# halajun/VDO_SLAM

Measured on NVIDIA H100. Metric: LM iterations/sec (batch factor-graph solve), higher is better.
Workload: dtype f64

## Files before the change

### vdo_slam_b200/csrc/ba_bodies.cuh

```cuda
#pragma once
#include "ba_math.cuh"
#include "ba_types.h"

namespace vdo {

VDO_HD double body_lin_tracklet(const BaDev& d, int t, bool write) {
  const int kb = d.tk_begin[t], ke = d.tk_begin[t + 1];
  double chi = 0.0, carry_d = 0.0, carry_b[3] = {0, 0, 0};
  double p[3] = {d.pt[3 * kb], d.pt[3 * kb + 1], d.pt[3 * kb + 2]};
  for (int k = kb; k < ke; ++k) {
    double dsum = carry_d, b[3] = {carry_b[0], carry_b[1], carry_b[2]};
    carry_d = 0; carry_b[0] = carry_b[1] = carry_b[2] = 0;
    const int eb = d.lm_obs_begin[k], ee = d.lm_obs_begin[k + 1];
    for (int e = eb; e < ee; ++e) {
      Iso T; iso_load(d.se3 + 12 * (size_t)d.lm_cam[e], T);
      double Zc[3]; iso_inv_apply(T, p, Zc);
      const double* z = d.lm_z + 3 * (size_t)e;
      double err[3] = {Zc[0] - z[0], Zc[1] - z[1], Zc[2] - z[2]};
      const int cls = d.lm_cls[e];
      const double w = d.obs_cls_w[cls];
      double rho, hw; huber(w * (err[0] * err[0] + err[1] * err[1] + err[2] * err[2]), d.obs_cls_d[cls], rho, hw);
      chi += rho;
      if (write) {
        const double om = w * hw;
// ... 133 lines not shown
    } else {
      d.tk_gamma[k] = 0.0;
    }
    d.pt_g[k] = 1.0 / (sk + tk - dk);
    t_next = tk;
  }
}

VDO_HD void body_vertex_transform(const BaDev& d, int c, const double* __restrict__ v, double* __restrict__ vw) {
  const double* T = d.se3 + 12 * (size_t)c;
  double al[3], be[3], tb[3];
  rot_apply(T, v + 6 * (size_t)c, al);
  rot_apply(T, v + 6 * (size_t)c + 3, be);
  cross3(T + 9, be, tb);
  double* o = vw + 6 * (size_t)c;
  o[0] = -al[0] - 2 * tb[0]; o[1] = -al[1] - 2 * tb[1]; o[2] = -al[2] - 2 * tb[2];
  o[3] = be[0]; o[4] = be[1]; o[5] = be[2];
  if (d.vh) {
    double* oh = d.vh + 6 * (size_t)c;
    oh[0] = al[0] + tb[0]; oh[1] = al[1] + tb[1]; oh[2] = al[2] + tb[2]; oh[3] = be[0]; oh[4] = be[1]; oh[5] = be[2];
  }
}

VDO_HD void body_schur_tracklet(const BaDev& d, int t, int mode, const double* __restrict__ v, double* __restrict__ out) {
  const int kb = d.tk_begin[t], ke = d.tk_begin[t + 1];
  double carry_u[3] = {0, 0, 0};
  double y_prev[3] = {0, 0, 0}, f_prev = 0.0, Rprev[9] = {1, 0, 0, 0, 1, 0, 0, 0, 1};
  double p[3] = {d.pt[3 * kb], d.pt[3 * kb + 1], d.pt[3 * kb + 2]};
  for (int k = kb; k < ke; ++k) {
    double u[3] = {carry_u[0], carry_u[1], carry_u[2]};
    carry_u[0] = carry_u[1] = carry_u[2] = 0;
    const int h = d.tk_h[k];
    double Rh[9] = {1, 0, 0, 0, 1, 0, 0, 0, 1};
    double pn[3] = {0, 0, 0};
    if (mode != 0) {
      const int eb = d.lm_obs_begin[k], ee = d.lm_obs_begin[k + 1];
      for (int e = eb; e < ee; ++e) {
        const double* w = d.vw + 6 * (size_t)d.lm_cam[e];
        double pxb[3]; cross3(p, w + 3, pxb);
        const double om = d.lm_omega[e];
        u[0] += om * (w[0] + 2 * pxb[0]); u[1] += om * (w[1] + 2 * pxb[1]); u[2] += om * (w[2] + 2 * pxb[2]);
      }
    }
    if (h >= 0) {
      Iso H; iso_load(d.se3 + 12 * (size_t)h, H);
#pragma unroll
      for (int i = 0; i < 9; ++i) Rh[i] = H.R[i];
      pn[0] = d.pt[3 * (k + 1)]; pn[1] = d.pt[3 * (k + 1) + 1]; pn[2] = d.pt[3 * (k + 1) + 2];
      if (mode != 0) {
        double q[3]; iso_inv_apply(H, pn, q);
        double a[3]; ter_Jh_mul(q, v + 6 * (size_t)h, a);
        const double om = d.tk_omega[k];
        u[0] += om * a[0]; u[1] += om * a[1]; u[2] += om * a[2];
        double Ra[3]; rot_apply(H.R, a, Ra);
        carry_u[0] = -om * Ra[0]; carry_u[1] = -om * Ra[1]; carry_u[2] = -om * Ra[2];
      }
    }
    double y[3];
    if (mode == 0) { y[0] = d.bl[3 * k]; y[1] = d.bl[3 * k + 1]; y[2] = d.bl[3 * k + 2]; }
    else if (mode == 1) { y[0] = u[0]; y[1] = u[1]; y[2] = u[2]; }
    else { y[0] = d.bl[3 * k] - u[0]; y[1] = d.bl[3 * k + 1] - u[1]; y[2] = d.bl[3 * k + 2] - u[2]; }
    if (k > kb) {
      double Ry[3]; rot_apply(Rprev, y_prev, Ry);
      y[0] += f_prev * Ry[0]; y[1] += f_prev * Ry[1]; y[2] += f_prev * Ry[2];
    }
    if (ke - kb == 1) {
      const double is = 1.0 / d.pt_s[k];
      out[3 * k] = y[0] * is; out[3 * k + 1] = y[1] * is; out[3 * k + 2] = y[2] * is;
      return;
    }
    out[3 * k] = y[0]; out[3 * k + 1] = y[1]; out[3 * k + 2] = y[2];
    y_prev[0] = y[0]; y_prev[1] = y[1]; y_prev[2] = y[2];
    f_prev = d.tk_omega[k] / d.pt_s[k];
#pragma unroll
    for (int i = 0; i < 9; ++i) Rprev[i] = Rh[i];
    if (h >= 0) { p[0] = pn[0]; p[1] = pn[1]; p[2] = pn[2]; }
    else if (k + 1 < ke) { p[0] = d.pt[3 * (k + 1)]; p[1] = d.pt[3 * (k + 1) + 1]; p[2] = d.pt[3 * (k + 1) + 2]; }
  }
  double zn[3] = {0, 0, 0};
  for (int k = ke - 1; k >= kb; --k) {
    double y[3] = {out[3 * k], out[3 * k + 1], out[3 * k + 2]};
    if (k < ke - 1) {
      const int h = d.tk_h[k];
      if (h >= 0) {
        const double* R = d.se3 + 12 * (size_t)h;
        double Rt[3]; rot_t_apply(R, zn, Rt);
        const double om = d.tk_omega[k];
        y[0] += om * Rt[0]; y[1] += om * Rt[1]; y[2] += om * Rt[2];
      }
    }
    const double is = 1.0 / d.pt_s[k];
    zn[0] = y[0] * is; zn[1] = y[1] * is; zn[2] = y[2] * is;
    out[3 * k] = zn[0]; out[3 * k + 1] = zn[1]; out[3 * k + 2] = zn[2];
  }
}

VDO_HD void body_lin_vertex_obs(const BaDev& d, const Iso& T, int e, double* A21, double* g6) {
  const double* p = d.pt + 3 * (size_t)d.vm_pt[e];
  double Zc[3]; iso_inv_apply(T, p, Zc);
  const double* z = d.vm_z + 3 * (size_t)e;
  double err[3] = {Zc[0] - z[0], Zc[1] - z[1], Zc[2] - z[2]};
  const int cls = d.vm_cls[e];
  const double w = d.obs_cls_w[cls];
  double rho, hw; huber(w * (err[0] * err[0] + err[1] * err[1] + err[2] * err[2]), d.obs_cls_d[cls], rho, hw);
  const double om = w * hw;
  d.vm_omega[e] = om;
  obs_accumulate_pose(Zc, err, om, A21, g6);
}
VDO_HD void body_schur_vertex_obs(const BaDev& d, const Iso& T, int e, double* acc6) {
  const int k = d.vm_pt[e];
  const double* p = d.pt + 3 * (size_t)k;
  double Zc[3]; iso_inv_apply(T, p, Zc);
  double a[3]; rot_t_apply(T.R, d.zl + 3 * (size_t)k, a);
  double o[6]; obs_JcT_mul(Zc, a, o);
  const double om = d.vm_omega[e];
#pragma unroll
  for (int i = 0; i < 6; ++i) acc6[i] += om * o[i];
}
VDO_HD void body_lin_vertex_ter(const BaDev& d, const Iso& H, int e, double* A21, double* g6) {
  const int k = d.hm_p1[e];
  const double* p1 = d.pt + 3 * (size_t)k;
  double q[3]; iso_inv_apply(H, p1 + 3, q);
  double err[3] = {p1[0] - q[0], p1[1] - q[1], p1[2] - q[2]};
  const int cls = d.hm_cls[e];
  const double w = d.ter_cls_w[cls];
  double rho, hw; huber(w * (err[0] * err[0] + err[1] * err[1] + err[2] * err[2]), d.ter_cls_d[cls], rho, hw);
  const double om = w * hw;
  d.hm_omega[e] = om;
  ter_accumulate_pose(q, err, om, A21, g6);
}
VDO_HD void body_schur_vertex_ter(const BaDev& d, const Iso& H, int e, double* acc6) {
  const int k = d.hm_p1[e];
  double q[3]; iso_inv_apply(H, d.pt + 3 * (size_t)(k + 1), q);
  double Rz[3]; rot_t_apply(H.R, d.zl + 3 * (size_t)(k + 1), Rz);
  const double* z1 = d.zl + 3 * (size_t)k;
  double a[3] = {z1[0] - Rz[0], z1[1] - Rz[1], z1[2] - Rz[2]};
  double o[6]; ter_JhT_mul(q, a, o);
  const double om = d.hm_omega[e];
#pragma unroll
  for (int i = 0; i < 6; ++i) acc6[i] += om * o[i];
}

VDO_HD bool body_se3_edge(const BaDev& d, int e, bool jac, double& chi, double* Hi, double* Hj, double* Hoff, double* gi, double* gj) {
  const int i = d.se_i[e], j = d.se_j[e];
  Iso Z, Xi; iso_load(d.se_Z + 12 * (size_t)e, Z); iso_load(d.se3 + 12 * (size_t)i, Xi);
  double err[6], Ji[36], Jj[36];
  double w = d.se_w[e];
  if (j < 0) {
    edge_prior_eval(Z, Xi, err, Ji, jac);
    double e2 = 0; for (int k = 0; k < 6; ++k) e2 += err[k] * err[k];
    chi = w * e2;
  } else {
    Iso Xj; iso_load(d.se3 + 12 * (size_t)j, Xj);
    edge_se3_eval(Z, Xi, Xj, err, Ji, Jj, jac);
    double e2 = 0; for (int k = 0; k < 6; ++k) e2 += err[k] * err[k];
    double rho, hw; huber(w * e2, d.se_delta[e], rho, hw);
    chi = rho; w *= hw;
  }
  if (!jac) return j >= 0;
  for (int r = 0; r < 6; ++r) {
    double g = 0;
    for (int k = 0; k < 6; ++k) g += Ji[6 * k + r] * err[k];
    gi[r] = -w * g;
    for (int c = 0; c < 6; ++c) {
      double s = 0;
      for (int k = 0; k < 6; ++k) s += Ji[6 * k + r] * Ji[6 * k + c];
      Hi[6 * r + c] = w * s;
    }
  }
  if (j >= 0) {
    for (int r = 0; r < 6; ++r) {
      double g = 0;
      for (int k = 0; k < 6; ++k) g += Jj[6 * k + r] * err[k];
      gj[r] = -w * g;
      for (int c = 0; c < 6; ++c) {
        double s = 0, o = 0;
        for (int k = 0; k < 6; ++k) { s += Jj[6 * k + r] * Jj[6 * k + c]; o += Ji[6 * k + r] * Jj[6 * k + c]; }
        Hj[6 * r + c] = w * s;
        Hoff[6 * r + c] = w * o;
      }
    }
  }
  return j >= 0;
}

VDO_HD void body_hpp_mul(const BaDev& d, int v, double lambda, const double* __restrict__ x, double* __restrict__ out) {
  const double* H = d.Hpp + 36 * (size_t)v;
  const double* xv = x + 6 * (size_t)v;
  double o[6];
#pragma unroll
  for (int r = 0; r < 6; ++r) {
    double s = lambda * xv[r];
#pragma unroll
    for (int c = 0; c < 6; ++c) s += H[6 * r + c] * xv[c];
    o[r] = s;
  }
  for (int n = d.nbr_begin[v]; n < d.nbr_begin[v + 1]; ++n) {
    const double* B = d.se_Hoff + 36 * (size_t)d.nbr_edge[n];
    const double* xo = x + 6 * (size_t)d.nbr_other[n];
    if (d.nbr_tr[n]) {
#pragma unroll
      for (int r = 0; r < 6; ++r)
#pragma unroll
        for (int c = 0; c < 6; ++c) o[r] += B[6 * c + r] * xo[c];
    } else {
#pragma unroll
      for (int r = 0; r < 6; ++r)
#pragma unroll
        for (int c = 0; c < 6; ++c) o[r] += B[6 * r + c] * xo[c];
    }
  }
#pragma unroll
  for (int r = 0; r < 6; ++r) out[6 * (size_t)v + r] = d.own ? o[r] : 0.0;
  body_vertex_transform(d, v, x, d.vw);
}

VDO_HD void body_precond_vertex_obs(const BaDev& d, const Iso& T, int e, double* A21) {
  const int k = d.vm_pt[e];
  double Zc[3]; iso_inv_apply(T, d.pt + 3 * (size_t)k, Zc);
  const double om = d.vm_omega[e];
  const double zero[3] = {0, 0, 0};
  double g[6] = {0, 0, 0, 0, 0, 0};
  obs_accumulate_pose(Zc, zero, om * om * d.pt_g[k], A21, g);
}
VDO_HD void body_precond_vertex_ter(const BaDev& d, const Iso& H, int e, double* A21) {
  const int k = d.hm_p1[e];
  double q[3]; iso_inv_apply(H, d.pt + 3 * (size_t)(k + 1), q);
  const double om = d.hm_omega[e];
  const double zero[3] = {0, 0, 0};
  double g[6] = {0, 0, 0, 0, 0, 0};
  ter_accumulate_pose(q, zero, om * om * d.tk_gamma[k], A21, g);
}
VDO_HD void mat6_mul(const double* A, const double* B, double* C) {
  for (int r = 0; r < 6; ++r) for (int c = 0; c < 6; ++c) { double s = 0; for (int k = 0; k < 6; ++k) s += A[6 * r + k] * B[6 * k + c]; C[6 * r + c] = s; }
}
VDO_HD void mat6_mul_nt(const double* A, const double* B, double* C) {
  for (int r = 0; r < 6; ++r) for (int c = 0; c < 6; ++c) { double s = 0; for (int k = 0; k < 6; ++k) s += A[6 * r + k] * B[6 * c + k]; C[6 * r + c] = s; }
}
VDO_HD void mat6_mul_tn(const double* A, const double* B, double* C) {
  for (int r = 0; r < 6; ++r) for (int c = 0; c < 6; ++c) { double s = 0; for (int k = 0; k < 6; ++k) s += A[6 * k + r] * B[6 * k + c]; C[6 * r + c] = s; }
}
VDO_HD void body_pcr_setup(const BaDev& d, int v, double* D, double* L) {
  const double* S = d.Minv + 36 * (size_t)v;
  for (int i = 0; i < 36; ++i) D[36 * (size_t)v + i] = S[i];
  const int e = d.pcr_edge[v];
  double* Lv = L + 36 * (size_t)v;
  if (e < 0) { for (int i = 0; i < 36; ++i) Lv[i] = 0; return; }
  const double* B = d.se_Hoff + 36 * (size_t)e;
  if (d.pcr_tr[v]) { for (int r = 0; r < 6; ++r) for (int c = 0; c < 6; ++c) Lv[6 * r + c] = B[6 * c + r]; }
  else { for (int i = 0; i < 36; ++i) Lv[i] = B[i]; }
}
VDO_HD void body_pcr_invert(const BaDev& d, int v, const double* D, double* Dinv, double lambda, int* bad) {
  double M[36];
  for (int i = 0; i < 36; ++i) M[i] = D[36 * (size_t)v + i];
  if (!spd6_inverse(M)) {
    for (int i = 0; i < 36; ++i) M[i] = 0;
    for (int i = 0; i < 6; ++i) M[7 * i] = 1.0 / (fabs(D[36 * (size_t)v + 7 * i]) + lambda);
    *bad = 1;
  }
  for (int i = 0; i < 36; ++i) Dinv[36 * (size_t)v + i] = M[i];
}
VDO_HD void body_pcr_AG(int v, int r, int c, int pb, int pe, int s, const double* L, const double* Dinv, double* A, double* G) {
  double a = 0.0, g = 0.0;
  if (v - s >= pb) {
    const double* Lv = L + 36 * (size_t)v + 6 * r; const double* Di = Dinv + 36 * (size_t)(v - s) + c;
    a = -(Lv[0] * Di[0] + Lv[1] * Di[6] + Lv[2] * Di[12] + Lv[3] * Di[18] + Lv[4] * Di[24] + Lv[5] * Di[30]);
  }
  if (v + s < pe) {
    const double* Lp = L + 36 * (size_t)(v + s) + r; const double* Di = Dinv + 36 * (size_t)(v + s) + c;
    g = -(Lp[0] * Di[0] + Lp[6] * Di[6] + Lp[12] * Di[12] + Lp[18] * Di[18] + Lp[24] * Di[24] + Lp[30] * Di[30]);
  }
  A[36 * (size_t)v + 6 * r + c] = a; G[36 * (size_t)v + 6 * r + c] = g;
}
VDO_HD void body_pcr_DL(int v, int r, int c, int pb, int pe, int s, const double* D, const double* L, const double* A, const double* G,
                        double* Dn, double* Ln) {
  double dd = D[36 * (size_t)v + 6 * r + c], ll = 0.0;
  if (v - s >= pb) {
    const double* a = A + 36 * (size_t)v + 6 * r; const double* Lv = L + 36 * (size_t)v + 6 * c;
    dd += a[0] * Lv[0] + a[1] * Lv[1] + a[2] * Lv[2] + a[3] * Lv[3] + a[4] * Lv[4] + a[5] * Lv[5];
    if (v - 2 * s >= pb) {
      const double* Lm = L + 36 * (size_t)(v - s) + c;
      ll = a[0] * Lm[0] + a[1] * Lm[6] + a[2] * Lm[12] + a[3] * Lm[18] + a[4] * Lm[24] + a[5] * Lm[30];
    }
  }
  if (v + s < pe) {
    const double* g = G + 36 * (size_t)v + 6 * r; const double* Lp = L + 36 * (size_t)(v + s) + c;
    dd += g[0] * Lp[0] + g[1] * Lp[6] + g[2] * Lp[12] + g[3] * Lp[18] + g[4] * Lp[24] + g[5] * Lp[30];
  }
  Dn[36 * (size_t)v + 6 * r + c] = dd; Ln[36 * (size_t)v + 6 * r + c] = ll;
}
VDO_HD void body_pcr_apply(int v, int pb, int pe, int s, const double* A, const double* G, const double* b, double* bn) {
  double o[6];
  for (int i = 0; i < 6; ++i) o[i] = b[6 * (size_t)v + i];
  if (v - s >= pb) {
    const double* a = A + 36 * (size_t)v; const double* x = b + 6 * (size_t)(v - s);
    for (int r = 0; r < 6; ++r) { double t = 0; for (int c = 0; c < 6; ++c) t += a[6 * r + c] * x[c]; o[r] += t; }
  }
  if (v + s < pe) {
    const double* g = G + 36 * (size_t)v; const double* x = b + 6 * (size_t)(v + s);
    for (int r = 0; r < 6; ++r) { double t = 0; for (int c = 0; c < 6; ++c) t += g[6 * r + c] * x[c]; o[r] += t; }
  }
  for (int i = 0; i < 6; ++i) bn[6 * (size_t)v + i] = o[i];
}
VDO_HD double pcr_apply_row(int v, int row, int pb, int pe, int s, const double* A, const double* G, const double* b) {
  double o = b[6 * (size_t)v + row];
  if (v - s >= pb) {
    const double* a = A + 36 * (size_t)v + 6 * row; const double* x = b + 6 * (size_t)(v - s);
    o += a[0] * x[0] + a[1] * x[1] + a[2] * x[2] + a[3] * x[3] + a[4] * x[4] + a[5] * x[5];
  }
  if (v + s < pe) {
    const double* g = G + 36 * (size_t)v + 6 * row; const double* x = b + 6 * (size_t)(v + s);
    o += g[0] * x[0] + g[1] * x[1] + g[2] * x[2] + g[3] * x[3] + g[4] * x[4] + g[5] * x[5];
  }
  return o;
}
VDO_HD int pcr_num_levels(int m) { int l = 0; while ((1 << l) < m) ++l; return l; }
VDO_HD void mul6(const double* M, const double* x, double* o) {
#pragma unroll
  for (int r = 0; r < 6; ++r) {
    double s = 0;
#pragma unroll
    for (int c = 0; c < 6; ++c) s += M[6 * r + c] * x[c];
    o[r] = s;
  }
}

VDO_HD double body_update_se3(const BaDev& d, int v, double lambda, bool reortho) {
  Iso T; iso_load(d.se3 + 12 * (size_t)v, T);
  const double* x = d.xp + 6 * (size_t)v;
  const double* b = d.bp + 6 * (size_t)v;
  iso_oplus(T, x);
  if (reortho) rot_reorthogonalize(T.R);
  iso_store(d.se3 + 12 * (size_t)v, T);
  double s = 0;
#pragma unroll
  for (int i = 0; i < 6; ++i) s += x[i] * (lambda * x[i] + b[i]);
  return d.own ? s : 0.0;
}
VDO_HD double body_update_pt(const BaDev& d, int k, double lambda) {
  double s = 0;
#pragma unroll
  for (int i = 0; i < 3; ++i) {
    const double x = d.xl[3 * (size_t)k + i];
    d.pt[3 * (size_t)k + i] += x;
    s += x * (lambda * x + d.bl[3 * (size_t)k + i]);
  }
  return s;
}

}
```

### vdo_slam_b200/csrc/ba_driver.cpp

```cpp
#include "ba_driver.h"

#include <algorithm>
#include <cfloat>
#include <cmath>
#include <cstdio>
#include <cstdlib>
#include <cstring>
#include <map>
#include <numeric>
#include <chrono>
#include <condition_variable>
#include <functional>
#include <mutex>
#include <thread>
#include <unistd.h>

namespace vdo {

namespace {
int host_threads() {
  const char* e = std::getenv("VDO_HOST_THREADS");
  const int v = e ? std::atoi(e) : (int)std::min(32u, std::max(1u, std::thread::hardware_concurrency()));
  return std::max(1, std::min(v, 64));
}
class HostPool {
 public:
  ~HostPool() {
    { std::lock_guard<std::mutex> lk(m_); stop_ = true; ++gen_; }
    cv_work_.notify_all();
    for (auto& t : th_) t.join();
  }
  void run(int nthreads, const std::function<void(int, int)>& fn) {
    if (nthreads <= 1 || inside_) { for (int t = 0; t < nthreads; ++t) fn(t, nthreads); return; }
    std::lock_guard<std::mutex> section(run_);
    {
      std::lock_guard<std::mutex> lk(m_);
      if (pid_ != getpid()) {
        new std::vector<std::thread>(std::move(th_));
        th_.clear(); pid_ = getpid();
      }
      while ((int)th_.size() < nthreads - 1) { const int id = (int)th_.size() + 1; th_.emplace_back([this, id] { worker(id); }); }
      fn_ = &fn; n_ = nthreads; pending_ = nthreads - 1; ++gen_;
    }
    cv_work_.notify_all();
    inside_ = true; fn(0, nthreads); inside_ = false;
    std::unique_lock<std::mutex> lk(m_);
    cv_done_.wait(lk, [this] { return pending_ == 0; });
    fn_ = nullptr;
  }
 private:
  void worker(int id) {
    inside_ = true;
    unsigned long seen = 0;
    for (;;) {
      const std::function<void(int, int)>* fn = nullptr; int n = 0;
      {
        std::unique_lock<std::mutex> lk(m_);
        cv_work_.wait(lk, [&] { return gen_ != seen; });
        seen = gen_;
        if (stop_) return;
        if (id < n_) { fn = fn_; n = n_; }
      }
      if (!fn) continue;
      (*fn)(id, n);
      std::lock_guard<std::mutex> lk(m_);
      if (--pending_ == 0) cv_done_.notify_one();
    }
  }
  std::vector<std::thread> th_;
  std::mutex m_, run_;
  std::condition_variable cv_work_, cv_done_;
  const std::function<void(int, int)>* fn_ = nullptr;
  int n_ = 0, pending_ = 0;
  unsigned long gen_ = 0;
  bool stop_ = false;
  pid_t pid_ = getpid();
  static thread_local bool inside_;
};
thread_local bool HostPool::inside_ = false;
HostPool& host_pool() { static HostPool* p = new HostPool; return *p; }
template <typename F> void parallel_for(int nthreads, F fn) {
  if (nthreads <= 1) { fn(0, 1); return; }
  const std::function<void(int, int)> f = fn;
  host_pool().run(nthreads, f);
}
struct Phase {
  BaBackend* be; float* acc; bool on;
  Phase(BaBackend* b, float* a, bool o) : be(b), acc(a), on(o) { if (on) be->timer_start(3); }
  ~Phase() { if (on) *acc += be->timer_stop_ms(3); }
};
}

void BaGraph::copy_bytes(void* dst, const void* src, size_t bytes) {
  if (bytes < ((size_t)4 << 20)) { std::memcpy(dst, src, bytes); return; }
  parallel_for(std::min(host_threads(), 16), [&](int t, int n) {
    const size_t a = (bytes * t / n) & ~(size_t)63, b = t + 1 == n ? bytes : ((bytes * (t + 1) / n) & ~(size_t)63);
    std::memcpy((char*)dst + a, (const char*)src + a, b - a);
  });
}
void BaGraph::fill_bytes(void* dst, int byte, size_t bytes) {
  if (bytes < ((size_t)8 << 20)) { std::memset(dst, byte, bytes); return; }
  parallel_for(std::min(host_threads(), 8), [&](int t, int n) {
    const size_t a = (bytes * t / n) & ~(size_t)63, b = t + 1 == n ? bytes : ((bytes * (t + 1) / n) & ~(size_t)63);
    std::memset((char*)dst + a, byte, b - a);
  });
}

BaGraph::~BaGraph() {
  if (finalized_) be_->release(d_);
  drop_stage();
  for (void* p : owned_) be_->free_(p);
}

int BaGraph::set_vertices(int n_se3, const double* se3, int n_pt, const double* pt) {
  if (finalized_) return fail(VDO_ERR_STATE, "set_vertices after finalize");
  if (n_se3 < 0 || n_pt < 0 || (n_se3 && !se3) || (n_pt && !pt)) return fail(VDO_ERR_ARG, "set_vertices: bad arguments");
  n_se3_ = n_se3; n_pt_ = n_pt;
  h_se3_ = HostBuf<double>(); h_pt_ = HostBuf<double>();
  append(h_se3_, se3, 12 * (size_t)n_se3);
  append(h_pt_, pt, 3 * (size_t)n_pt);
  return VDO_OK;
}
int BaGraph::add_prior(int n, const int* v, const double* Z, const double* w) {
  if (finalized_) return fail(VDO_ERR_STATE, "add after finalize");
  for (int i = 0; i < n; ++i) if (v[i] < 0 || v[i] >= n_se3_) return fail(VDO_ERR_ARG, "prior edge: vertex out of range");
  pr_v_.insert(pr_v_.end(), v, v + n); pr_Z_.insert(pr_Z_.end(), Z, Z + 12 * (size_t)n); pr_w_.insert(pr_w_.end(), w, w + n);
  return VDO_OK;
}
int BaGraph::add_se3(int n, const int* ij, const double* Z, const double* w, const double* delta) {
  if (finalized_) return fail(VDO_ERR_STATE, "add after finalize");
  for (int i = 0; i < 2 * n; ++i) if (ij[i] < 0 || ij[i] >= n_se3_) return fail(VDO_ERR_ARG, "se3 edge: vertex out of range");
  for (int i = 0; i < n; ++i) if (ij[2 * i] == ij[2 * i + 1]) return fail(VDO_ERR_ARG, "se3 edge: self loop");
  se_ij_.insert(se_ij_.end(), ij, ij + 2 * (size_t)n); se_Z_.insert(se_Z_.end(), Z, Z + 12 * (size_t)n);
  se_w_.insert(se_w_.end(), w, w + n); se_d_.insert(se_d_.end(), delta, delta + n);
  return VDO_OK;
}
int BaGraph::add_obs(int n, const int* cp, const double* z, const double* w, const double* delta) {
  if (finalized_) return fail(VDO_ERR_STATE, "add after finalize");
  for (int i = 0; i < n; ++i)
    if (cp[2 * i] < 0 || cp[2 * i] >= n_se3_ || cp[2 * i + 1] < 0 || cp[2 * i + 1] >= n_pt_) return fail(VDO_ERR_ARG, "pointxyz edge: vertex out of range");
  append(ob_cp_, cp, 2 * (size_t)n); append(ob_z_, z, 3 * (size_t)n);
  append(ob_w_, w, (size_t)n); append(ob_d_, delta, (size_t)n);
  return VDO_OK;
}
int BaGraph::add_ter(int n, const int* pph, const double* w, const double* delta) {
  if (finalized_) return fail(VDO_ERR_STATE, "add after finalize");
  for (int i = 0; i < n; ++i)
    if (pph[3 * i] < 0 || pph[3 * i] >= n_pt_ || pph[3 * i + 1] < 0 || pph[3 * i + 1] >= n_pt_ || pph[3 * i + 2] < 0 || pph[3 * i + 2] >= n_se3_)
      return fail(VDO_ERR_ARG, "landmark-motion edge: vertex out of range");
  append(te_pph_, pph, 3 * (size_t)n); append(te_w_, w, (size_t)n); append(te_d_, delta, (size_t)n);
  return VDO_OK;
}

namespace {
std::pair<int, int> thread_range(int n, int t, int nt) { return {(int)((int64_t)n * t / nt), (int)((int64_t)n * (t + 1) / nt)}; }
struct Switches { bool chunked, dense, band; };
Switches read_switches() {
  auto is = [](const char* name, const char* v) { const char* e = std::getenv(name); return e && std::string(e) == v; };
  return Switches{is("VDO_BA_LAYOUT", "chunked"), !is("VDO_BA_DENSE", "0"), !is("VDO_BA_BAND", "0")}; }
struct ClassTable {
  std::map<std::pair<double, double>, int> ids;
  std::vector<double> w, d;
  int get(double ww, double dd) {
    auto key = std::make_pair(ww, dd > 0 ? dd : 0.0);
    auto it = ids.find(key);
    if (it != ids.end()) return it->second;
    int id = (int)w.size();
    ids[key] = id; w.push_back(ww); d.push_back(key.second);
    return id;
  }
};
template <typename V, typename F> void vertex_major(int C, int n, V vertex_of, F put, std::vector<Chunk>& chunks) {
  std::vector<int> begin(C + 1, 0);
  for (int i = 0; i < n; ++i) if (vertex_of(i) >= 0) begin[vertex_of(i) + 1]++;
  for (int v = 0; v < C; ++v) begin[v + 1] += begin[v];
  std::vector<int> fill(begin.begin(), begin.end() - 1);
  for (int i = 0; i < n; ++i) if (vertex_of(i) >= 0) put(i, fill[vertex_of(i)]++);
  for (int v = 0; v < C; ++v)
    for (int b = begin[v]; b < begin[v + 1]; b += VDO_CHUNK) chunks.push_back(Chunk{v, b, std::min(b + VDO_CHUNK, begin[v + 1]), 0});
}
void counting_sort(std::vector<int>& ids, const HostBuf<int>& key_of_id, int nkeys, int NT) {
  const int n = (int)ids.size();
  if (n == 0) return;
  const int W = (n < 65536 || (size_t)nkeys * NT > 4 * (size_t)n) ? 1 : NT;
  std::vector<int> keys(n), out(n), hist((size_t)W * nkeys, 0);
  parallel_for(W, [&](int t, int w) {
    const auto [a, b] = thread_range(n, t, w);
    int* h = &hist[(size_t)t * nkeys];
    for (int i = a; i < b; ++i) { const int k = key_of_id[ids[i]]; keys[i] = k; h[k]++; }
  });
  { int run = 0; for (int k = 0; k < nkeys; ++k) for (int t = 0; t < W; ++t) { int& h = hist[(size_t)t * nkeys + k]; const int c = h; h = run; run += c; } }
  parallel_for(W, [&](int t, int w) {
    const auto [a, b] = thread_range(n, t, w);
    int* h = &hist[(size_t)t * nkeys];
    for (int i = a; i < b; ++i) out[h[keys[i]]++] = ids[i];
  });
  ids.swap(out);
}
std::vector<int> se3_path_order(int C, const std::vector<int>& se_ij, std::vector<int>& new_of_old) {
  const int Es = (int)se_ij.size() / 2;
  std::vector<int> path_begin, deg(C, 0), nb0(C, -1), nb1(C, -1), comp(C);
  std::iota(comp.begin(), comp.end(), 0);
  auto find = [&](int x) { while (comp[x] != x) { comp[x] = comp[comp[x]]; x = comp[x]; } return x; };
  std::vector<char> bad_comp(C, 0);
  for (int e = 0; e < Es; ++e) {
    int a = se_ij[2 * e], b = se_ij[2 * e + 1];
    int ra = find(a), rb = find(b);
    if (ra == rb) bad_comp[ra] = 1;
    else { comp[ra] = rb; if (bad_comp[ra]) bad_comp[rb] = 1; }
    if (deg[a] == 0) nb0[a] = b; else if (deg[a] == 1) nb1[a] = b;
    if (deg[b] == 0) nb0[b] = a; else if (deg[b] == 1) nb1[b] = a;
    deg[a]++; deg[b]++;
  }
  for (int v = 0; v < C; ++v) if (deg[v] > 2) bad_comp[find(v)] = 1;
  new_of_old.assign(C, -1);
  int cnt = 0;
  for (int v = 0; v < C; ++v) {
    if (new_of_old[v] != -1) continue;
    const bool is_path = !bad_comp[find(v)];
    if (!is_path || deg[v] == 0) { path_begin.push_back(cnt); new_of_old[v] = cnt++; continue; }
    if (deg[v] == 2) continue;
    path_begin.push_back(cnt);
    int prev = -1, cur = v;
    while (cur != -1) {
      new_of_old[cur] = cnt++;
      int nx = (nb0[cur] != prev) ? nb0[cur] : nb1[cur];
      if (deg[cur] == 1 && prev != -1) nx = -1;
      prev = cur; cur = nx;
    }
  }
  for (int v = 0; v < C; ++v) if (new_of_old[v] == -1) { path_begin.push_back(cnt); new_of_old[v] = cnt++; }
  path_begin.push_back(cnt);
  return path_begin;
}
bool pack_tiles(const std::vector<int>& tk_begin, int Tstat, const HostBuf<int>& lm_begin, const HostBuf<int>& lm_cam, int C, int NT,
                std::vector<Tile>& tiles, int& n_stat) {
  const int T = (int)tk_begin.size() - 1, nseg_st = std::max(1, std::min(48, Tstat / 8192)), nseg_ch = std::max(1, std::min(16, (T - Tstat) / 2048));
  struct SegOut { std::vector<Tile> tiles; int bad = 0; };
  std::vector<SegOut> segs((size_t)nseg_st + nseg_ch);
  auto pack = [&](int t_lo, int t_hi, SegOut& out) {
    if (t_lo >= t_hi) return;
    Tile cur{0, 0, 0, 0, 0, 0, 0, 0, 0, 0, 0, 0, 0, 0, 0, 0};
    std::vector<int> cam_tile(C, -1), fresh;
    int tile_serial = 0, ncam_cur = 0;
    auto close = [&](int t) {
      if (cur.t1 > cur.t0) out.tiles.push_back(cur);
      cur.t0 = cur.t1 = t; cur.k0 = cur.k1 = tk_begin[t]; cur.e0 = cur.e1 = lm_begin[tk_begin[t]];
      ++tile_serial; ncam_cur = 0;
    };
    close(t_lo);
    for (int t = t_lo; t < t_hi; ++t) {
      const int nl = tk_begin[t + 1] - tk_begin[t], ea = lm_begin[tk_begin[t]], eb = lm_begin[tk_begin[t + 1]], ne = eb - ea;
      if (nl > VDO_TILE_L || ne > VDO_TILE_E) { out.bad = 1; return; }
      auto count_fresh = [&]() { fresh.clear(); for (int e = ea; e < eb; ++e) if (cam_tile[lm_cam[e]] != tile_serial) { cam_tile[lm_cam[e]] = tile_serial; fresh.push_back(lm_cam[e]); } };
      count_fresh();
      if ((cur.k1 - cur.k0) + nl > VDO_TILE_L || (cur.e1 - cur.e0) + ne > VDO_TILE_E || ncam_cur + (int)fresh.size() > 255) { close(t); count_fresh(); }
      if ((int)fresh.size() > 255) { out.bad = 1; return; }
      ncam_cur += (int)fresh.size();
      cur.t1 = t + 1; cur.k1 = tk_begin[t + 1]; cur.e1 = eb;
    }
    if (cur.t1 > cur.t0) out.tiles.push_back(cur);
  };
  const int nseg = nseg_st + nseg_ch;
  parallel_for(std::min(NT, nseg), [&](int w, int n) {
    for (int sg = w; sg < nseg; sg += n) {
      const bool st = sg < nseg_st;
      const auto [a, b] = st ? thread_range(Tstat, sg, nseg_st) : thread_range(T - Tstat, sg - nseg_st, nseg_ch);
      pack(st ? a : Tstat + a, st ? b : Tstat + b, segs[sg]);
    }
  });
  for (int sg = 0; sg < nseg; ++sg) {
    if (segs[sg].bad) { tiles.clear(); return false; }
    if (sg == nseg_st) n_stat = (int)tiles.size();
    tiles.insert(tiles.end(), segs[sg].tiles.begin(), segs[sg].tiles.end());
  }
  return true;
}
struct TileRuns {
  std::vector<Seg> os, ts, os2, ts2; std::vector<int> verts;
  void append(const TileRuns& w, Tile* t, int n) {
    auto cat = [&](auto& dst, const auto& src, int Tile::*lo, int Tile::*hi) {
      const int base = (int)dst.size();
      for (int i = 0; i < n; ++i) { t[i].*lo += base; if (hi) t[i].*hi += base; }
      dst.insert(dst.end(), src.begin(), src.end());
    };
    cat(os, w.os, &Tile::os0, &Tile::os1); cat(ts, w.ts, &Tile::ts0, &Tile::ts1);
    cat(os2, w.os2, &Tile::qo0, &Tile::qo1); cat(ts2, w.ts2, &Tile::qt0, &Tile::qt1);
    cat(verts, w.verts, &Tile::vs0, nullptr);
  }
};
void cut_runs(const std::vector<int>& keys, const HostBuf<uint16_t>& perm, int base, int n, int cap, std::vector<Seg>& out) {
  for (int a = 0; a < n;) {
    const int v = keys[perm[base + a]];
    int b = a;
    while (b < n && b - a < cap && keys[perm[base + b]] == v) ++b;
    out.push_back(Seg{v, base + a, b - a, 0});
    a = b;
  }
}
}
struct BaGraph::Tracklets { std::vector<int> begin; HostBuf<int> old_of_new; int Tstat = 0, T = 0, P = 0; std::vector<int64_t> bucket; HostBuf<int> eidx, n_obs; };
struct BaGraph::EdgeClasses { ClassTable table; HostBuf<uint8_t> of_edge; };
struct BaGraph::LmStream { HostBuf<int> begin, cam; HostBuf<double> z; HostBuf<uint8_t> cls; int E = 0; };
struct BaGraph::Ternary { HostBuf<int> h; HostBuf<uint8_t> cls; ClassTable table; int E = 0; };
struct BaGraph::TileLayout { bool tiled = false; std::vector<Tile> tiles; int n_stat = 0; TileRuns runs;
                             HostBuf<uint16_t> ob_perm, tr_perm; HostBuf<uint8_t> lm_lml, lm_cslot, tk_hslot; HostBuf<uint32_t> ob_ps; };
struct BaGraph::Chunked { std::vector<int> vm_pt; std::vector<double> vm_z; std::vector<uint8_t> vm_cls; std::vector<Chunk> obs_chunks;
                          std::vector<int> hm_p1; std::vector<uint8_t> hm_cls; std::vector<Chunk> ter_chunks; };
struct BaGraph::Se3Edges { std::vector<int> i, j; std::vector<double> Z, w, d; std::vector<int> nbr_begin, nbr_edge, nbr_other;
                           std::vector<uint8_t> nbr_tr; std::vector<int> path_of, pcr_edge; std::vector<uint8_t> pcr_tr; int pcr_levels = 0; };
struct BaGraph::Solvers { bool dense = false; int band_W = 0, band_v0 = 0, band_n = 0; };
int BaGraph::order_tracklets(int NT, const Lap& lap, Tracklets& tk) {
  const int C = n_se3_, P = n_pt_, Eo = (int)ob_w_.size(), Et = (int)te_w_.size(), rank = be_->rank, world = be_->world;
  HostBuf<int> next = stage_fill<int>(P, 0xFF), prev = stage_fill<int>(P, 0xFF), ter_of = stage_fill<int>(P, 0xFF);
  for (int e = 0; e < Et; ++e) {
    int p1 = te_pph_[3 * e], p2 = te_pph_[3 * e + 1];
    if (p1 == p2 || next[p1] != -1 || prev[p2] != -1)
      return fail(VDO_ERR_UNSUPPORTED, "landmark-motion edges must form simple chains (one predecessor / successor per landmark)");
    next[p1] = p2; prev[p2] = p1; ter_of[p1] = e;
  }
  lap("  chain links");
  new_of_old_.assign(P, -1);
  tk.old_of_new = stage<int>(P);
  const int NB = NT, P0 = std::max(P, 1);
  auto bucket_of = [NB, P0](int p) { return (int)((int64_t)p * NB / P0); };
  std::vector<int64_t> tb((size_t)NT * NB + 1, 0);
  parallel_for(NT, [&](int t, int n) {
    const auto [a, b] = thread_range(Eo, t, n);
    int64_t* c = &tb[(size_t)t * NB];
    for (int e = a; e < b; ++e) c[bucket_of(ob_cp_[2 * e + 1])]++;
  });
  std::vector<int64_t> off((size_t)NB * NT + 1, 0);
  { int64_t run = 0; for (int b = 0; b < NB; ++b) for (int t = 0; t < NT; ++t) { off[(size_t)b * NT + t] = run; run += tb[(size_t)t * NB + b]; } off[(size_t)NB * NT] = run; }
  tk.eidx = stage<int>(Eo);
  parallel_for(NT, [&](int t, int n) {
    const auto [a, b] = thread_range(Eo, t, n);
    std::vector<int64_t> cur(NB);
    for (int k = 0; k < NB; ++k) cur[k] = off[(size_t)k * NT + t];
    for (int e = a; e < b; ++e) tk.eidx[cur[bucket_of(ob_cp_[2 * e + 1])]++] = e;
  });
  for (int b = 0; b <= NB; ++b) tk.bucket.push_back(off[(size_t)b * NT]);
  HostBuf<int> first_cam = stage<int>(P); tk.n_obs = stage_fill<int>(P, 0);
  parallel_for(NB, [&](int b, int) {
    const int lo = (int)(((int64_t)b * P + NB - 1) / NB), hi = (int)(((int64_t)(b + 1) * P + NB - 1) / NB);
    for (int p = lo; p < hi && p < P; ++p) first_cam[p] = C;
    for (int64_t q = tk.bucket[b]; q < tk.bucket[b + 1]; ++q) {
      const int e = tk.eidx[q], p = ob_cp_[2 * e + 1], c = new_se3_of_old_[ob_cp_[2 * e]];
      if (c < first_cam[p]) first_cam[p] = c;
      tk.n_obs[p]++;
    }
  });
  lap("  first_cam scan");
  std::vector<int> stat_ids, chain_heads;
  {
    std::vector<size_t> ns(NT + 1, 0), nc(NT + 1, 0);
    parallel_for(NT, [&](int t, int n) {
      const auto [a, b] = thread_range(P, t, n);
      size_t s0 = 0, c0 = 0;
      for (int p = a; p < b; ++p) if (prev[p] == -1) { if (next[p] == -1) ++s0; else ++c0; }
      ns[t + 1] = s0; nc[t + 1] = c0;
    });
    for (int t = 0; t < NT; ++t) { ns[t + 1] += ns[t]; nc[t + 1] += nc[t]; }
    stat_ids.resize(ns[NT]); chain_heads.resize(nc[NT]);
    parallel_for(NT, [&](int t, int n) {
      const auto [a, b] = thread_range(P, t, n);
      size_t s0 = ns[t], c0 = nc[t];
      for (int p = a; p < b; ++p) if (prev[p] == -1) { if (next[p] == -1) stat_ids[s0++] = p; else chain_heads[c0++] = p; }
    });
  }
  lap("  collect heads");
  {
    int mx = 0;
    for (int p : stat_ids) mx = std::max(mx, tk.n_obs[p]);
    HostBuf<int> neg = stage<int>(P);
    parallel_for(NT, [&](int t, int n) {
      const auto [a, b] = thread_range((int)stat_ids.size(), t, n);
      for (int i = a; i < b; ++i) neg[stat_ids[i]] = mx - tk.n_obs[stat_ids[i]];
    });
    counting_sort(stat_ids, neg, mx + 1, NT);
  }
  counting_sort(stat_ids, first_cam, C + 1, NT);
  {
    HostBuf<int> first_h = stage_fill<int>(P, 0);
    for (int p : chain_heads) first_h[p] = new_se3_of_old_[te_pph_[3 * ter_of[p] + 2]];
    counting_sort(chain_heads, first_cam, C + 1, NT);
    counting_sort(chain_heads, first_h, C + 1, NT);
  }
  lap("  counting sorts");
  const int n_heads = (int)chain_heads.size();
  std::vector<int> chain_len(n_heads);
  std::vector<int64_t> seen_part(NT, 0);
  parallel_for(NT, [&](int t, int n) {
    const auto [a, b] = thread_range(n_heads, t, n);
    int64_t sum = 0;
    for (int i = a; i < b; ++i) { int len = 0; for (int q = chain_heads[i]; q != -1; q = next[q]) ++len; chain_len[i] = len; sum += len; }
    seen_part[t] = sum;
  });
  int64_t n_seen = (int64_t)stat_ids.size();
  for (int64_t v : seen_part) n_seen += v;
  if (n_seen != P) return fail(VDO_ERR_UNSUPPORTED, "landmark-motion edges contain a cycle");
  std::vector<int> stat_keep, head_keep, head_len;
  if (world == 1) { stat_keep.swap(stat_ids); head_keep.swap(chain_heads); head_len.swap(chain_len); }
  else {
    for (size_t i = rank; i < stat_ids.size(); i += world) stat_keep.push_back(stat_ids[i]);
    for (size_t i = rank; i < chain_heads.size(); i += world) { head_keep.push_back(chain_heads[i]); head_len.push_back(chain_len[i]); }
  }
  const int Tstat = (int)stat_keep.size(), Tch = (int)head_keep.size();
  tk.begin.resize((size_t)Tstat + Tch + 1);
  { int run = Tstat; for (int i = 0; i < Tch; ++i) { tk.begin[Tstat + i] = run; run += head_len[i]; } tk.begin[Tstat + Tch] = run; tk.P = run; }
  parallel_for(NT, [&](int t, int n) {
    const auto [a, b] = thread_range(Tstat, t, n);
    for (int i = a; i < b; ++i) { tk.begin[i] = i; new_of_old_[stat_keep[i]] = i; tk.old_of_new[i] = stat_keep[i]; }
    const auto [c, d2] = thread_range(Tch, t, n);
    for (int i = c; i < d2; ++i) { int k = tk.begin[Tstat + i]; for (int q = head_keep[i]; q != -1; q = next[q]) { new_of_old_[q] = k; tk.old_of_new[k++] = q; } }
  });
  tk.Tstat = Tstat; tk.T = Tstat + Tch;
  return VDO_OK;
}
int BaGraph::edge_classes(const HostBuf<double>& w, const HostBuf<double>& d, int NT, const char* family, EdgeClasses& out) {
  const int n = (int)w.size();
  out.of_edge = stage<uint8_t>(n);
  std::vector<char> uniform(NT, 1);
  if (n > 0) {
    const double w0 = w[0], d0 = d[0];
    parallel_for(NT, [&](int t, int nt) {
      const auto [a, b] = thread_range(n, t, nt);
      char u = 1;
      for (int e = a; e < b; ++e) if (w[e] != w0 || d[e] != d0) { u = 0; break; }
      uniform[t] = u;
    });
  }
  bool all_uniform = n > 0;
  for (char u : uniform) all_uniform = all_uniform && u;
  if (all_uniform) { const int c0 = out.table.get(w[0], d[0]); fill_bytes(out.of_edge.p, c0, (size_t)n); return VDO_OK; }
  double lw = 0, ld = 0; int lc = -1;
  for (int e = 0; e < n; ++e) {
    if (lc < 0 || w[e] != lw || d[e] != ld) {
      lc = out.table.get(w[e], d[e]); lw = w[e]; ld = d[e];
      if (lc > 255) return fail(VDO_ERR_UNSUPPORTED, std::string("more than 256 distinct (information, Huber delta) pairs on ") + family + " edges");
    }
    out.of_edge[e] = (uint8_t)lc;
  }
  return VDO_OK;
}
BaGraph::LmStream BaGraph::landmark_stream(const Tracklets& tk, const HostBuf<uint8_t>& ecls, int NT, const Lap& lap) {
  const int P = tk.P, NB = (int)tk.bucket.size() - 1;
  LmStream lm;
  lm.begin = stage<int>((size_t)P + 1); lm.begin[0] = 0;
  parallel_for(NT, [&](int t, int n) {
    const auto [a, b] = thread_range(P, t, n);
    for (int k = a; k < b; ++k) lm.begin[k + 1] = tk.n_obs[tk.old_of_new[k]];
  });
  lap("  count");
  for (int k = 0; k < P; ++k) lm.begin[k + 1] += lm.begin[k];
  const int Eo = lm.E = lm.begin[P];
  lm.cam = stage<int>(Eo); lm.z = stage<double>(3 * (size_t)Eo); lm.cls = stage<uint8_t>(Eo);
  HostBuf<int> written = tk.n_obs;
  fill_bytes(written.p, 0, sizeof(int) * (size_t)n_pt_);
  lap("  prefix + alloc");
  parallel_for(NB, [&](int b, int) {
    for (int64_t q = tk.bucket[b]; q < tk.bucket[b + 1]; ++q) {
      const int e = tk.eidx[q], p = ob_cp_[2 * e + 1], k = new_of_old_[p];
      if (k < 0) continue;
      const int pos = lm.begin[k] + written[p]++;
      lm.cam[pos] = new_se3_of_old_[ob_cp_[2 * e]];
      lm.z[3 * (size_t)pos] = ob_z_[3 * (size_t)e]; lm.z[3 * (size_t)pos + 1] = ob_z_[3 * (size_t)e + 1]; lm.z[3 * (size_t)pos + 2] = ob_z_[3 * (size_t)e + 2];
      lm.cls[pos] = ecls[e];
    }
  });
  return lm;
}
int BaGraph::ternary_edges(const Tracklets& tk, int NT, Ternary& ter) {
  const int P = tk.P, Et_all = (int)te_w_.size();
  ter.h = stage_fill<int>(P, 0xFF); ter.cls = stage_fill<uint8_t>(P, 0);
  EdgeClasses tc;
  if (int rc = edge_classes(te_w_, te_d_, NT, "landmark-motion", tc)) return rc;
  ter.table = std::move(tc.table);
  parallel_for(NT, [&](int t, int n) {
    const auto [a, b] = thread_range(Et_all, t, n);
    for (int e = a; e < b; ++e)
      if (const int k = new_of_old_[te_pph_[3 * e]]; k >= 0) { ter.h[k] = new_se3_of_old_[te_pph_[3 * e + 2]]; ter.cls[k] = tc.of_edge[e]; }
  });
  ter.E = tk.P - tk.T;
  return VDO_OK;
}
BaGraph::Chunked BaGraph::chunked_streams(const LmStream& lm, const Ternary& ter, int C, int P) {
  Chunked ch;
  ch.vm_pt.resize(lm.E); ch.vm_z.resize(3 * (size_t)lm.E); ch.vm_cls.resize(lm.E);
  int k = 0;
  vertex_major(C, lm.E, [&](int pos) { return lm.cam[pos]; }, [&](int pos, int q) {
    while (lm.begin[k + 1] <= pos) ++k;
    ch.vm_pt[q] = k; ch.vm_cls[q] = lm.cls[pos];
    for (int i = 0; i < 3; ++i) ch.vm_z[3 * (size_t)q + i] = lm.z[3 * (size_t)pos + i];
  }, ch.obs_chunks);
  ch.hm_p1.resize(ter.E); ch.hm_cls.resize(ter.E);
  vertex_major(C, P, [&](int k) { return ter.h[k]; }, [&](int k, int q) { ch.hm_p1[q] = k; ch.hm_cls[q] = ter.cls[k]; }, ch.ter_chunks);
  return ch;
}
int BaGraph::tile_runs(const LmStream& lm, const Ternary& ter, int P, int NT, TileLayout& tl) {
  const int Eo = lm.E;
  tl.ob_perm = stage<uint16_t>(Eo); tl.tr_perm = stage_fill<uint16_t>(P, 0); tl.lm_lml = stage<uint8_t>(Eo); tl.ob_ps = stage<uint32_t>(Eo);
  tl.lm_cslot = stage<uint8_t>(Eo); tl.tk_hslot = stage_fill<uint8_t>(P, 0xFF);
  const int ntl = (int)tl.tiles.size();
  const int NW = std::max(1, std::min(NT, ntl / 64 + 1));
  std::vector<TileRuns> w_runs(NW);
  std::vector<char> w_bad(NW, 0);
  parallel_for(NW, [&](int wt, int wn) {
    std::vector<int> keys(std::max(VDO_TILE_E, VDO_TILE_L)), idx(keys.size()), bucket;
    TileRuns& r = w_runs[wt];
    auto sort_and_cut = [&](int n, int base, HostBuf<uint16_t>& perm, std::vector<Seg>& segs, std::vector<Seg>& segs2, HostBuf<uint8_t>& slot) {
      if (n == 0) return 0;
      int lo = keys[idx[0]], hi = lo;
      for (int a = 1; a < n; ++a) { lo = std::min(lo, keys[idx[a]]); hi = std::max(hi, keys[idx[a]]); }
      const int range = hi - lo + 1;
      if (range <= 8 * n + 64) {
        bucket.assign(range + 1, 0);
        for (int a = 0; a < n; ++a) bucket[keys[idx[a]] - lo + 1]++;
        for (int a = 0; a < range; ++a) bucket[a + 1] += bucket[a];
        for (int a = 0; a < n; ++a) perm[base + bucket[keys[idx[a]] - lo]++] = (uint16_t)idx[a];
      } else {
        std::stable_sort(idx.begin(), idx.begin() + n, [&](int x, int y) { return keys[x] < keys[y]; });
        for (int a = 0; a < n; ++a) perm[base + a] = (uint16_t)idx[a];
      }
      cut_runs(keys, perm, base, n, VDO_SEG, segs);
      cut_runs(keys, perm, base, n, VDO_SEG2, segs2);
      int nv = 0;
      for (int q = 0; q < n; ++q) {
        const int i = perm[base + q];
        if (q == 0 || keys[i] != keys[perm[base + q - 1]]) { r.verts.push_back(keys[i]); ++nv; }
        slot[base + i] = (uint8_t)(nv - 1);
      }
      return nv;
    };
    const auto [ta, tb] = thread_range(ntl, wt, wn);
    for (int ti = ta; ti < tb; ++ti) {
      Tile& t = tl.tiles[ti];
      for (int k = t.k0; k < t.k1; ++k) for (int e = lm.begin[k]; e < lm.begin[k + 1]; ++e) tl.lm_lml[e] = (uint8_t)(k - t.k0);
      const int ne = t.e1 - t.e0;
      for (int i = 0; i < ne; ++i) { keys[i] = lm.cam[t.e0 + i]; idx[i] = i; }
      t.os0 = (int)r.os.size(); t.qo0 = (int)r.os2.size(); t.vs0 = (int)r.verts.size();
      const int ncam = sort_and_cut(ne, t.e0, tl.ob_perm, r.os, r.os2, tl.lm_cslot);
      t.os1 = (int)r.os.size(); t.qo1 = (int)r.os2.size();
      for (int q = 0; q < ne; ++q) { const int i = tl.ob_perm[t.e0 + q]; tl.ob_ps[t.e0 + q] = (uint32_t)i | ((uint32_t)tl.lm_lml[t.e0 + i] << 16); }
      int nt = 0;
      for (int k = t.k0; k < t.k1; ++k) if (ter.h[k] >= 0) { keys[k - t.k0] = ter.h[k]; idx[nt++] = k - t.k0; }
      t.ts0 = (int)r.ts.size(); t.qt0 = (int)r.ts2.size();
      const int nmot = sort_and_cut(nt, t.k0, tl.tr_perm, r.ts, r.ts2, tl.tk_hslot);
      t.ts1 = (int)r.ts.size(); t.qt1 = (int)r.ts2.size();
      if (ncam > 255 || nmot > 255) w_bad[wt] = 1;
      t.nv = ncam | (nmot << 16);
    }
  });
  for (int wt = 0; wt < NW; ++wt) {
    const auto [ta, tb] = thread_range(ntl, wt, NW);
    tl.runs.append(w_runs[wt], tl.tiles.data() + ta, tb - ta);
    if (w_bad[wt]) return fail(VDO_ERR_UNSUPPORTED, "a tile meets more than 255 motion vertices");
  }
  return VDO_OK;
}
BaGraph::Se3Edges BaGraph::se3_edges(const std::vector<int>& path_begin) const {
  const int C = n_se3_, Ep = (int)pr_w_.size(), Es = (int)se_w_.size(), Ese = Ep + Es;
  auto S3 = [&](int old_id) { return new_se3_of_old_[old_id]; };
  Se3Edges se;
  se.i.resize(Ese); se.j.resize(Ese); se.Z.resize(12 * (size_t)Ese); se.w.resize(Ese); se.d.resize(Ese);
  for (int e = 0; e < Ep; ++e) { se.i[e] = S3(pr_v_[e]); se.j[e] = -1; se.w[e] = pr_w_[e]; se.d[e] = 0; std::memcpy(&se.Z[12 * (size_t)e], &pr_Z_[12 * (size_t)e], 96); }
  for (int e = 0; e < Es; ++e) {
    int q = Ep + e;
    se.i[q] = S3(se_ij_[2 * e]); se.j[q] = S3(se_ij_[2 * e + 1]); se.w[q] = se_w_[e]; se.d[q] = se_d_[e] > 0 ? se_d_[e] : 0;
    std::memcpy(&se.Z[12 * (size_t)q], &se_Z_[12 * (size_t)e], 96);
  }
  se.nbr_begin.assign(C + 1, 0);
  for (int e = Ep; e < Ese; ++e) { se.nbr_begin[se.i[e] + 1]++; se.nbr_begin[se.j[e] + 1]++; }
  for (int v = 0; v < C; ++v) se.nbr_begin[v + 1] += se.nbr_begin[v];
  std::vector<int> nfill(se.nbr_begin.begin(), se.nbr_begin.end() - 1);
  se.nbr_edge.resize(2 * (size_t)Es); se.nbr_other.resize(2 * (size_t)Es); se.nbr_tr.resize(2 * (size_t)Es);
  for (int e = Ep; e < Ese; ++e) {
    int a = nfill[se.i[e]]++; se.nbr_edge[a] = e; se.nbr_other[a] = se.j[e]; se.nbr_tr[a] = 0;
    int b = nfill[se.j[e]]++; se.nbr_edge[b] = e; se.nbr_other[b] = se.i[e]; se.nbr_tr[b] = 1;
  }
  const int n_paths = (int)path_begin.size() - 1;
  se.path_of.resize(C); se.pcr_edge.assign(C, -1); se.pcr_tr.assign(C, 0);
  int max_len = 1;
  for (int pth = 0; pth < n_paths; ++pth) {
    for (int v = path_begin[pth]; v < path_begin[pth + 1]; ++v) se.path_of[v] = pth;
    max_len = std::max(max_len, path_begin[pth + 1] - path_begin[pth]);
  }
  for (int e = Ep; e < Ese; ++e) {
    int a = se.i[e], b = se.j[e];
    if (se.path_of[a] != se.path_of[b]) continue;
    if (b == a + 1) { se.pcr_edge[b] = e; se.pcr_tr[b] = 1; }
    else if (a == b + 1) { se.pcr_edge[a] = e; se.pcr_tr[a] = 0; }
  }
  while ((1 << se.pcr_levels) < max_len) ++se.pcr_levels;
  return se;
}
void BaGraph::states(const Tracklets& tk, int NT, HostBuf<double>& se3, HostBuf<double>& pt) {
  const int C = n_se3_, P = tk.P;
  se3 = stage<double>(12 * (size_t)C);
  for (int o = 0; o < C; ++o) std::memcpy(&se3[12 * (size_t)new_se3_of_old_[o]], &h_se3_[12 * (size_t)o], 96);
  pt = stage<double>(3 * (size_t)P);
  parallel_for(NT, [&](int t, int n) {
    const auto [a, b] = thread_range(P, t, n);
    for (int k = a; k < b; ++k) for (int i = 0; i < 3; ++i) pt[3 * (size_t)k + i] = h_pt_[3 * (size_t)tk.old_of_new[k] + i];
  });
}
BaGraph::Solvers BaGraph::choose_solvers(bool allow_dense, bool allow_band, bool tiled, const Tracklets& tk, const LmStream& lm, int NT) const {
  const int C = n_se3_, Tstat = tk.Tstat, Wmax = be_->band_max_width();
  Solvers s;
  s.dense = allow_dense && tiled && be_->world == 1 && Tstat == tk.T && 6 * C <= be_->dense_capacity();
  if (!tiled || Tstat == 0 || Wmax <= 0) return s;
  std::vector<int> w_W(NT, 0), w_v0(NT, C), w_v1(NT, -1), w_bad(NT, 0);
  parallel_for(NT, [&](int t, int n) {
    const auto [a, b] = thread_range(Tstat, t, n);
    int W = 0, v0 = C, v1 = -1, bad = 0;
    for (int k = a; k < b && !bad; ++k) {
      const int e0 = lm.begin[k], e1 = lm.begin[k + 1];
      if (e1 <= e0) continue;
      for (int e = e0 + 1; e < e1; ++e) if (lm.cam[e] <= lm.cam[e - 1]) { bad = 1; break; }
      W = std::max(W, lm.cam[e1 - 1] - lm.cam[e0] + 1); v0 = std::min(v0, lm.cam[e0]); v1 = std::max(v1, lm.cam[e1 - 1]);
    }
    w_W[t] = W; w_v0[t] = v0; w_v1[t] = v1; w_bad[t] = bad;
  });
  int W = 0, v0 = C, v1 = -1, bad = 0;
  for (int t = 0; t < NT; ++t) { W = std::max(W, w_W[t]); v0 = std::min(v0, w_v0[t]); v1 = std::max(v1, w_v1[t]); bad |= w_bad[t]; }
  if (allow_band && !bad && v1 >= v0 && W <= Wmax && (size_t)(v1 - v0 + 1) * W * 80 <= ((size_t)512 << 20)) {
    s.band_W = W; s.band_v0 = v0; s.band_n = v1 - v0 + 1;
  }
  return s;
}
void BaGraph::upload_layout(const std::vector<int>& path_begin, const Tracklets& tk, const LmStream& lm, const EdgeClasses& oc, const Ternary& ter,
                            const TileLayout& tl, const Chunked& ch, const Se3Edges& se, const HostBuf<double>& se3, const HostBuf<double>& pt,
                            const Solvers& sv) {
  const int C = n_se3_, P = tk.P, Eo = lm.E, Ese = (int)se.i.size(), n_paths = (int)path_begin.size() - 1, rank = be_->rank, world = be_->world;
  BaDev& d = d_;
  d.C = C; d.P = P; d.T = tk.T; d.Tstat = tk.Tstat; d.own = (rank == 0) ? 1 : 0;
  P_all_ = n_pt_; d.Eobs = Eo; d.Eter = ter.E; d.Ese = Ese;
  d.n_obs_chunks = (int)ch.obs_chunks.size(); d.n_ter_chunks = (int)ch.ter_chunks.size(); d.n_nbr = (int)se.nbr_edge.size();
  d.se3 = upload(se3); d.pt = upload(pt);
  d.se3_init = dalloc<double>(12 * (size_t)C); d.pt_init = dalloc<double>(3 * (size_t)P);
  be_->d2d(d.se3_init, d.se3, 96 * (size_t)C); be_->d2d(d.pt_init, d.pt, 24 * (size_t)P);
  d.se3_bk = dalloc<double>(12 * (size_t)C); d.pt_bk = dalloc<double>(3 * (size_t)P);
  d.tk_begin = upload(tk.begin);
  d.lm_obs_begin = upload(lm.begin); d.lm_cam = upload(lm.cam); d.lm_z = upload(lm.z); d.lm_cls = upload(lm.cls); d.lm_omega = dalloc<double>(Eo);
  d.tk_h = upload(ter.h); d.tk_cls = upload(ter.cls); d.tk_omega = dalloc<double>(P);
  d.tiled = tl.tiled ? 1 : 0;
  if (!tl.tiled) {
    d.vm_pt = upload(ch.vm_pt); d.vm_z = upload(ch.vm_z); d.vm_cls = upload(ch.vm_cls); d.vm_omega = dalloc<double>(Eo); d.obs_chunks = upload(ch.obs_chunks);
    d.hm_p1 = upload(ch.hm_p1); d.hm_cls = upload(ch.hm_cls); d.hm_omega = dalloc<double>(ter.E); d.ter_chunks = upload(ch.ter_chunks);
  } else {
    const std::vector<Tile>& tiles = tl.tiles;
    d.n_tiles = (int)tiles.size(); d.n_tiles_stat = tl.n_stat; d.n_osegs = (int)tl.runs.os.size(); d.n_tsegs = (int)tl.runs.ts.size();
    d.capE_st = d.capE_ch = 16; d.capV_st = d.capV_ch = d.capH_ch = 1;
    for (int ti = 0; ti < d.n_tiles; ++ti) {
      const bool st = ti < tl.n_stat;
      int& cap = st ? d.capE_st : d.capE_ch;
      cap = std::max(cap, (tiles[ti].e1 - tiles[ti].e0 + 15) & ~15);
      int& cv = st ? d.capV_st : d.capV_ch;
      cv = std::max(cv, tiles[ti].nv & 0xFFFF);
      if (!st) d.capH_ch = std::max(d.capH_ch, tiles[ti].nv >> 16);
    }
    d.tiles = upload(tiles); d.osegs = upload(tl.runs.os); d.tsegs = upload(tl.runs.ts); d.osegs2 = upload(tl.runs.os2); d.tsegs2 = upload(tl.runs.ts2);
    d.ob_perm = upload(tl.ob_perm); d.tr_perm = upload(tl.tr_perm); d.lm_lml = upload(tl.lm_lml); d.ob_ps = upload(tl.ob_ps);
    d.tile_verts = upload(tl.runs.verts); d.lm_cslot = upload(tl.lm_cslot); d.tk_hslot = upload(tl.tk_hslot);
    d.pt_Q = dalloc<double>(9 * (size_t)std::max(P - tk.Tstat, 1));
    d.accO = dalloc<double>(16 * (size_t)C); d.accT = dalloc<double>(16 * (size_t)C); d.acc6 = dalloc<double>(12 * (size_t)C);
    d.vh = dalloc<double>(6 * (size_t)C);
  }
  d.se_i = upload(se.i); d.se_j = upload(se.j); d.se_Z = upload(se.Z); d.se_w = upload(se.w); d.se_delta = upload(se.d); d.se_Hoff = dalloc<double>(36 * (size_t)Ese);
  d.nbr_begin = upload(se.nbr_begin); d.nbr_edge = upload(se.nbr_edge); d.nbr_other = upload(se.nbr_other); d.nbr_tr = upload(se.nbr_tr);
  d.Hpp = dalloc<double>(42 * (size_t)C); d.bp = d.Hpp + 36 * (size_t)C; d.hll = dalloc<double>(P); d.bl = dalloc<double>(3 * (size_t)P);
  d.pt_s = dalloc<double>(P); d.Minv = dalloc<double>(36 * (size_t)C);
  d.pt_g = dalloc<double>(P); d.tk_gamma = dalloc<double>(P);
  d.n_paths = n_paths; d.pcr_levels = se.pcr_levels;
  d.path_begin = upload(path_begin); d.path_of = upload(se.path_of); d.pcr_edge = upload(se.pcr_edge); d.pcr_tr = upload(se.pcr_tr);
  d.pcr_D = dalloc<double>(72 * (size_t)C); d.pcr_L = dalloc<double>(72 * (size_t)C); d.pcr_Dinv = dalloc<double>(36 * (size_t)C);
  d.pcr_A = dalloc<double>(36 * (size_t)C * std::max(se.pcr_levels, 1)); d.pcr_G = dalloc<double>(36 * (size_t)C * std::max(se.pcr_levels, 1));
  d.pcr_b = dalloc<double>(12 * (size_t)C);
  d.xp = dalloc<double>(6 * (size_t)C); d.r = dalloc<double>(6 * (size_t)C); d.z = dalloc<double>(6 * (size_t)C);
  d.p = dalloc<double>(6 * (size_t)C); d.Ap = dalloc<double>(6 * (size_t)C); d.rhs = dalloc<double>(6 * (size_t)C);
  d.p2 = dalloc<double>(6 * (size_t)C); d.ticket = dalloc<unsigned int>(4);
  if (sv.dense) d.Sdense = dalloc<double>((size_t)36 * C * C + 6 * (size_t)C + 8);
  if (sv.band_W) {
    d.band_W = sv.band_W; d.band_v0 = sv.band_v0; d.band_n = sv.band_n;
    d.band = dalloc<double>((size_t)d.band_n * d.band_W * 10);
  }
  d.zl = tl.tiled ? nullptr : dalloc<double>(3 * (size_t)P); d.xl = dalloc<double>(3 * (size_t)P); d.vw = dalloc<double>(6 * (size_t)C);
  auto upload256 = [&](std::vector<double> v) { v.resize(256, 0.0); return upload(v); };
  d.obs_cls_w = upload256(oc.table.w); d.obs_cls_d = upload256(oc.table.d); d.ter_cls_w = upload256(ter.table.w); d.ter_cls_d = upload256(ter.table.d);
  d.scal = dalloc<double>(SC_N);
  d.n_part_pap = tl.tiled ? std::max(1, (C + 127) / 128) : 148;
  d.n_part_rz = std::max(1, n_paths) * 8;
  d.part_pap = dalloc<double>(d.n_part_pap); d.part_rz = dalloc<double>(d.n_part_rz);
  const bool sharded = be_->shard_paths(d);
  std::vector<int> own, shorts;
  for (int pth = 0; pth < n_paths; ++pth) {
    if (sharded && pth % world != rank) continue;
    if (path_begin[pth + 1] - path_begin[pth] > VDO_PCR_SHORT) own.push_back(pth); else shorts.push_back(pth);
  }
  d.n_own_long = (int)own.size();
  own.insert(own.end(), shorts.begin(), shorts.end());
  d.n_own_paths = (int)own.size();
  d.own_paths = upload(own);
  be_->sync();
}
int BaGraph::finalize() {
  if (finalized_) return fail(VDO_ERR_STATE, "finalize called twice");
  const Switches sw = read_switches();
  const bool prof = std::getenv("VDO_PROFILE") != nullptr;
  auto tp0 = std::chrono::steady_clock::now();
  const Lap lap = [&](const char* what) {
    if (!prof) return;
    auto t = std::chrono::steady_clock::now();
    std::fprintf(stderr, "[vdo_b200] finalize: %-28s %.1f ms\n", what, std::chrono::duration<double, std::milli>(t - tp0).count());
    tp0 = t;
  };
  const int C = n_se3_, NT = host_threads();
  int rc;
  const std::vector<int> path_begin = se3_path_order(C, se_ij_, new_se3_of_old_);
  lap("se3 paths");
  Tracklets tk; if ((rc = order_tracklets(NT, lap, tk))) return rc;
  lap("tracklet order");
  EdgeClasses oc; if ((rc = edge_classes(ob_w_, ob_d_, NT, "pointxyz", oc))) return rc;
  lap("  edge classes");
  const LmStream lm = landmark_stream(tk, oc.of_edge, NT, lap);
  lap("landmark-major stream");
  TileLayout tl;
  tl.tiled = !sw.chunked && pack_tiles(tk.begin, tk.Tstat, lm.begin, lm.cam, C, NT, tl.tiles, tl.n_stat);
  Ternary ter; if ((rc = ternary_edges(tk, NT, ter))) return rc;
  const Chunked ch = tl.tiled ? Chunked() : chunked_streams(lm, ter, C, tk.P);
  lap("ternary / chunked streams");
  if (tl.tiled && (rc = tile_runs(lm, ter, tk.P, NT, tl))) return rc;
  lap("tile segments");
  const Se3Edges se = se3_edges(path_begin);
  HostBuf<double> se3, pt; states(tk, NT, se3, pt);
  lap("se3 edges, states");
  upload_layout(path_begin, tk, lm, oc, ter, tl, ch, se, se3, pt, choose_solvers(sw.dense, sw.band, tl.tiled, tk, lm, NT));
  lap("alloc + upload");
  ob_z_ = HostBuf<double>(); ob_w_ = HostBuf<double>(); ob_d_ = HostBuf<double>(); ob_cp_ = HostBuf<int>();
  te_pph_ = HostBuf<int>(); te_w_ = HostBuf<double>(); te_d_ = HostBuf<double>();
  std::vector<double>().swap(se_Z_); std::vector<double>().swap(pr_Z_);
  h_se3_ = HostBuf<double>(); h_pt_ = HostBuf<double>();
  n_prior_ = (int)pr_w_.size();
  drop_stage();
  finalized_ = true;
  return VDO_OK;
}

int BaGraph::get_vertices(double* se3, double* pt) {
  if (!finalized_) return fail(VDO_ERR_STATE, "get_vertices before finalize");
  if (se3) {
    std::vector<double> tmp(12 * (size_t)d_.C);
    be_->d2h(tmp.data(), d_.se3, 96 * (size_t)d_.C);
    for (int o = 0; o < d_.C; ++o) std::memcpy(se3 + 12 * (size_t)o, &tmp[12 * (size_t)new_se3_of_old_[o]], 96);
  }
  if (pt) {
    HostBuf<double> tmp = stage<double>(3 * (size_t)d_.P);
    be_->d2h(tmp.data(), d_.pt, 24 * (size_t)d_.P);
    const int Pa = P_all_;
    parallel_for(std::min(host_threads(), 8), [&](int t, int n) {
      const auto [a, b] = thread_range(Pa, t, n);
      for (int o = a; o < b; ++o) {
        const int k = new_of_old_[o];
        if (k < 0) continue;
        pt[3 * (size_t)o] = tmp[3 * (size_t)k]; pt[3 * (size_t)o + 1] = tmp[3 * (size_t)k + 1]; pt[3 * (size_t)o + 2] = tmp[3 * (size_t)k + 2];
      }
    });
    drop_stage();
  }
  return VDO_OK;
}
int BaGraph::reset_vertices() {
  if (!finalized_) return fail(VDO_ERR_STATE, "reset_vertices before finalize");
  be_->d2d(d_.se3, d_.se3_init, 96 * (size_t)d_.C);
  be_->d2d(d_.pt, d_.pt_init, 24 * (size_t)d_.P);
  oplus_calls_ = 0;
  return VDO_OK;
}
int BaGraph::info(int64_t out[8]) const {
  out[0] = d_.C; out[1] = d_.P; out[2] = d_.Eobs; out[3] = d_.Eter; out[4] = d_.Ese; out[5] = n_prior_; out[6] = d_.T; out[7] = (int64_t)bytes_;
  return VDO_OK;
}

int BaGraph::solver_info(int64_t out[8]) const {
  out[0] = d_.tiled; out[1] = d_.n_tiles; out[2] = d_.n_tiles_stat; out[3] = d_.band ? d_.band_W : 0; out[4] = d_.band ? d_.band_n : 0;
  out[5] = d_.Sdense ? 1 : 0; out[6] = d_.xg_paths; out[7] = d_.n_paths;
  return VDO_OK;
}

void BaGraph::zero_system() {
  be_->zero(d_.Hpp, 336 * (size_t)d_.C);
  be_->zero(d_.scal, sizeof(double) * SC_LAMBDA);
}

struct BaGraph::Round {
  std::vector<int> flag, rt;
  std::vector<double> lam, tol2;
  explicit Round(int n) : flag(n, 0), rt(n, 0), lam(n, 0.0), tol2(n, 0.0) {}
  void set(BaBackend* be) const { be->batch_set(flag.data(), lam.data(), rt.data(), tol2.data()); }
};

void BaGraph::lin_round(BaGraph* const* gs, int n, Round& r) {
  BaBackend* be = gs[0]->be_;
  for (int k = 0; k < n; ++k) if (r.flag[k] & BaBackend::BATCH_LIN) gs[k]->zero_system();
  r.set(be);
  be->lin_tracklets_batch(BaBackend::BATCH_LIN, true);
  be->lin_vertex_batch(BaBackend::BATCH_LIN);
  be->lin_se3_edges_batch(BaBackend::BATCH_LIN, true);
  for (int k = 0; k < n; ++k) {
    if (!(r.flag[k] & BaBackend::BATCH_LIN)) continue;
    be->allreduce_sum(gs[k]->d_.Hpp, 42 * (size_t)gs[k]->d_.C);
    be->allreduce_sum(gs[k]->d_.scal + SC_CHI2, 1);
  }
  be->max_diagonal_batch(BaBackend::BATCH_MAXDIAG);
  for (int k = 0; k < n; ++k) if (r.flag[k] & BaBackend::BATCH_MAXDIAG) be->allreduce_max(gs[k]->d_.scal + SC_MAXDIAG, 1);
}

void BaGraph::chi2_step(BaGraph* const* gs, int n, const Round& r, int len) {
  BaBackend* be = gs[0]->be_;
  for (int k = 0; k < n; ++k) if (r.flag[k] & BaBackend::BATCH_TRIAL) be->zero(gs[k]->d_.scal + SC_CHI2, sizeof(double));
  be->lin_tracklets_batch(BaBackend::BATCH_TRIAL, false);
  be->lin_se3_edges_batch(BaBackend::BATCH_TRIAL, false);
  for (int k = 0; k < n; ++k) if (r.flag[k] & BaBackend::BATCH_TRIAL) be->allreduce_sum(gs[k]->d_.scal + SC_CHI2, len);
}

void BaGraph::trial_round(BaGraph* const* gs, int n, Round& r, int pcg_max_iterations, Stage last, float* prof_ms, int* pcg_iters, int* ok) {
  using B = BaBackend;
  BaBackend* be = gs[0]->be_;
  const bool prof = prof_ms != nullptr;
  float unused[5];
  float* ms = prof ? prof_ms : unused;
  for (int k = 0; k < n; ++k) if (r.flag[k] & B::BATCH_TRIAL) { gs[k]->push(); pcg_iters[k] = 0; ok[k] = 1; }
  r.set(be);
  {
    Phase ph(be, &ms[0], prof);
    be->factor_landmarks_batch(B::BATCH_TRIAL);
    be->dense_solve_batch(B::BATCH_DENSE);
    be->precondition_batch(B::BATCH_PCG);
  }
  {
    Phase ph(be, &ms[1], prof);
    be->schur_rhs_batch(B::BATCH_PCG);
    for (int k = 0; k < n; ++k) if (r.flag[k] & B::BATCH_PCG) be->allreduce_sum(gs[k]->d_.rhs, 6 * (size_t)gs[k]->d_.C);
    be->pcg_init_batch(B::BATCH_PCG);
  }
  if (last == SETUP) return;
  {
    Phase ph(be, &ms[2], prof);
    const int chunk = 8;
    std::vector<int> run;
    for (int k = 0; k < n; ++k) if (r.flag[k] & B::BATCH_PCG) run.push_back(k);
    std::vector<const double*> src;
    std::vector<double> sc;
    for (int it = 0; !run.empty() && it < pcg_max_iterations; it += chunk) {
      be->pcg_iterate_batch(B::BATCH_PCG, chunk);
      src.clear();
      for (int k : run) src.push_back(gs[k]->d_.scal);
      sc.resize(run.size() * SC_N);
      be->read_scalars(src.data(), (int)run.size(), SC_N, sc.data());
      size_t m = 0;
      for (size_t j = 0; j < run.size(); ++j) {
        const int k = run[j];
        const double* c = &sc[j * SC_N];
        if (c[SC_DONE] == 0.0 && it + chunk < pcg_max_iterations) { run[m++] = k; continue; }
        BaDev& d = gs[k]->d_;
        pcg_iters[k] = (int)c[SC_ITERS];
        if (c[SC_DONE] >= 2.0 || !std::isfinite(c[SC_RZ])) ok[k] = 0;
        if (d.xg_paths) be->allreduce_sum(d.xp, 6 * (size_t)d.C);
        r.flag[k] &= ~B::BATCH_PCG;
      }
      const bool changed = m < run.size();
      run.resize(m);
      if (changed && !run.empty()) r.set(be);
    }
  }
  {
    Phase ph(be, &ms[3], prof);
    be->back_substitute_batch(B::BATCH_TRIAL);
  }
  if (last == BACKSUB) return;
  Phase ph(be, &ms[4], prof);
  for (int k = 0; k < n; ++k) if (r.flag[k] & B::BATCH_TRIAL) be->zero(gs[k]->d_.scal + SC_SCALE, sizeof(double));
  be->apply_update_batch(B::BATCH_TRIAL);
  chi2_step(gs, n, r, 2);
}

bool BaGraph::lone(Stage last, double lambda, int solver, double tol2, int pcg_max_iterations, int* pcg_iters) {
  BaGraph* self = this;
  BaDev* d = &d_;
  Round r(1);
  int it = 0, ok = 1;
  be_->batch_begin(&d, 1);
  r.flag[0] = BaBackend::BATCH_LIN;
  lin_round(&self, 1, r);
  if (last != LINEARIZE) {
    r.flag[0] = BaBackend::BATCH_TRIAL | solver; r.lam[0] = lambda; r.tol2[0] = tol2;
    trial_round(&self, 1, r, pcg_max_iterations, last, nullptr, &it, &ok);
  }
  be_->batch_end();
  if (pcg_iters) *pcg_iters = it;
  return ok != 0;
}

struct BaGraph::LmState {
  BaGraph* g = nullptr; double* hist = nullptr;
  double lambda = -1, ni = 2; int nbad = 0, trials = 0, pcg_total = 0, iters_done = 0, it = 0;
  bool stop_flag = false, ok = true, done = false;
  double chi2_check = 0, last_chi_action = 0, chi_cur = 0, chi_init = 0, gain_prev = 1.0;
  bool in_iter = false, trial_ok = true;
  double ini = 0, current = 0; int qmax = 0; double rho = 0;
};

int BaGraph::optimize(const vdo_lm_options& o_in, vdo_lm_stats* stats, double* hist) {
  BaGraph* self = this;
  return optimize_batch(&self, 1, o_in, stats, &hist);
}

void BaGraph::push() {
  be_->d2d(d_.se3_bk, d_.se3, 96 * (size_t)d_.C);
  be_->d2d(d_.pt_bk, d_.pt, 24 * (size_t)d_.P);
}
void BaGraph::pop() {
  be_->d2d(d_.se3, d_.se3_bk, 96 * (size_t)d_.C);
  be_->d2d(d_.pt, d_.pt_bk, 24 * (size_t)d_.P);
}
bool BaGraph::next_oplus_reorthogonalizes() {
  ++oplus_calls_;
  if (oplus_calls_ <= 1000) return false;
  oplus_calls_ = 0;
  return true;
}

int BaGraph::optimize_batch(BaGraph* const* gs, int n, const vdo_lm_options& o_in, vdo_lm_stats* stats, double* const* hists) {
  for (int k = 0; k < n; ++k) if (!gs[k]->finalized_) return gs[k]->fail(VDO_ERR_STATE, "optimize before finalize");
  vdo_lm_options opt = o_in;
  if (opt.max_trials <= 0) opt.max_trials = 10;
  if (opt.pcg_rel_tol <= 0) opt.pcg_rel_tol = 1e-6;
  if (opt.pcg_max_iterations <= 0) opt.pcg_max_iterations = 2000;
  BaBackend* be = gs[0]->be_;
  const int launches0 = be->launches();
  const bool prof = std::getenv("VDO_PROFILE") != nullptr;
  float prof_ms[5] = {0, 0, 0, 0, 0};
  std::vector<LmState> S(n);
  std::vector<const double*> src(n);
  std::vector<double> sc((size_t)n * SC_N);
  std::vector<int> act, pcg_iters(n, 0), trial_ok(n, 1);
  act.reserve(n);
  std::vector<BaDev*> ds(n);
  Round r(n);
  be->timer_start(0);
  for (int k = 0; k < n; ++k) {
    S[k].g = gs[k]; S[k].hist = hists ? hists[k] : nullptr;
    ds[k] = &gs[k]->d_;
    r.flag[k] = BaBackend::BATCH_TRIAL;
    src[k] = gs[k]->d_.scal + SC_CHI2;
  }
  be->batch_begin(ds.data(), n);
  r.set(be);
  chi2_step(gs, n, r, 1);
  float ms_lin = 0, ms_solve = 0;
  be->read_scalars(src.data(), n, 1, sc.data());
  for (int k = 0; k < n; ++k) {
    S[k].chi_cur = S[k].chi_init = sc[k];
    if (S[k].hist) S[k].hist[0] = sc[k];
  }
  const double loose_tol = opt.pcg_loose_tol, switch_gain = opt.pcg_switch_gain;
  bool solve_timer = false;
  for (;;) {
    act.clear();
    for (int k = 0; k < n; ++k) {
      LmState& s = S[k];
      if (s.done || s.in_iter) continue;
      if (s.it < opt.max_iterations && ((!s.stop_flag && s.ok) || opt.force_all_iterations)) act.push_back(k); else s.done = true;
    }
    if (!act.empty()) {
      be->timer_start(1);
      int n0 = 0;
      std::fill(r.flag.begin(), r.flag.end(), 0);
      for (int k : act) {
        LmState& s = S[k]; BaGraph* g = s.g;
        g->cur_pcg_tol_ = (loose_tol > opt.pcg_rel_tol && switch_gain > 0 && s.gain_prev > switch_gain) ? loose_tol : opt.pcg_rel_tol;
// ... 285 lines not shown
```

### vdo_slam_b200/csrc/ba_kernels.cu

```cuda
#include <cuda_runtime.h>
#include <cooperative_groups.h>

#include <cstdio>
#include <cstring>

#include <dlfcn.h>
#include <nccl.h>

#include <map>
#include <set>
#include <type_traits>
#include <utility>

#include "ba_bodies.cuh"

namespace cg = cooperative_groups;

namespace vdo {

constexpr int PCR_CL = 8;

#define CK(x)                                                                                       \
  do {                                                                                              \
    cudaError_t e_ = (x);                                                                           \
// ... 29 lines not shown
       BT_DINIT, BT_DSE3, BT_FROM_BAND, BT_SCHUR2, BT_FIN_SCHUR2, BT_DSCHUR, BT_CHOL,
       BT_PRE_BEGIN, BT_PRE_ST, BT_PRE_CH, BT_PRE_FIN, BT_PCR_L, BT_PCR_S, BT_RHS_ST, BT_RHS_CH, BT_VERT, BT_PCG_L, BT_PCG_S, BT_PCG_FIN, BT_BAND_MUL,
       BT_S2_ST, BT_S2_CH, BT_PHPP, BT_FIN_DOT, BT_N };
struct BatchDev { const BaDev* ds; const int* first; const int* band_per; int* flags; double* lambda; int* reortho; double* tol2; int n; };
struct One {
  BaDev d; double lam; int rt, par, band_per;
  __device__ __forceinline__ const BaDev* pick(int& blk, int& g) const { blk = blockIdx.x; g = 0; return &d; }
  __device__ __forceinline__ double lambda(int) const { return lam; }
  __device__ __forceinline__ int reortho(int) const { return rt; }
  __device__ __forceinline__ int parity() const { return par; }
  __device__ __forceinline__ int tiles_per_cta(int) const { return band_per; }
  __device__ __forceinline__ int ctas(int) const { return (int)gridDim.x; }
};
struct Many {
  BatchDev B; const int* f; int bit, par;
  __device__ __forceinline__ const BaDev* pick(int& blk, int& g) const {
    const int b = blockIdx.x;
    int lo = 0, hi = B.n;
    while (hi - lo > 1) { const int mid = (lo + hi) >> 1; if (f[mid] <= b) lo = mid; else hi = mid; }
    blk = b - f[lo]; g = lo;
    return (B.flags[lo] & bit) ? B.ds + lo : nullptr;
  }
  __device__ __forceinline__ double lambda(int g) const { return B.lambda[g]; }
  __device__ __forceinline__ int reortho(int g) const { return B.reortho[g]; }
  __device__ __forceinline__ int parity() const { return par; }
  __device__ __forceinline__ int tiles_per_cta(int g) const { return B.band_per[g]; }
  __device__ __forceinline__ int ctas(int g) const { return f[g + 1] - f[g]; }
};
#define VDO_PICK                                   \
  int blk_, g_;                                    \
  const BaDev* const dp_ = s.pick(blk_, g_);       \
  if (!dp_) return;                                \
  const BaDev& d = *dp_;
__host__ __device__ __forceinline__ unsigned int pcg_total_ctas(const BaDev& d) { return (unsigned int)(d.n_own_long * PCR_CL + (d.n_own_paths - d.n_own_long)); }

template <bool WRITE>
__global__ void __launch_bounds__(128) k_lin_tracklets(BaDev d) {
  __shared__ double red[32];
  const int t = d.Tstat + blockIdx.x * blockDim.x + threadIdx.x;
  double chi = 0.0;
  if (t < d.T) chi = body_lin_tracklet(d, t, WRITE);
  chi = block_sum(chi, red);
  if (threadIdx.x == 0 && chi != 0.0) atomicAdd(d.scal + SC_CHI2, chi);
}
template <bool WRITE>
__global__ void __launch_bounds__(256) k_lin_static(BaDev d) {
  __shared__ double red[32];
  const int k = blockIdx.x * blockDim.x + threadIdx.x;
  double chi = 0.0;
  if (k < d.Tstat) chi = body_lin_static(d, k, WRITE);
  chi = block_sum(chi, red);
  if (threadIdx.x == 0 && chi != 0.0) atomicAdd(d.scal + SC_CHI2, chi);
}

template <int NV>
__device__ __forceinline__ void block_reduce_vec(double* acc, double* smem ) {
  const int lane = threadIdx.x & 31, w = threadIdx.x >> 5, nw = blockDim.x >> 5;
#pragma unroll
  for (int i = 0; i < NV; ++i) {
    double v = warp_sum(acc[i]);
    if (lane == 0) smem[w * NV + i] = v;
  }
  __syncthreads();
  if (threadIdx.x < NV) {
    double s = 0;
    for (int k = 0; k < nw; ++k) s += smem[k * NV + threadIdx.x];
    smem[threadIdx.x] = s;
  }
  __syncthreads();
}

template <int MODE, bool OBS>
__global__ void __launch_bounds__(128) k_vertex_sym(BaDev d) {
  __shared__ double sm[4 * 27];
  const Chunk ch = OBS ? d.obs_chunks[blockIdx.x] : d.ter_chunks[blockIdx.x];
  Iso T; iso_load(d.se3 + 12 * (size_t)ch.v, T);
  double acc[27];
#pragma unroll
  for (int i = 0; i < 27; ++i) acc[i] = 0.0;
  for (int e = ch.begin + threadIdx.x; e < ch.end; e += blockDim.x) {
    if (MODE == 0) { if (OBS) body_lin_vertex_obs(d, T, e, acc, acc + 21); else body_lin_vertex_ter(d, T, e, acc, acc + 21); }
    else { if (OBS) body_precond_vertex_obs(d, T, e, acc); else body_precond_vertex_ter(d, T, e, acc); }
  }
  block_reduce_vec<27>(acc, sm);
  if (threadIdx.x < 36) {
    const int r = threadIdx.x / 6, c = threadIdx.x % 6;
    const double v = sm[r <= c ? sym6_idx(r, c) : sym6_idx(c, r)];
    if (MODE == 0) atomicAdd(d.Hpp + 36 * (size_t)ch.v + threadIdx.x, v);
    else atomicAdd(d.Minv + 36 * (size_t)ch.v + threadIdx.x, -v);
  } else if (MODE == 0 && threadIdx.x < 42) {
    atomicAdd(d.bp + 6 * (size_t)ch.v + (threadIdx.x - 36), sm[21 + threadIdx.x - 36]);
  }
}

template <bool OBS>
__global__ void __launch_bounds__(128) k_schur_vertex(BaDev d, double sign, double* __restrict__ out, int check_done) {
  __shared__ double sm[4 * 6];
  if (check_done && d.scal[SC_DONE] != 0.0) return;
  const Chunk ch = OBS ? d.obs_chunks[blockIdx.x] : d.ter_chunks[blockIdx.x];
  Iso T; iso_load(d.se3 + 12 * (size_t)ch.v, T);
  double acc[6] = {0, 0, 0, 0, 0, 0};
  for (int e = ch.begin + threadIdx.x; e < ch.end; e += blockDim.x) {
    if (OBS) body_schur_vertex_obs(d, T, e, acc); else body_schur_vertex_ter(d, T, e, acc);
  }
  block_reduce_vec<6>(acc, sm);
  if (threadIdx.x < 6) atomicAdd(out + 6 * (size_t)ch.v + threadIdx.x, sign * sm[threadIdx.x]);
}

template <bool WRITE>
__device__ __forceinline__ void k_lin_se3_edges_body(const BaDev& d, int bx) {
  __shared__ double red[32];
  const int e = bx * blockDim.x + threadIdx.x;
  double chi = 0.0;
  if (e < d.Ese) {
    double Hi[36], Hj[36], Ho[36], gi[6], gj[6];
    const bool binary = body_se3_edge(d, e, WRITE, chi, Hi, Hj, Ho, gi, gj);
    if (!d.own) chi = 0.0;
    if (WRITE) {
      const int i = d.se_i[e];
      if (d.own) {
        for (int k = 0; k < 36; ++k) atomicAdd(d.Hpp + 36 * (size_t)i + k, Hi[k]);
        for (int k = 0; k < 6; ++k) atomicAdd(d.bp + 6 * (size_t)i + k, gi[k]);
      }
      if (binary) {
        const int j = d.se_j[e];
        for (int k = 0; k < 36; ++k) { if (d.own) atomicAdd(d.Hpp + 36 * (size_t)j + k, Hj[k]); d.se_Hoff[36 * (size_t)e + k] = Ho[k]; }
        if (d.own) for (int k = 0; k < 6; ++k) atomicAdd(d.bp + 6 * (size_t)j + k, gj[k]);
      }
    }
  }
  chi = block_sum(chi, red);
  if (threadIdx.x == 0 && chi != 0.0) atomicAdd(d.scal + SC_CHI2, chi);
}
template <class S, bool WRITE>
__global__ void __launch_bounds__(64) k_lin_se3_edges(S s) { VDO_PICK k_lin_se3_edges_body<WRITE>(d, blk_); }

__device__ __forceinline__ void k_max_diagonal_body(const BaDev& d, int bx, int gx) {
  __shared__ double red[32];
  const int n1 = d.C * 6, n = n1 + d.P;
  double m = 0.0;
  for (int i = bx * blockDim.x + threadIdx.x; i < n; i += gx * blockDim.x)
    m = fmax(m, i < n1 ? fabs(d.Hpp[36 * (size_t)(i / 6) + 7 * (i % 6)]) : fabs(d.hll[i - n1]));
#pragma unroll
  for (int o = 16; o > 0; o >>= 1) m = fmax(m, __shfl_down_sync(0xffffffffu, m, o));
  const int lane = threadIdx.x & 31, w = threadIdx.x >> 5;
  if (lane == 0) red[w] = m;
  __syncthreads();
  if (threadIdx.x == 0) {
    for (int k = 1; k < (int)(blockDim.x >> 5); ++k) m = fmax(m, red[k]);
    atomicMax(reinterpret_cast<unsigned long long*>(d.scal + SC_MAXDIAG), (unsigned long long)__double_as_longlong(m));
  }
}
template <class S>
__global__ void __launch_bounds__(256) k_max_diagonal(S s) { VDO_PICK k_max_diagonal_body(d, blk_, s.ctas(g_)); }

__device__ __forceinline__ void k_factor_landmarks_body(const BaDev& d, double lambda, int bx) {
  const int t = bx * blockDim.x + threadIdx.x;
  if (t < d.Tstat) body_factor_static(d, t, lambda);
  else if (t < d.T) body_factor_tracklet(d, t, lambda);
}
template <class S>
__global__ void __launch_bounds__(128) k_factor_landmarks(S s) { VDO_PICK k_factor_landmarks_body(d, s.lambda(g_), blk_); }

template <int MODE>
__global__ void __launch_bounds__(128) k_schur_chains8(BaDev d, const double* __restrict__ v, double* __restrict__ out) {
  if (MODE == 1 && d.scal[SC_DONE] != 0.0) return;
  const int lane8 = threadIdx.x & 7;
  const int t = d.Tstat + ((blockIdx.x * blockDim.x + threadIdx.x) >> 3);
  const bool live = t < d.T;
  const int kb = live ? d.tk_begin[t] : 0, ke = live ? d.tk_begin[t + 1] : 0;
  const unsigned FULL = 0xffffffffu;
  double seg_w[3] = {0, 0, 0};
  double seg_c[3] = {0, 0, 0};
  for (int base = kb; __any_sync(FULL, base < ke); base += 8) {
    const int k = base + lane8;
    const bool valid = k < ke;
    double u[3] = {0, 0, 0}, cn[3] = {0, 0, 0}, R[9] = {1, 0, 0, 0, 1, 0, 0, 0, 1};
    double f = 0.0;
    if (valid) {
      const int h = d.tk_h[k];
      const double om = d.tk_omega[k];
      f = om / d.pt_s[k];
      if (MODE != 0) {
        const double p[3] = {d.pt[3 * (size_t)k], d.pt[3 * (size_t)k + 1], d.pt[3 * (size_t)k + 2]};
        for (int e = d.lm_obs_begin[k]; e < d.lm_obs_begin[k + 1]; ++e) {
          const double* w = d.vw + 6 * (size_t)d.lm_cam[e];
          double pxb[3]; cross3(p, w + 3, pxb);
          const double oe = d.lm_omega[e];
          u[0] += oe * (w[0] + 2 * pxb[0]); u[1] += oe * (w[1] + 2 * pxb[1]); u[2] += oe * (w[2] + 2 * pxb[2]);
        }
      }
      if (h >= 0) {
        Iso H; iso_load(d.se3 + 12 * (size_t)h, H);
#pragma unroll
        for (int i = 0; i < 9; ++i) R[i] = H.R[i];
        if (MODE != 0) {
          const double pn[3] = {d.pt[3 * (size_t)(k + 1)], d.pt[3 * (size_t)(k + 1) + 1], d.pt[3 * (size_t)(k + 1) + 2]};
          double q[3]; iso_inv_apply(H, pn, q);
          double a[3]; ter_Jh_mul(q, v + 6 * (size_t)h, a);
          u[0] += om * a[0]; u[1] += om * a[1]; u[2] += om * a[2];
          double Ra[3]; rot_apply(H.R, a, Ra);
          cn[0] = -om * Ra[0]; cn[1] = -om * Ra[1]; cn[2] = -om * Ra[2];
        }
      }
    }
    double cp[3];
#pragma unroll
    for (int i = 0; i < 3; ++i) { cp[i] = __shfl_up_sync(FULL, cn[i], 1, 8); if (lane8 == 0) cp[i] = seg_c[i]; }
#pragma unroll
    for (int i = 0; i < 3; ++i) { u[i] += cp[i]; seg_c[i] = __shfl_sync(FULL, cn[i], 7, 8); }
    double y[3];
    if (valid) {
      if (MODE == 0) { y[0] = d.bl[3 * (size_t)k]; y[1] = d.bl[3 * (size_t)k + 1]; y[2] = d.bl[3 * (size_t)k + 2]; }
      else if (MODE == 1) { y[0] = u[0]; y[1] = u[1]; y[2] = u[2]; }
      else { y[0] = d.bl[3 * (size_t)k] - u[0]; y[1] = d.bl[3 * (size_t)k + 1] - u[1]; y[2] = d.bl[3 * (size_t)k + 2] - u[2]; }
    } else { y[0] = y[1] = y[2] = 0; }
    double wout[3] = {0, 0, 0};
#pragma unroll
    for (int j = 0; j < 8; ++j) {
      double win[3];
#pragma unroll
      for (int i = 0; i < 3; ++i) win[i] = __shfl_up_sync(FULL, wout[i], 1, 8);
      if (lane8 == j) {
        if (j == 0) { win[0] = seg_w[0]; win[1] = seg_w[1]; win[2] = seg_w[2]; }
        y[0] += win[0]; y[1] += win[1]; y[2] += win[2];
        double Ry[3]; rot_apply(R, y, Ry);
        wout[0] = f * Ry[0]; wout[1] = f * Ry[1]; wout[2] = f * Ry[2];
      }
    }
#pragma unroll
    for (int i = 0; i < 3; ++i) seg_w[i] = __shfl_sync(FULL, wout[i], 7, 8);
    if (valid) { out[3 * (size_t)k] = y[0]; out[3 * (size_t)k + 1] = y[1]; out[3 * (size_t)k + 2] = y[2]; }
  }
  double seg_z[3] = {0, 0, 0};
  const int nseg = (ke - kb + 7) >> 3;
  int max_seg = nseg;
  { const int a = __shfl_xor_sync(FULL, max_seg, 8); if (a > max_seg) max_seg = a; }
  { const int a = __shfl_xor_sync(FULL, max_seg, 16); if (a > max_seg) max_seg = a; }
  for (int sgi = max_seg - 1; sgi >= 0; --sgi) {
    const int k = kb + 8 * sgi + lane8;
    const bool valid = sgi < nseg && k < ke;
    double y[3] = {0, 0, 0}, Rt[9] = {1, 0, 0, 0, 1, 0, 0, 0, 1}, om = 0.0, is = 0.0;
    bool last = true;
    if (valid) {
      y[0] = out[3 * (size_t)k]; y[1] = out[3 * (size_t)k + 1]; y[2] = out[3 * (size_t)k + 2];
      is = 1.0 / d.pt_s[k];
      const int h = d.tk_h[k];
      if (h >= 0 && k + 1 < ke) {
        last = false; om = d.tk_omega[k];
        const double* Rp = d.se3 + 12 * (size_t)h;
#pragma unroll
        for (int i = 0; i < 9; ++i) Rt[i] = Rp[i];
      }
    }
    double z[3] = {0, 0, 0};
#pragma unroll
    for (int j = 7; j >= 0; --j) {
      double zn[3];
#pragma unroll
      for (int i = 0; i < 3; ++i) zn[i] = __shfl_down_sync(FULL, z[i], 1, 8);
      if (lane8 == j && valid) {
        if (j == 7) { zn[0] = seg_z[0]; zn[1] = seg_z[1]; zn[2] = seg_z[2]; }
        if (!last) {
          double t3[3]; rot_t_apply(Rt, zn, t3);
          y[0] += om * t3[0]; y[1] += om * t3[1]; y[2] += om * t3[2];
        }
        z[0] = y[0] * is; z[1] = y[1] * is; z[2] = y[2] * is;
      }
    }
#pragma unroll
    for (int i = 0; i < 3; ++i) seg_z[i] = __shfl_sync(FULL, z[i], 0, 8);
    if (valid) { out[3 * (size_t)k] = z[0]; out[3 * (size_t)k + 1] = z[1]; out[3 * (size_t)k + 2] = z[2]; }
  }
}

template <int MODE>
__global__ void __launch_bounds__(256) k_schur_static(BaDev d, double* __restrict__ out) {
  if (MODE == 1 && d.scal[SC_DONE] != 0.0) return;
  const int k = blockIdx.x * blockDim.x + threadIdx.x;
  if (k < d.Tstat) body_schur_static(d, k, MODE, out);
}

__device__ __forceinline__ void k_precond_begin_body(const BaDev& d, double lambda, int bx) {
  const int i = bx * blockDim.x + threadIdx.x;
  if (i < d.C * 36) { const int k = i % 36; d.Minv[i] = d.own ? d.Hpp[i] + ((k % 7) == 0 ? lambda : 0.0) : 0.0; }
}
template <class S>
__global__ void __launch_bounds__(128) k_precond_begin(S s) { VDO_PICK k_precond_begin_body(d, s.lambda(g_), blk_); }

__global__ void k_set_scalars(BaDev d, double lambda, double tol2) { d.scal[SC_LAMBDA] = lambda; d.scal[SC_TOL2] = tol2; }
__device__ __forceinline__ void k_vertex_transform_body(const BaDev& d, const double* __restrict__ x, int bx) {
  const int v = bx * blockDim.x + threadIdx.x;
  if (v < d.C) body_vertex_transform(d, v, x, d.vw);
}
template <class S>
__global__ void __launch_bounds__(128) k_vertex_transform(S s, const double* __restrict__ x) { VDO_PICK k_vertex_transform_body(d, x ? x : d.xp, blk_); }
__global__ void __launch_bounds__(128) k_hpp_mul(BaDev d, const double* __restrict__ x, double* __restrict__ out) {
  if (d.scal[SC_DONE] != 0.0) return;
  const double lambda = d.scal[SC_LAMBDA];
  const int v = blockIdx.x * blockDim.x + threadIdx.x;
  if (v < d.C) body_hpp_mul(d, v, lambda, x, out);
}


__device__ __forceinline__ bool gj6_rows(double (&a)[6], int i) {
  bool ok = true;
#pragma unroll
  for (int k = 0; k < 6; ++k) {
    double rk[6];
#pragma unroll
    for (int c = 0; c < 6; ++c) rk[c] = __shfl_sync(0xffffffffu, a[c], k, 8);
    const double piv = rk[k];
    if (!(piv > 0.0) || !(piv < 1e300)) ok = false;
    const double pinv = 1.0 / piv;
    if (i == k) {
#pragma unroll
      for (int c = 0; c < 6; ++c) a[c] = (c == k) ? pinv : rk[c] * pinv;
    } else {
      const double f = a[k] * pinv;
#pragma unroll
      for (int c = 0; c < 6; ++c) a[c] = (c == k) ? -f : a[c] - f * rk[c];
    }
  }
  return ok;
}
template <int CL>
__device__ __forceinline__ void k_pcr_factor_body(const BaDev& d, double lambda, int path0, int bx) {
  cg::cluster_group cl = cg::this_cluster();
  const int path = d.own_paths[path0 + bx / CL];
  const int pb = d.path_begin[path], pe = d.path_begin[path + 1];
  const int nl = pcr_num_levels(pe - pb);
  const int tid = cl.block_rank() * blockDim.x + threadIdx.x, nth = CL * blockDim.x;
  const int grp = tid >> 3, i = tid & 7, ngrp = nth >> 3;
  const size_t N36 = 36 * (size_t)d.C;
  __shared__ double sblk[32 * 180];
  double* const Dm = d.pcr_D;
  double* const DI[2] = {d.pcr_Dinv, d.pcr_D + N36};
  int bad = 0;
  const int n_round = (pe - pb + ngrp - 1) / ngrp;
  auto idle_row = [&](double (&a)[6]) {
#pragma unroll
    for (int c = 0; c < 6; ++c) a[c] = (c == (i % 6)) ? 1.0 : 0.0;
  };
  auto finish = [&](double (&a)[6], bool act, int v, double* out) {
    double dii = 1.0;
#pragma unroll
    for (int c = 0; c < 6; ++c) if (act && c == i) dii = a[c];
    const bool ok = gj6_rows(a, i);
    if (!act) return;
    if (!ok) {
#pragma unroll
      for (int c = 0; c < 6; ++c) a[c] = (c == i) ? 1.0 / (fabs(dii) + lambda) : 0.0;
      if (i == 0) bad = 1;
    }
    double* o = out + 36 * (size_t)v + 6 * i;
#pragma unroll
    for (int c = 0; c < 6; ++c) o[c] = a[c];
  };
  for (int r = 0; r < n_round; ++r) {
    const int v = pb + r * ngrp + grp;
    const bool act = v < pe && i < 6;
    double a[6];
    idle_row(a);
    if (act) {
      const double* S = d.Minv + 36 * (size_t)v + 6 * i;
      double* Dv = Dm + 36 * (size_t)v + 6 * i;
#pragma unroll
      for (int c = 0; c < 6; ++c) { a[c] = S[c]; Dv[c] = a[c]; }
      const int e = d.pcr_edge[v];
      double* Lv = d.pcr_L + 36 * (size_t)v + 6 * i;
      if (e < 0) {
#pragma unroll
        for (int c = 0; c < 6; ++c) Lv[c] = 0.0;
      } else {
        const double* B = d.se_Hoff + 36 * (size_t)e;
        const bool tr = d.pcr_tr[v] != 0;
#pragma unroll
        for (int c = 0; c < 6; ++c) Lv[c] = tr ? B[6 * c + i] : B[6 * i + c];
      }
    }
    finish(a, act, v, nl > 0 ? DI[0] : d.Minv);
  }
  if (nl > 0) cl.sync();
  int cur = 0;
  for (int l = 0; l < nl; ++l) {
    const double* L = d.pcr_L + cur * N36; double* Ln = d.pcr_L + (1 - cur) * N36;
    const double* Di = DI[cur]; double* Dout = (l + 1 < nl) ? DI[1 - cur] : d.Minv;
    double *A = d.pcr_A + l * N36, *G = d.pcr_G + l * N36;
    const int s = 1 << l;
    for (int r = 0; r < n_round; ++r) {
      const int v = pb + r * ngrp + grp;
      const bool has_v = v < pe, act = has_v && i < 6;
      double* blk = sblk + 180 * (threadIdx.x >> 3);
      __syncwarp();
      if (has_v) {
        const bool hm = v - s >= pb, hp = v + s < pe, hmm = v - 2 * s >= pb;
        const double *s0 = L + 36 * (size_t)v, *s1 = Di + 36 * (size_t)(hm ? v - s : v), *s2 = L + 36 * (size_t)(hm ? v - s : v), *s3 = L + 36 * (size_t)(hp ? v + s : v),
                     *s4 = Di + 36 * (size_t)(hp ? v + s : v);
        double tmp[23];
#pragma unroll
        for (int u = 0; u < 23; ++u) {
          const int e = (threadIdx.x & 7) + 8 * u, bq = e / 36, o = e - 36 * bq;
          const double* sp = bq == 0 ? s0 : bq == 1 ? s1 : bq == 2 ? s2 : bq == 3 ? s3 : s4;
          const bool on = bq == 0 ? true : bq == 1 ? hm : bq == 2 ? hmm : hp;
          tmp[u] = (e < 180 && on) ? sp[o] : 0.0;
        }
#pragma unroll
        for (int u = 0; u < 23; ++u) { const int e = (threadIdx.x & 7) + 8 * u; if (e < 180) blk[e] = tmp[u]; }
      }
      __syncwarp();
      double dn[6];
      idle_row(dn);
      if (act) {
        const double *Lv = blk, *Dim = blk + 36, *Lm = blk + 72, *Lp = blk + 108, *Dip = blk + 144;
        double av[6] = {0, 0, 0, 0, 0, 0}, gv[6] = {0, 0, 0, 0, 0, 0}, ln[6] = {0, 0, 0, 0, 0, 0};
        double* Dv = Dm + 36 * (size_t)v + 6 * i;
#pragma unroll
        for (int c = 0; c < 6; ++c) dn[c] = Dv[c];
#pragma unroll
        for (int k = 0; k < 6; ++k) {
          const double lk = Lv[6 * i + k], lp = Lp[6 * k + i];
#pragma unroll
          for (int c = 0; c < 6; ++c) { av[c] -= lk * Dim[6 * k + c]; gv[c] -= lp * Dip[6 * k + c]; }
        }
#pragma unroll
        for (int k = 0; k < 6; ++k) {
#pragma unroll
          for (int c = 0; c < 6; ++c) { dn[c] += av[k] * Lv[6 * c + k] + gv[k] * Lp[6 * k + c]; ln[c] += av[k] * Lm[6 * k + c]; }
        }
        double* Ao = A + 36 * (size_t)v + 6 * i; double* Go = G + 36 * (size_t)v + 6 * i; double* Lo = Ln + 36 * (size_t)v + 6 * i;
#pragma unroll
        for (int c = 0; c < 6; ++c) { Ao[c] = av[c]; Go[c] = gv[c]; Lo[c] = ln[c]; Dv[c] = dn[c]; }
      }
      finish(dn, act, v, Dout);
    }
    if (l + 1 < nl) cl.sync();
    cur = 1 - cur;
  }
  if (bad) atomicAdd(d.scal + SC_BAD, 1.0);
}
template <class S, int CL>
__global__ void __cluster_dims__(CL, 1, 1) __launch_bounds__(256, 2) k_pcr_factor(S s) { VDO_PICK k_pcr_factor_body<CL>(d, s.lambda(g_), CL > 1 ? 0 : d.n_own_long, blk_); }

template <int CL>
__device__ __forceinline__ double pcr_solve_path(const BaDev& d, cg::cluster_group& cl, int pb, int pe, const double* __restrict__ r, double* __restrict__ z) {
  const int nl = pcr_num_levels(pe - pb);
  const int tid = cl.block_rank() * blockDim.x + threadIdx.x, nth = CL * blockDim.x;
  const int n_items = 6 * (pe - pb);
  const size_t N6 = 6 * (size_t)d.C, N36 = 36 * (size_t)d.C;
  const double* src = r;
  int cur = 0;
  constexpr int KP = 3;
  double pa[KP][6], pg[KP][6];
  auto fetch = [&](int l) {
    const int s = 1 << l;
    const double* A = d.pcr_A + l * N36; const double* G = d.pcr_G + l * N36;
#pragma unroll
    for (int k = 0; k < KP; ++k) {
      const int w = tid + k * nth;
      const int v = pb + w / 6, row = w % 6;
      const bool ia = w < n_items && v - s >= pb, ig = w < n_items && v + s < pe;
      const double* a = A + 36 * (size_t)v + 6 * row; const double* g = G + 36 * (size_t)v + 6 * row;
#pragma unroll
      for (int i = 0; i < 6; ++i) { pa[k][i] = ia ? a[i] : 0.0; pg[k][i] = ig ? g[i] : 0.0; }
    }
  };
  if (nl > 0) fetch(0);
  for (int l = 0; l < nl; ++l) {
    double* dst = d.pcr_b + cur * N6;
    const int s = 1 << l;
#pragma unroll
    for (int k = 0; k < KP; ++k) {
      const int w = tid + k * nth;
      if (w < n_items) {
        const int v = pb + w / 6, row = w % 6;
        double o = src[6 * (size_t)v + row];
        if (v - s >= pb) { const double* x = src + 6 * (size_t)(v - s); o += pa[k][0] * x[0] + pa[k][1] * x[1] + pa[k][2] * x[2] + pa[k][3] * x[3] + pa[k][4] * x[4] + pa[k][5] * x[5]; }
        if (v + s < pe) { const double* x = src + 6 * (size_t)(v + s); o += pg[k][0] * x[0] + pg[k][1] * x[1] + pg[k][2] * x[2] + pg[k][3] * x[3] + pg[k][4] * x[4] + pg[k][5] * x[5]; }
        dst[6 * (size_t)v + row] = o;
      }
    }
    for (int w = tid + KP * nth; w < n_items; w += nth) {
      const int v = pb + w / 6, row = w % 6;
      dst[6 * (size_t)v + row] = pcr_apply_row(v, row, pb, pe, s, d.pcr_A + l * N36, d.pcr_G + l * N36, src);
    }
    if (l + 1 < nl) fetch(l + 1);
    cl.sync();
    src = dst; cur = 1 - cur;
  }
  double rz = 0.0;
  for (int w = tid; w < n_items; w += nth) {
    const int v = pb + w / 6, row = w % 6;
    const double* m = d.Minv + 36 * (size_t)v + 6 * row; const double* x = src + 6 * (size_t)v;
    const double zz = m[0] * x[0] + m[1] * x[1] + m[2] * x[2] + m[3] * x[3] + m[4] * x[4] + m[5] * x[5];
    z[6 * (size_t)v + row] = zz;
    rz += zz * r[6 * (size_t)v + row];
  }
  return rz;
}

template <int CL>
__device__ __forceinline__ void xchg_publish_z(const BaDev& d, cg::cluster_group& cl, int path, int pb, int pe, double rz_part, int* is_last_sm, unsigned int total_ctas) {
  const int tid = cl.block_rank() * blockDim.x + threadIdx.x, nth = CL * blockDim.x;
  const int pidx = path * PCR_CL + (int)cl.block_rank();
  if (threadIdx.x == 0) d.part_rz[pidx] = rz_part;
  if (!d.xg_paths) return;
  cl.sync();
  for (int r = 0; r < d.xg_world; ++r) {
    if (r == d.xg_rank) continue;
    double* zr = d.xg_slots[r] + d.xg_off_z;
    for (int w = tid; w < 6 * (pe - pb); w += nth) { const size_t q = 6 * (size_t)pb + w; zr[q] = d.z[q]; }
    if (threadIdx.x == 0) (d.xg_slots[r] + d.xg_off_prz)[pidx] = rz_part;
  }
  __syncthreads();
  if (threadIdx.x == 0) {
    __threadfence_system();
    const unsigned int t = atomicAdd(d.ticket + 2, 1u);
    *is_last_sm = (t == total_ctas - 1) ? 1 : 0;
  }
  __syncthreads();
  if (!*is_last_sm || threadIdx.x != 0) return;
  __threadfence_system();
  d.ticket[2] = 0u;
  const unsigned long long epoch = d.xg_epoch[192] + 1ull;
  d.xg_epoch[192] = epoch;
  for (int r = 0; r < d.xg_world; ++r) { volatile unsigned long long* f = d.xg_flags[r] + 320 + d.xg_rank; *f = epoch; }
}
__device__ __forceinline__ bool xchg_wait_z(const BaDev& d) {
  const unsigned long long epoch = d.xg_epoch[192];
  volatile unsigned long long* f = d.xg_flags[d.xg_rank] + 320;
  const long long t0 = clock64();
  for (int r = 0; r < d.xg_world; ++r)
    while (f[r] < epoch) if (clock64() - t0 > 4000000000ll) return false;
  __threadfence_system();
  return true;
}

template <int CL>
__device__ __forceinline__ void k_pcg_init_body(const BaDev& d, int path0, unsigned int total_ctas, int bx) {
  __shared__ double red[32];
  __shared__ int is_last;
  cg::cluster_group cl = cg::this_cluster();
  const int path = d.own_paths[path0 + bx / CL];
  const int pb = d.path_begin[path], pe = d.path_begin[path + 1];
  const int tid = cl.block_rank() * blockDim.x + threadIdx.x, nth = CL * blockDim.x;
  for (int w = tid; w < 6 * (pe - pb); w += nth) { const size_t q = 6 * (size_t)pb + w; d.r[q] = d.rhs[q]; d.xp[q] = 0.0; }
  if (pe - pb > 1) cl.sync();
  double rz = pcr_solve_path<CL>(d, cl, pb, pe, d.r, d.z);
  for (int w = tid; w < 6 * (pe - pb); w += nth) { const size_t q = 6 * (size_t)pb + w; d.p[q] = d.z[q]; }
  rz = block_sum(rz, red);
  if (threadIdx.x == 0) red[0] = rz;
  __syncthreads();
  xchg_publish_z<CL>(d, cl, path, pb, pe, red[0], &is_last, total_ctas);
}
template <class S, int CL>
__global__ void __cluster_dims__(CL, 1, 1) __launch_bounds__(256) k_pcg_init(S s) { VDO_PICK k_pcg_init_body<CL>(d, CL > 1 ? 0 : d.n_own_long, pcg_total_ctas(d), blk_); }
__device__ __forceinline__ void k_pcg_init_fin_body(const BaDev& d) {
  __shared__ double red[33];
  __shared__ int okw;
  if (d.xg_paths) {
    if (threadIdx.x == 0) okw = xchg_wait_z(d) ? 1 : 0;
    __syncthreads();
    if (!okw) { if (threadIdx.x == 0) d.scal[SC_DONE] = 3.0; return; }
  }
  const double rz = det_sum(d.part_rz, d.n_paths * PCR_CL, red);
  if (threadIdx.x != 0) return;
  d.scal[SC_RZ] = rz; d.scal[SC_RZ0] = rz; d.scal[SC_RZ_NEW] = 0.0; d.scal[SC_PAP] = 0.0; d.scal[SC_ITERS] = 0.0; d.scal[SC_BETA] = 0.0;
  d.scal[SC_DONE] = (rz > 0.0) ? 0.0 : 1.0;
}
template <class S>
__global__ void __launch_bounds__(256) k_pcg_init_fin(S s) { VDO_PICK (void)blk_; k_pcg_init_fin_body(d); }
__global__ void __launch_bounds__(256) k_pcg_dot(BaDev d) {
  __shared__ double red[32];
  if (d.scal[SC_DONE] != 0.0) return;
  const int n = d.C * 6;
  double s = 0.0;
  for (int i = blockIdx.x * blockDim.x + threadIdx.x; i < n; i += gridDim.x * blockDim.x) s += d.p[i] * d.Ap[i];
  s = block_sum(s, red);
  if (threadIdx.x == 0) d.part_pap[blockIdx.x] = s;
}
template <bool FUSED, int CL>
__device__ __forceinline__ void k_pcg_step_a_body(const BaDev& d, const double* __restrict__ p, int path0, unsigned int total_ctas, int bx) {
  __shared__ double red[33];
  __shared__ int is_last;
  if (d.scal[SC_DONE] != 0.0) return;
  cg::cluster_group cl = cg::this_cluster();
  const double pap = det_sum(d.part_pap, d.n_part_pap, red), rz = d.scal[SC_RZ];
  const double alpha = (pap > 0.0) ? rz / pap : 0.0;
  const int path = d.own_paths[path0 + bx / CL];
  const int pb = d.path_begin[path], pe = d.path_begin[path + 1];
  const int tid = cl.block_rank() * blockDim.x + threadIdx.x, nth = CL * blockDim.x;
  for (int w = tid; w < 6 * (pe - pb); w += nth) { const size_t q = 6 * (size_t)pb + w; d.xp[q] += alpha * p[q]; d.r[q] -= alpha * d.Ap[q]; }
  if (pe - pb > 1) cl.sync();
  double rzn = pcr_solve_path<CL>(d, cl, pb, pe, d.r, d.z);
  rzn = block_sum(rzn, red);
  if (threadIdx.x == 0) red[0] = rzn;
  __syncthreads();
  xchg_publish_z<CL>(d, cl, path, pb, pe, red[0], &is_last, total_ctas);
  if (!FUSED || d.xg_paths) return;
  if (threadIdx.x == 0) {
    __threadfence();
    const unsigned int t = atomicAdd(d.ticket, 1u);
    is_last = (t == total_ctas - 1) ? 1 : 0;
  }
  __syncthreads();
  if (!is_last) return;
  __threadfence();
  const double rz_new = det_sum(d.part_rz, d.n_paths * PCR_CL, red);
  if (threadIdx.x != 0) return;
  *d.ticket = 0u;
  if (!(pap > 0.0) || !isfinite(pap) || !isfinite(rz_new)) { d.scal[SC_DONE] = 2.0; return; }
  d.scal[SC_BETA] = rz_new / rz; d.scal[SC_RZ] = rz_new; d.scal[SC_ITERS] += 1.0;
  if (rz_new <= d.scal[SC_TOL2] * d.scal[SC_RZ0]) d.scal[SC_DONE] = 1.0;
}
template <class S, bool FUSED, int CL>
__global__ void __cluster_dims__(CL, 1, 1) __launch_bounds__(256) k_pcg_step_a(S s) {
  VDO_PICK k_pcg_step_a_body<FUSED, CL>(d, s.parity() ? d.p : d.p2, CL > 1 ? 0 : d.n_own_long, pcg_total_ctas(d), blk_);
}
__device__ __forceinline__ void k_pcg_p_hpp_body(const BaDev& d, const double* __restrict__ p_in, double* __restrict__ p_out, double* __restrict__ out, int bx) {
  if (d.scal[SC_DONE] != 0.0) return;
  const double lambda = d.scal[SC_LAMBDA], beta = d.scal[SC_BETA];
  const int v = bx * (blockDim.x >> 3) + (threadIdx.x >> 3), r = threadIdx.x & 7;
  if (v >= d.C) return;
  double xv[6];
#pragma unroll
  for (int c = 0; c < 6; ++c) xv[c] = d.z[6 * (size_t)v + c] + beta * p_in[6 * (size_t)v + c];
  if (r < 6) {
    const double xr = d.z[6 * (size_t)v + r] + beta * p_in[6 * (size_t)v + r];
    p_out[6 * (size_t)v + r] = xr;
    const double* H = d.Hpp + 36 * (size_t)v + 6 * r;
    double o = lambda * xr;
#pragma unroll
    for (int c = 0; c < 6; ++c) o += H[c] * xv[c];
    for (int n = d.nbr_begin[v]; n < d.nbr_begin[v + 1]; ++n) {
      const double* B = d.se_Hoff + 36 * (size_t)d.nbr_edge[n];
      const size_t u = 6 * (size_t)d.nbr_other[n];
      double xo[6];
#pragma unroll
      for (int c = 0; c < 6; ++c) xo[c] = d.z[u + c] + beta * p_in[u + c];
      if (d.nbr_tr[n]) {
#pragma unroll
        for (int c = 0; c < 6; ++c) o += B[6 * c + r] * xo[c];
      } else {
#pragma unroll
        for (int c = 0; c < 6; ++c) o += B[6 * r + c] * xo[c];
      }
    }
    out[6 * (size_t)v + r] = d.own ? o : 0.0;
  }
  __syncwarp(0xffu << (threadIdx.x & 24));
  if (r == 0) body_vertex_transform(d, v, p_out, d.vw);
}
template <class S>
__global__ void __launch_bounds__(128) k_pcg_p_hpp(S s) { VDO_PICK k_pcg_p_hpp_body(d, s.parity() ? d.p2 : d.p, s.parity() ? d.p : d.p2, d.Ap, blk_); }

__global__ void __launch_bounds__(128) k_xchg_scatter(BaDev d, double sign, const double* __restrict__ own_part) {
  __shared__ int is_last;
  if (d.scal[SC_DONE] != 0.0) return;
  const unsigned long long epoch = *d.xg_epoch + 1ull;
  const size_t n6 = 6 * (size_t)d.C;
  const size_t slot = ((epoch & 1ull) * (size_t)d.xg_world + (size_t)d.xg_rank) * n6;
  const int v = blockIdx.x * blockDim.x + threadIdx.x;
  if (v < d.C) {
    const double* T = d.se3 + 12 * (size_t)v;
    double* a = d.acc6 + 12 * (size_t)v;
    const double F[3] = {a[0] + a[6], a[1] + a[7], a[2] + a[8]};
    const double G[3] = {2 * a[0] + a[6], 2 * a[1] + a[7], 2 * a[2] + a[8]};
    double txg[3]; cross3(T + 9, G, txg);
    const double M[3] = {a[3] + a[9] - txg[0], a[4] + a[10] - txg[1], a[5] + a[11] - txg[2]};
    double o0[3], o1[3];
    rot_t_apply(T, F, o0); rot_t_apply(T, M, o1);
    const double* op = own_part + 6 * (size_t)v;
    const double o[6] = {op[0] + sign * o0[0], op[1] + sign * o0[1], op[2] + sign * o0[2], op[3] + sign * o1[0], op[4] + sign * o1[1], op[5] + sign * o1[2]};
#pragma unroll
    for (int i = 0; i < 12; ++i) a[i] = 0.0;
    for (int r = 0; r < d.xg_world; ++r) {
      double* dst = d.xg_slots[r] + slot + 6 * (size_t)v;
#pragma unroll
      for (int i = 0; i < 6; ++i) dst[i] = o[i];
    }
  }
  __syncthreads();
  if (threadIdx.x == 0) {
    __threadfence_system();
    const unsigned int t = atomicAdd(d.ticket + 1, 1u);
    is_last = (t == gridDim.x - 1) ? 1 : 0;
  }
  __syncthreads();
  if (!is_last || threadIdx.x != 0) return;
  __threadfence_system();
  d.ticket[1] = 0u;
  *d.xg_epoch = epoch;
  for (int r = 0; r < d.xg_world; ++r) {
    volatile unsigned long long* f = d.xg_flags[r] + d.xg_rank;
    *f = epoch;
  }
}
__global__ void __launch_bounds__(128) k_xchg_reduce(BaDev d, double* __restrict__ out, const double* __restrict__ pdot) {
  __shared__ double red[32];
  __shared__ int failed;
  if (d.scal[SC_DONE] != 0.0) return;
  const unsigned long long epoch = *d.xg_epoch;
  if (threadIdx.x == 0) {
    failed = 0;
    volatile unsigned long long* f = d.xg_flags[d.xg_rank];
    const long long t0 = clock64();
    for (int r = 0; r < d.xg_world; ++r)
      while (f[r] < epoch) {
        if (clock64() - t0 > 4000000000ll) { failed = 1; break; }
      }
    __threadfence_system();
  }
  __syncthreads();
  if (failed) { if (threadIdx.x == 0 && blockIdx.x == 0) d.scal[SC_DONE] = 3.0; return; }
  const size_t n6 = 6 * (size_t)d.C;
  const double* base = d.xg_slots[d.xg_rank] + (epoch & 1ull) * (size_t)d.xg_world * n6;
  const int v = blockIdx.x * blockDim.x + threadIdx.x;
  double s = 0.0;
  if (v < d.C) {
    double o[6] = {0, 0, 0, 0, 0, 0};
    for (int r = 0; r < d.xg_world; ++r) {
      const volatile double* src = base + (size_t)r * n6 + 6 * (size_t)v;
#pragma unroll
      for (int i = 0; i < 6; ++i) o[i] += src[i];
    }
    const double* pv = pdot + 6 * (size_t)v;
#pragma unroll
    for (int i = 0; i < 6; ++i) { out[6 * (size_t)v + i] = o[i]; s += pv[i] * o[i]; }
  }
  s = block_sum(s, red);
  if (threadIdx.x == 0) d.part_pap[blockIdx.x] = s;
}

__global__ void __launch_bounds__(256) k_pcg_step_b(BaDev d) {
  __shared__ double red[33];
  if (d.scal[SC_DONE] != 0.0) return;
  const double beta = det_sum(d.part_rz, d.n_paths * PCR_CL, red) / d.scal[SC_RZ];
  const int n = d.C * 6;
  for (int i = blockIdx.x * blockDim.x + threadIdx.x; i < n; i += gridDim.x * blockDim.x) d.p[i] = d.z[i] + beta * d.p[i];
}
__global__ void __launch_bounds__(256) k_pcg_scalars(BaDev d) {
  __shared__ double red[33];
  if (d.scal[SC_DONE] != 0.0) return;
  const double tol2 = d.scal[SC_TOL2];
  const double pap = det_sum(d.part_pap, d.n_part_pap, red);
  const double rzn = det_sum(d.part_rz, d.n_paths * PCR_CL, red);
  if (threadIdx.x != 0) return;
  if (!(pap > 0.0) || !isfinite(pap) || !isfinite(rzn)) { d.scal[SC_DONE] = 2.0; return; }
  d.scal[SC_RZ] = rzn; d.scal[SC_RZ_NEW] = 0.0; d.scal[SC_PAP] = 0.0; d.scal[SC_ITERS] += 1.0;
  if (rzn <= tol2 * d.scal[SC_RZ0]) d.scal[SC_DONE] = 1.0;
}

__global__ void __launch_bounds__(256) k_pcg_scalars_x(BaDev d) {
  __shared__ double red[33];
  __shared__ int okw;
  if (d.scal[SC_DONE] != 0.0) return;
  if (threadIdx.x == 0) okw = xchg_wait_z(d) ? 1 : 0;
  __syncthreads();
  if (!okw) { if (threadIdx.x == 0) d.scal[SC_DONE] = 3.0; return; }
  const double pap = det_sum(d.part_pap, d.n_part_pap, red);
  const double rz_new = det_sum(d.part_rz, d.n_paths * PCR_CL, red);
  if (threadIdx.x != 0) return;
  const double rz = d.scal[SC_RZ];
  if (!(pap > 0.0) || !isfinite(pap) || !isfinite(rz_new)) { d.scal[SC_DONE] = 2.0; return; }
  d.scal[SC_BETA] = rz_new / rz; d.scal[SC_RZ] = rz_new; d.scal[SC_ITERS] += 1.0;
  if (rz_new <= d.scal[SC_TOL2] * d.scal[SC_RZ0]) d.scal[SC_DONE] = 1.0;
}

__device__ __forceinline__ void k_dense_init_body(const BaDev& d, double lambda, int n, int bx) {
  const int i = bx * blockDim.x + threadIdx.x;
  double* S = d.Sdense; double* rhs = S + (size_t)n * n;
  if (i < n * n) {
    const int r = i / n, c = i % n, vr = r / 6, vc = c / 6;
    double v = 0.0;
    if (vr == vc) { v = d.Hpp[36 * (size_t)vr + 6 * (r % 6) + (c % 6)]; if (r == c) v += lambda; }
    S[i] = v;
  }
  if (i < n) rhs[i] = d.bp[i];
  if (i == 0) rhs[n] = 0.0;
}
template <class S>
__global__ void __launch_bounds__(128) k_dense_init(S s) { VDO_PICK k_dense_init_body(d, s.lambda(g_), 6 * d.C, blk_); }
__device__ __forceinline__ void k_dense_se3_edges_body(const BaDev& d, int n, int bx) {
  const int e = bx * blockDim.x + threadIdx.x;
  if (e >= d.Ese || d.se_j[e] < 0) return;
  const int i = d.se_i[e], j = d.se_j[e];
  const double* H = d.se_Hoff + 36 * (size_t)e;
  double* S = d.Sdense;
  for (int r = 0; r < 6; ++r)
    for (int c = 0; c < 6; ++c) {
      if (i > j) atomicAdd(S + (size_t)(6 * i + r) * n + 6 * j + c, H[6 * r + c]);
      else atomicAdd(S + (size_t)(6 * j + c) * n + 6 * i + r, H[6 * r + c]);
    }
}
template <class S>
__global__ void __launch_bounds__(64) k_dense_se3_edges(S s) { VDO_PICK k_dense_se3_edges_body(d, 6 * d.C, blk_); }
__device__ __forceinline__ void k_dense_schur_body(const BaDev& d, int n, int bx) {
  const int k = bx * blockDim.x + threadIdx.x;
  if (k >= d.P) return;
  const int eb = d.lm_obs_begin[k], ee = d.lm_obs_begin[k + 1];
  if (ee <= eb) return;
  const double is = 1.0 / d.pt_s[k];
  const double p[3] = {d.pt[3 * (size_t)k], d.pt[3 * (size_t)k + 1], d.pt[3 * (size_t)k + 2]};
  const double bls[3] = {d.bl[3 * (size_t)k] * is, d.bl[3 * (size_t)k + 1] * is, d.bl[3 * (size_t)k + 2] * is};
  double* S = d.Sdense; double* rhs = S + (size_t)n * n;
  auto make_M = [&](int e, double* M) -> int {
    const int c = d.lm_cam[e];
    const double* T = d.se3 + 12 * (size_t)c;
    const double w[3] = {p[0] - T[9], p[1] - T[10], p[2] - T[11]};
    double Zc[3]; rot_t_apply(T, w, Zc);
    const double om = d.lm_omega[e];
    const double A[9] = {0, 2 * Zc[2], -2 * Zc[1], -2 * Zc[2], 0, 2 * Zc[0], 2 * Zc[1], -2 * Zc[0], 0};
#pragma unroll
    for (int r = 0; r < 3; ++r)
#pragma unroll
      for (int q = 0; q < 3; ++q) {
        M[3 * r + q] = -om * T[3 * q + r];
        M[9 + 3 * r + q] = om * (A[3 * r] * T[3 * q] + A[3 * r + 1] * T[3 * q + 1] + A[3 * r + 2] * T[3 * q + 2]);
      }
    return c;
  };
  for (int e1 = eb; e1 < ee; ++e1) {
    double M1[18]; const int c1 = make_M(e1, M1);
#pragma unroll
    for (int r = 0; r < 6; ++r) atomicAdd(rhs + 6 * c1 + r, -(M1[3 * r] * bls[0] + M1[3 * r + 1] * bls[1] + M1[3 * r + 2] * bls[2]));
    for (int e2 = eb; e2 < ee; ++e2) {
      double M2[18]; const int c2 = make_M(e2, M2);
      if (c2 > c1) continue;
#pragma unroll
      for (int r = 0; r < 6; ++r)
#pragma unroll
        for (int q = 0; q < 6; ++q) {
          atomicAdd(S + (size_t)(6 * c1 + r) * n + 6 * c2 + q, -is * (M1[3 * r] * M2[3 * q] + M1[3 * r + 1] * M2[3 * q + 1] + M1[3 * r + 2] * M2[3 * q + 2]));
        }
    }
  }
}
template <class S>
__global__ void __launch_bounds__(128) k_dense_schur(S s) { VDO_PICK k_dense_schur_body(d, 6 * d.C, blk_); }
__device__ __forceinline__ void k_dense_from_band_body(const BaDev& d, int n, int bx) {
  const int idx = bx * blockDim.x + threadIdx.x;
  const int W = d.band_W;
  if (idx >= d.band_n * W) return;
  const int a = idx / W, k = idx - a * W, b = a + k;
  if (b >= d.band_n) return;
  const double* m = d.band + (size_t)idx * 10;
  if (m[0] == 0.0) return;
  const int va = d.band_v0 + a, vb = d.band_v0 + b;
  const double* Ta = d.se3 + 12 * (size_t)va; const double* Tb = d.se3 + 12 * (size_t)vb;
  auto skew = [](const double* t, double* K) { K[0] = 0; K[1] = -t[2]; K[2] = t[1]; K[3] = t[2]; K[4] = 0; K[5] = -t[0]; K[6] = -t[1]; K[7] = t[0]; K[8] = 0; };
  double X[36], Kc[36], Z[36];
  {
    double tx[9]; skew(Ta + 9, tx);
    for (int r = 0; r < 3; ++r)
      for (int c = 0; c < 3; ++c) {
        const double txr = tx[3 * r] * Ta[c] + tx[3 * r + 1] * Ta[3 + c] + tx[3 * r + 2] * Ta[6 + c];
        X[6 * r + c] = -Ta[3 * r + c]; X[6 * r + 3 + c] = -2.0 * txr;
        X[6 * (r + 3) + c] = 0.0; X[6 * (r + 3) + 3 + c] = Ta[3 * r + c];
      }
  }
  {
    const double m1[3] = {m[1], m[2], m[3]};
    double m1x[9]; skew(m1, m1x);
    const double M2[9] = {m[4], m[5], m[6], m[5], m[7], m[8], m[6], m[8], m[9]};
    const double tr = m[4] + m[7] + m[9];
    for (int r = 0; r < 3; ++r)
      for (int c = 0; c < 3; ++c) {
        Kc[6 * r + c] = (r == c) ? m[0] : 0.0; Kc[6 * r + 3 + c] = 2.0 * m1x[3 * r + c];
        Kc[6 * (r + 3) + c] = 2.0 * m1x[3 * r + c]; Kc[6 * (r + 3) + 3 + c] = 4.0 * (M2[3 * r + c] - (r == c ? tr : 0.0));
      }
  }
  mat6_mul(Kc, X, Z);
  double Y[36];
  {
    double tx[9]; skew(Tb + 9, tx);
    for (int r = 0; r < 3; ++r)
      for (int c = 0; c < 3; ++c) {
        const double rtx = Tb[r] * tx[c] + Tb[3 + r] * tx[3 + c] + Tb[6 + r] * tx[6 + c];
        Y[6 * r + c] = Tb[3 * c + r]; Y[6 * r + 3 + c] = 0.0;
        Y[6 * (r + 3) + c] = -2.0 * rtx; Y[6 * (r + 3) + 3 + c] = Tb[3 * c + r];
      }
  }
  double B[36];
  mat6_mul(Y, Z, B);
  double* S = d.Sdense;
  for (int r = 0; r < 6; ++r)
    for (int c = 0; c < 6; ++c) S[(size_t)(6 * vb + r) * n + 6 * va + c] += B[6 * r + c];
}
template <class S>
__global__ void __launch_bounds__(128) k_dense_from_band(S s) { VDO_PICK k_dense_from_band_body(d, 6 * d.C, blk_); }
constexpr int DENSE_MAX = 168;
__device__ __forceinline__ void dmma_m8n8k4(double& c0, double& c1, double a, double b) {
  asm volatile("mma.sync.aligned.m8n8k4.row.col.f64.f64.f64.f64 {%0, %1}, {%2}, {%3}, {%0, %1};" : "+d"(c0), "+d"(c1) : "d"(a), "d"(b));
}
__device__ __forceinline__ void k_dense_chol_body(const BaDev& d, int n, int bx) {
  extern __shared__ double sA[];
  const int npad = (n + 7) & ~7, ld = npad + 1;
  const int tid = threadIdx.x, lane = tid & 31, warp = tid >> 5, nw = blockDim.x >> 5;
  double* S = d.Sdense; double* rhs = S + (size_t)n * n;
  __shared__ int bad;
  if (tid == 0) bad = 0;
  for (int i = tid; i < npad * npad; i += blockDim.x) {
    const int r = i / npad, c = i % npad;
    double v = 0.0;
    if (r < n && c < n) v = (c <= r) ? S[(size_t)r * n + c] : S[(size_t)c * n + r];
    else if (r == c) v = 1.0;
    sA[r * ld + c] = v;
  }
  __syncthreads();
  const int nb = npad / 8;
  for (int kb = 0; kb < nb; ++kb) {
    const int k0 = 8 * kb;
    if (warp == 0) {
      for (int j = 0; j < 8; ++j) {
        double djj = sA[(k0 + j) * ld + k0 + j];
        if (!(djj > 0.0)) { if (lane == 0) bad = 1; djj = 1.0; }
        const double l = sqrt(djj);
        __syncwarp();
        if (lane == j) sA[(k0 + j) * ld + k0 + j] = l;
// ... 196 lines not shown
    if (flag != 0.0) { xchg_release(); xg.tried = true; std::fprintf(stderr, "[vdo_b200] rank %d: peer-memory exchange unavailable, using NCCL all-reduces per PCG iteration\n", rank); return false; }
    std::vector<double*> hs(world); std::vector<unsigned long long*> hf(world);
    for (int r = 0; r < world; ++r) { hf[r] = (unsigned long long*)xg.peer[r]; hs[r] = (double*)(xg.peer[r] + XG_HDR); }
    CK(cudaMalloc(&xg.d_slots, sizeof(double*) * (size_t)world)); CK(cudaMalloc(&xg.d_flags, sizeof(unsigned long long*) * (size_t)world));
    CK(cudaMemcpyAsync(xg.d_slots, hs.data(), sizeof(double*) * (size_t)world, cudaMemcpyHostToDevice, st));
    CK(cudaMemcpyAsync(xg.d_flags, hf.data(), sizeof(unsigned long long*) * (size_t)world, cudaMemcpyHostToDevice, st));
    xg.d_epoch = (unsigned long long*)(xg.local + 8 * 256);
    CK(cudaStreamSynchronize(st));
    xg.ok = true;
    return true;
  }
  cudaStream_t st = nullptr, st2 = nullptr;
  cudaEvent_t ev_fork = nullptr, ev_join = nullptr;
  int n_launch = 0;
  cudaEvent_t ev0[4], ev1[4];
  ~CudaBackend() override {
    for (int i = 0; i < 4; ++i) { cudaEventDestroy(ev0[i]); cudaEventDestroy(ev1[i]); }
    if (gather_buf) free_(gather_buf);
    for (auto& kv : pool) cudaFree(kv.second);
    arena.destroy();
    xchg_release();
    if (comm) g_nccl.CommDestroy(comm);
    if (ev_fork) cudaEventDestroy(ev_fork);
    if (ev_join) cudaEventDestroy(ev_join);
    if (st2) cudaStreamDestroy(st2);
    if (st) cudaStreamDestroy(st);
  }
  struct PinnedArena : HostArena {
    char* raw_alloc(size_t b) override { void* p = nullptr; if (cudaHostAlloc(&p, b, cudaHostAllocDefault) != cudaSuccess) { cudaGetLastError(); p = std::malloc(b); pageable.insert(p); } return (char*)p; }
    void raw_free(char* p) override { if (pageable.count(p)) { pageable.erase(p); std::free(p); } else cudaFreeHost(p); }
    std::set<void*> pageable;
  } arena;
  HostArena& staging() override { return arena; }
  std::multimap<size_t, void*> pool;
  std::map<void*, size_t> live;
  size_t pool_bytes = 0;
  static constexpr size_t POOL_MAX = (size_t)24 << 30;
  static size_t size_class(size_t b) {
    size_t p2 = 256;
    while (p2 < b) p2 <<= 1;
    if (p2 <= 4096) return p2;
    const size_t step = p2 >> 4;
    return (b + step - 1) / step * step;
  }
  void* alloc(size_t b) override {
    b = b ? b : 8;
    const size_t cls = size_class(b);
    void* p = nullptr;
    auto it = pool.find(cls);
    if (it != pool.end()) { p = it->second; pool_bytes -= cls; pool.erase(it); }
    else CK(cudaMalloc(&p, cls));
    live[p] = cls;
    CK(cudaMemsetAsync(p, 0, b, st));
    return p;
  }
  void free_(void* p) override {
    auto it = live.find(p);
    if (it == live.end()) { cudaFree(p); return; }
    const size_t b = it->second;
    live.erase(it);
    if (pool_bytes + b <= POOL_MAX) { pool.emplace(b, p); pool_bytes += b; }
    else cudaFree(p);
  }
  void h2d_async(void* d, const void* s, size_t b) override { CK(cudaMemcpyAsync(d, s, b, cudaMemcpyHostToDevice, st)); }
  void h2d(void* d, const void* s, size_t b) override { CK(cudaMemcpyAsync(d, s, b, cudaMemcpyHostToDevice, st)); CK(cudaStreamSynchronize(st)); }
  void d2h(void* d, const void* s, size_t b) override { CK(cudaMemcpyAsync(d, s, b, cudaMemcpyDeviceToHost, st)); CK(cudaStreamSynchronize(st)); }
  void d2d(void* d, const void* s, size_t b) override { CK(cudaMemcpyAsync(d, s, b, cudaMemcpyDeviceToDevice, st)); }
  double* gather_buf = nullptr; size_t gather_cap = 0;
  void read_scalars(const double* const* src, int n, int len, double* out) override {
    if (n == 1) { d2h(out, src[0], sizeof(double) * (size_t)len); return; }
    const size_t total = (size_t)n * len;
    if (total > gather_cap) {
      if (gather_buf) free_(gather_buf);
      gather_cap = std::max(total, (size_t)1024);
      gather_buf = (double*)alloc(sizeof(double) * gather_cap);
    }
    for (int k0 = 0; k0 < n; k0 += GATHER_MAX) {
      GatherSrc g;
      g.n = std::min(GATHER_MAX, n - k0); g.len = len;
      for (int k = 0; k < g.n; ++k) g.src[k] = src[k0 + k];
      k_gather_scalars<<<1, 256, 0, st>>>(g, gather_buf + (size_t)k0 * len); ++n_launch;
    }
    d2h(out, gather_buf, sizeof(double) * total);
  }
  void zero(void* d, size_t b) override { CK(cudaMemsetAsync(d, 0, b, st)); }
  void sync() override { CK(cudaStreamSynchronize(st)); }
  int launches() const override { return n_launch; }
  void* stream() const override { return (void*)st; }
  void timer_start(int s) override { CK(cudaEventRecord(ev0[s], st)); }
  float timer_stop_ms(int s) override { float ms = 0; CK(cudaEventRecord(ev1[s], st)); CK(cudaEventSynchronize(ev1[s])); CK(cudaEventElapsedTime(&ms, ev0[s], ev1[s])); return ms; }

  static int nblk(int n, int b) { return n > 0 ? (n + b - 1) / b : 0; }
#define LAUNCH(kern, grid, block, ...)                         \
  do {                                                         \
    if ((grid) > 0) { kern<<<(grid), (block), 0, st>>>(__VA_ARGS__); ++n_launch; } \
  } while (0)

  int band_per(const BaDev& d) const { return max(1, (d.n_tiles_stat + n_sm * 3 - 1) / (n_sm * 3)); }
  int grid(const BaDev& d, int t) const {
    const int ns = d.n_tiles_stat, nc = d.n_tiles - d.n_tiles_stat;
    switch (t) {
      case BT_TILE_LIN: case BT_BACKSUB: case BT_PRE_ST: case BT_RHS_ST: return ns;
      case BT_TILE_LIN_CH: case BT_BACKSUB_CH: case BT_PRE_CH: case BT_RHS_CH: case BT_S2_CH: return nc;
      case BT_FIN_LIN: case BT_VTRANS: case BT_PRE_FIN: case BT_VERT: return nblk(d.C, 128);
      case BT_SE3: case BT_DSE3: return nblk(d.Ese, 64);
      case BT_MAXDIAG: return min(nblk(d.C * 6 + d.P, 256), n_sm * 8);
      case BT_FACTOR: return nblk(d.T, 128);
      case BT_BAND_FORM: return d.band && ns > 0 ? nblk(ns, band_per(d)) : 0;
      case BT_UPDATE: return nblk(d.C + d.P, 128);
      case BT_DINIT: return nblk(36 * d.C * d.C, 128);
      case BT_FROM_BAND: return d.band ? nblk(d.band_n * d.band_W, 128) : 0;
      case BT_SCHUR2: return d.band ? ns : 0;
      case BT_FIN_SCHUR2: return d.band ? nblk(d.C, 128) : 0;
      case BT_DSCHUR: return d.band ? 0 : nblk(d.P, 128);
      case BT_CHOL: case BT_PCG_FIN: return 1;
      case BT_PRE_BEGIN: return nblk(d.C * 36, 128);
      case BT_PCR_L: case BT_PCG_L: return d.n_own_long * PCR_CL;
      case BT_PCR_S: case BT_PCG_S: return d.n_own_paths - d.n_own_long;
      case BT_BAND_MUL: return d.band && ns > 0 ? nblk(d.band_n, 8) : 0;
      case BT_S2_ST: return d.band ? 0 : ns;
      case BT_PHPP: return nblk(d.C, 16);
      case BT_FIN_DOT: return nblk(d.C, 128);
    }
    return 0;
  }
  static int threads(int t) {
    switch (t) {
      case BT_TILE_LIN: case BT_TILE_LIN_CH: case BT_BAND_FORM: case BT_BACKSUB: case BT_BACKSUB_CH: case BT_SCHUR2: case BT_PRE_ST: case BT_PRE_CH:
      case BT_RHS_ST: case BT_RHS_CH: case BT_S2_ST: case BT_S2_CH: return VDO_TILE_L;
      case BT_SE3: case BT_DSE3: return 64;
      case BT_MAXDIAG: case BT_CHOL: case BT_PCR_L: case BT_PCR_S: case BT_PCG_L: case BT_PCG_S: case BT_PCG_FIN: case BT_BAND_MUL: return 256;
      case BT_FIN_DOT: return 1024;
    }
    return 128;
  }
  static size_t smem(const BaDev& d, int t) {
    switch (t) {
      case BT_TILE_LIN: return smem_lin(false, d.capE_st, d.capV_st, 0);
      case BT_TILE_LIN_CH: return smem_lin(true, d.capE_ch, d.capV_ch, d.capH_ch);
      case BT_PRE_ST: return smem_pre(false, d.capE_st);
      case BT_PRE_CH: return smem_pre(true, d.capE_ch);
      case BT_SCHUR2: case BT_RHS_ST: case BT_S2_ST: case BT_BACKSUB: return smem_sch2(false, d.capE_st, d.capV_st, 1);
      case BT_RHS_CH: case BT_S2_CH: case BT_BACKSUB_CH: return smem_sch2(true, d.capE_ch, d.capV_ch, d.capH_ch);
      case BT_BAND_FORM: return smem_band(d.capE_st);
      case BT_CHOL: { const size_t npad = (6 * (size_t)d.C + 7) & ~(size_t)7; return sizeof(double) * npad * (npad + 1); }
    }
    return 0;
  }
  template <class S> static void optin() {
    BaDev m;
    m.capE_st = m.capE_ch = VDO_TILE_E; m.capV_st = m.capV_ch = m.capH_ch = 255; m.C = DENSE_MAX / 6;
    auto set = [&](const void* f, int t) { if (smem(m, t) > 48 * 1024) CK(cudaFuncSetAttribute(f, cudaFuncAttributeMaxDynamicSharedMemorySize, (int)smem(m, t))); };
    set((const void*)k_tile_lin<S, false, true>, BT_TILE_LIN); set((const void*)k_tile_lin<S, false, false>, BT_TILE_LIN);
    set((const void*)k_tile_lin<S, true, true>, BT_TILE_LIN_CH); set((const void*)k_tile_lin<S, true, false>, BT_TILE_LIN_CH);
    set((const void*)k_tile_precond<S, false>, BT_PRE_ST); set((const void*)k_tile_precond<S, true>, BT_PRE_CH);
    set((const void*)k_tile_schur2<S, false, 0>, BT_RHS_ST); set((const void*)k_tile_schur2<S, false, 1>, BT_S2_ST);
    set((const void*)k_tile_schur2<S, true, 0>, BT_RHS_CH); set((const void*)k_tile_schur2<S, true, 1>, BT_S2_CH);
    set((const void*)k_tile_schur2<S, false, 2>, BT_BACKSUB); set((const void*)k_tile_schur2<S, true, 2>, BT_BACKSUB_CH);
    set((const void*)k_band_form<S>, BT_BAND_FORM);
    set((const void*)k_dense_chol<S>, BT_CHOL);
  }

  One one(const BaDev& d, double lambda = 0.0, int reortho = 0, int parity = 0) const { return One{d, lambda, reortho, parity, band_per(d)}; }
  Many many(int bit) const {
    Many s{bdev, nullptr, bit, 0};
    bool live = false;
    for (int f : tflags) live |= (f & (bit == BATCH_PCG ? BATCH_PCG : ~0)) != 0;
    if (!live) s.B.n = 0;
    return s;
  }
  static void set_parity(One& s, int par) { s.par = par; }
  static void set_parity(Many& s, int par) { s.par = par; }
  int ctas(const One& s, int t) const { return grid(s.d, t); }
  int ctas(const Many& s, int t) const { return s.B.n ? bfirst[(size_t)t * (s.B.n + 1) + s.B.n] : 0; }
  size_t smem_of(const One& s, int t) const { return smem(s.d, t); }
  size_t smem_of(const Many&, int t) const { return bsmem[t]; }
  static One with_table(One s, int) { return s; }
  static Many with_table(Many s, int t) { s.f = s.B.first + (size_t)t * (s.B.n + 1); return s; }
  template <class F> void each(const One& s, F f) { f(s.d); }
  template <class F> void each(const Many& s, F f) { for (size_t i = 0; i < tab.size(); ++i) if (tflags[i] & s.bit) f(*bds_[tab[i]]); }
  template <class S, class... P, class... A> void run(void (*k)(S, P...), const S& s, int t, cudaStream_t stream, A... a) {
    const int n = ctas(s, t);
    if (n > 0) { k<<<n, threads(t), smem_of(s, t), stream>>>(with_table(s, t), a...); ++n_launch; }
  }

  template <class S> void lin_tiles(const S& s, bool write, int part) {
    if (part != 1) run(write ? k_tile_lin<S, false, true> : k_tile_lin<S, false, false>, s, BT_TILE_LIN, st);
    if (part != 0) run(write ? k_tile_lin<S, true, true> : k_tile_lin<S, true, false>, s, BT_TILE_LIN_CH, st);
  }
  template <class S> void max_diag(const S& s) {
    each(s, [&](const BaDev& d) { zero(d.scal + SC_MAXDIAG, sizeof(double)); });
    run(k_max_diagonal<S>, s, BT_MAXDIAG, st);
  }
  template <class S> void band_form_(const S& s) {
    each(s, [&](const BaDev& d) { if (d.band && d.n_tiles_stat > 0) zero(d.band, sizeof(double) * 10 * (size_t)d.band_n * d.band_W); });
    run(k_band_form<S>, s, BT_BAND_FORM, st);
  }
  template <class S> void dense_solve_(const S& s) {
    run(k_dense_init<S>, s, BT_DINIT, st);
    run(k_dense_se3_edges<S>, s, BT_DSE3, st);
    band_form_(s);
    run(k_dense_from_band<S>, s, BT_FROM_BAND, st);
    run(k_tile_schur2<S, false, 0>, s, BT_SCHUR2, st);
    run(k_tile_finalize_schur2<S, FIN_DENSE_RHS>, s, BT_FIN_SCHUR2, st);
    run(k_dense_schur<S>, s, BT_DSCHUR, st);
    run(k_dense_chol<S>, s, BT_CHOL, st);
    each(s, [&](const BaDev& d) { d2d(d.scal + SC_DENSE, d.Sdense + 36 * (size_t)d.C * d.C + 6 * (size_t)d.C, sizeof(double)); });
  }
  template <class S> void precond_tiles(const S& s) {
    run(k_tile_precond<S, false>, s, BT_PRE_ST, st);
    run(k_tile_precond<S, true>, s, BT_PRE_CH, st);
    run(k_tile_finalize_precond<S>, s, BT_PRE_FIN, st);
  }
  template <class S> void pcr_factor(const S& s) {
    run(k_pcr_factor<S, PCR_CL>, s, BT_PCR_L, st);
    run(k_pcr_factor<S, 1>, s, BT_PCR_S, st);
  }
  template <class S> void rhs_tiles(const S& s) {
    run(k_tile_schur2<S, false, 0>, s, BT_RHS_ST, st);
    run(k_tile_schur2<S, true, 0>, s, BT_RHS_CH, st);
  }
  template <class S> void schur_product(const S& s, int part, cudaStream_t chain_stream) {
    if (part != 1) { run(k_band_mul<S>, s, BT_BAND_MUL, st); run(k_tile_schur2<S, false, 1>, s, BT_S2_ST, st); }
    if (part != 0) run(k_tile_schur2<S, true, 1>, s, BT_S2_CH, chain_stream);
  }
  template <class S> void backsub_tiles(const S& s) {
    run(k_tile_schur2<S, false, 2>, s, BT_BACKSUB, st);
    run(k_tile_schur2<S, true, 2>, s, BT_BACKSUB_CH, st);
  }
  template <bool FUSED, class S> void step_a(const S& s) {
    bool fork = ctas(s, BT_PCG_L) > 0 && ctas(s, BT_PCG_S) > 0;
    if constexpr (std::is_same<S, One>::value) fork &= !s.d.xg_paths;
    if (fork) { CK(cudaEventRecord(ev_fork, st)); CK(cudaStreamWaitEvent(st2, ev_fork, 0)); }
    run(k_pcg_step_a<S, FUSED, PCR_CL>, s, BT_PCG_L, st);
    run(k_pcg_step_a<S, FUSED, 1>, s, BT_PCG_S, fork ? st2 : st);
    if (fork) { CK(cudaEventRecord(ev_join, st2)); CK(cudaStreamWaitEvent(st, ev_join, 0)); }
  }
  template <class S> void pcg_init_(const S& s) {
    each(s, [&](const BaDev& d) {
      zero(d.scal + SC_PAP, 6 * sizeof(double));
      if (d.xg_paths) zero(d.xp, 48 * (size_t)d.C);
    });
    if constexpr (std::is_same<S, Many>::value) {
      if (s.B.n) { k_batch_scalars<<<nblk(s.B.n, 128), 128, 0, st>>>(s.B, s.bit); ++n_launch; }
      each(s, [&](const BaDev& d) { set_cache.erase(d.scal); });
    }
    run(k_pcg_init<S, PCR_CL>, s, BT_PCG_L, st);
    run(k_pcg_init<S, 1>, s, BT_PCG_S, st);
    run(k_pcg_init_fin<S>, s, BT_PCG_FIN, st);
  }
  template <class S> void pcg_fused(S s, int b, bool peer) {
    set_parity(s, b & 1);
    run(k_pcg_p_hpp<S>, s, BT_PHPP, st);
    CK(cudaEventRecord(ev_fork, st)); CK(cudaStreamWaitEvent(st2, ev_fork, 0));
    schur_product(s, -1, st2);
    CK(cudaEventRecord(ev_join, st2)); CK(cudaStreamWaitEvent(st, ev_join, 0));
    if constexpr (std::is_same<S, One>::value) {
      const BaDev& d = s.d;
      const double* p_out = (b & 1) ? d.p : d.p2;
      if (peer) {
        LAUNCH(k_xchg_scatter, nblk(d.C, 128), 128, d, -1.0, (const double*)d.Ap);
        LAUNCH(k_xchg_reduce, nblk(d.C, 128), 128, d, d.Ap, p_out);
      }
    }
    if (!peer) run(k_tile_finalize_ap_dot<S>, s, BT_FIN_DOT, st);
    step_a<true>(s);
    if constexpr (std::is_same<S, One>::value) { if (s.d.xg_paths) LAUNCH(k_pcg_scalars_x, 1, 256, s.d); }
  }
  template <class F> cudaGraphExec_t capture(F body, int* launches) {
    cudaGraph_t g = nullptr; cudaGraphExec_t ge = nullptr;
    const int before = n_launch;
    CK(cudaStreamBeginCapture(st, cudaStreamCaptureModeThreadLocal));
    body();
    CK(cudaStreamEndCapture(st, &g));
    CK(cudaGraphInstantiate(&ge, g, 0));
    cudaGraphDestroy(g);
    *launches = n_launch - before;
    n_launch = before;
    return ge;
  }

  void lin_tracklets(BaDev& d, bool write) override {
    if (d.tiled) { lin_tiles(one(d), write, -1); return; }
    if (write) { LAUNCH(k_lin_static<true>, nblk(d.Tstat, 256), 256, d); LAUNCH(k_lin_tracklets<true>, nblk(d.T - d.Tstat, 128), 128, d); }
    else { LAUNCH(k_lin_static<false>, nblk(d.Tstat, 256), 256, d); LAUNCH(k_lin_tracklets<false>, nblk(d.T - d.Tstat, 128), 128, d); }
  }
  void lin_vertex_obs(BaDev& d) override {
    if (d.tiled) { run(k_tile_finalize_lin<One>, one(d), BT_FIN_LIN, st); return; }
    auto k = k_vertex_sym<0, true>; LAUNCH(k, d.n_obs_chunks, 128, d);
  }
  void lin_vertex_ter(BaDev& d) override { if (d.tiled) return; auto k = k_vertex_sym<0, false>; LAUNCH(k, d.n_ter_chunks, 128, d); }
  void lin_se3_edges(BaDev& d, bool write) override { run(write ? k_lin_se3_edges<One, true> : k_lin_se3_edges<One, false>, one(d), BT_SE3, st); }
  void max_diagonal(BaDev& d) override { max_diag(one(d)); }
  int band_max_width() const override { return 32; }
  void band_form(BaDev& d) override { band_form_(one(d)); }
  void factor_landmarks(BaDev& d, double lambda) override { run(k_factor_landmarks<One>, one(d, lambda), BT_FACTOR, st); }
  void precond_begin(BaDev& d, double lambda) override { run(k_precond_begin<One>, one(d, lambda), BT_PRE_BEGIN, st); }
  void precond_vertex_obs(BaDev& d) override {
    if (d.tiled) { precond_tiles(one(d)); return; }
    auto k = k_vertex_sym<1, true>; LAUNCH(k, d.n_obs_chunks, 128, d);
  }
  void precond_vertex_ter(BaDev& d) override { if (d.tiled) return; auto k = k_vertex_sym<1, false>; LAUNCH(k, d.n_ter_chunks, 128, d); }
  void precond_factor(BaDev& d, double lambda) override { pcr_factor(one(d, lambda)); }
  void schur_landmarks(BaDev& d, int mode, const double* v) override {
    if (d.tiled) {
      if (mode == 0) rhs_tiles(one(d)); else if (mode == 1) schur_product(one(d), -1, st); else backsub_tiles(one(d));
      return;
    }
    const int g = nblk((d.T - d.Tstat) * 8, 128), gs = nblk(d.Tstat, 256);
    if (mode == 0) { LAUNCH(k_schur_static<0>, gs, 256, d, d.zl); LAUNCH(k_schur_chains8<0>, g, 128, d, v, d.zl); }
    else if (mode == 1) { LAUNCH(k_schur_static<1>, gs, 256, d, d.zl); LAUNCH(k_schur_chains8<1>, g, 128, d, v, d.zl); }
    else { LAUNCH(k_schur_static<2>, gs, 256, d, d.xl); LAUNCH(k_schur_chains8<2>, g, 128, d, v, d.xl); }
  }
  void schur_landmarks_part(BaDev& d, int mode, const double* v, int part) override {
    if (d.tiled) { schur_product(one(d), part, st); return; }
    const int g = nblk((d.T - d.Tstat) * 8, 128), gs = nblk(d.Tstat, 256);
    if (part == 0) LAUNCH(k_schur_static<1>, gs, 256, d, d.zl); else LAUNCH(k_schur_chains8<1>, g, 128, d, v, d.zl);
    (void)mode;
  }
  void lin_tracklets_part(BaDev& d, bool write, int part) override {
    if (d.tiled) { lin_tiles(one(d), true, part); return; }
    (void)write;
    if (part == 0) LAUNCH(k_lin_static<true>, nblk(d.Tstat, 256), 256, d); else LAUNCH(k_lin_tracklets<true>, nblk(d.T - d.Tstat, 128), 128, d);
  }
  void schur_vertex_obs(BaDev& d, double sign, double* out) override {
    if (d.tiled) { run(out == d.Ap ? k_tile_finalize_schur2<One, FIN_AP> : k_tile_finalize_schur2<One, FIN_RHS>, one(d), BT_VERT, st); return; }
    LAUNCH(k_schur_vertex<true>, d.n_obs_chunks, 128, d, sign, out, out == d.Ap ? 1 : 0);
  }
  void schur_vertex_ter(BaDev& d, double sign, double* out) override {
    if (d.tiled) return;
    LAUNCH(k_schur_vertex<false>, d.n_ter_chunks, 128, d, sign, out, out == d.Ap ? 1 : 0);
  }
  std::map<const double*, std::pair<double, double>> set_cache;
  std::pair<double, double>& cached(const BaDev& d) { return set_cache.try_emplace(d.scal, -1.0, -1.0).first->second; }
  void set_scalars(BaDev& d, double lambda, double tol2) {
    std::pair<double, double>& c = cached(d);
    if (lambda != c.first || tol2 != c.second) { LAUNCH(k_set_scalars, 1, 1, d, lambda, tol2); c = {lambda, tol2}; }
  }
  void vertex_transform(BaDev& d, const double* v) override { run(k_vertex_transform<One>, one(d), BT_VTRANS, st, v); }
  void hpp_mul(BaDev& d, double lambda, const double* x, double* out) override { const double t2 = cached(d).second; set_scalars(d, lambda, t2 < 0 ? 0.0 : t2); LAUNCH(k_hpp_mul, nblk(d.C, 128), 128, d, x, out); }
  void pcg_init(BaDev& d) override { pcg_init_(one(d)); }
  void pcg_dot_pAp(BaDev& d) override { LAUNCH(k_pcg_dot, d.n_part_pap, 256, d); }
  void pcg_step(BaDev& d, double tol2) override {
    set_scalars(d, cached(d).first, tol2);
    step_a<false>(one(d, 0.0, 0, 1));
    LAUNCH(k_pcg_step_b, min(nblk(d.C * 6, 256), n_sm), 256, d);
    LAUNCH(k_pcg_scalars, 1, 256, d);
  }
  std::map<std::pair<const void*, int>, cudaGraphExec_t> graphs;
  void pcg_iterate(BaDev& d, double lambda, double tol2, int n) override {
    bool peer = false;
    if (world > 1) {
      peer = d.tiled && d.xg_paths && xg.ok;
      if (!peer) { BaBackend::pcg_iterate(d, lambda, tol2, n); return; }
    }
    set_scalars(d, lambda, tol2);
    auto key = std::make_pair((const void*)d.scal, n);
    auto it = graphs.find(key);
    if (it == graphs.end()) {
      cudaGraphExec_t ge = capture([&] {
        const int gch = nblk((d.T - d.Tstat) * 8, 128), gst = nblk(d.Tstat, 256);
        for (int b = 0; b < n; ++b) {
          if (d.tiled) { pcg_fused(one(d), b, peer); continue; }
          LAUNCH(k_hpp_mul, nblk(d.C, 128), 128, d, (const double*)d.p, d.Ap);
          CK(cudaEventRecord(ev_fork, st)); CK(cudaStreamWaitEvent(st2, ev_fork, 0));
          LAUNCH(k_schur_static<1>, gst, 256, d, d.zl);
          if (gch > 0) { k_schur_chains8<1><<<gch, 128, 0, st2>>>(d, (const double*)d.p, d.zl); ++n_launch; }
          CK(cudaEventRecord(ev_join, st2)); CK(cudaStreamWaitEvent(st, ev_join, 0));
          CK(cudaEventRecord(ev_fork, st)); CK(cudaStreamWaitEvent(st2, ev_fork, 0));
          schur_vertex_obs(d, -1.0, d.Ap);
          if (d.n_ter_chunks > 0) { k_schur_vertex<false><<<d.n_ter_chunks, 128, 0, st2>>>(d, -1.0, d.Ap, 1); ++n_launch; }
          CK(cudaEventRecord(ev_join, st2)); CK(cudaStreamWaitEvent(st, ev_join, 0));
          LAUNCH(k_pcg_dot, d.n_part_pap, 256, d);
          step_a<false>(one(d, 0.0, 0, 1));
          LAUNCH(k_pcg_step_b, min(nblk(d.C * 6, 256), n_sm), 256, d);
          LAUNCH(k_pcg_scalars, 1, 256, d);
        }
      }, &per_batch[key]);
      it = graphs.emplace(key, ge).first;
    }
    CK(cudaGraphLaunch(it->second, st));
    n_launch += per_batch[key];
  }
  std::map<std::pair<const void*, int>, int> per_batch;
  bool shard_paths(BaDev& d) override {
    if (world <= 1 || !d.tiled || d.n_paths < world) return false;
    if (!xchg_setup(d.C, d.n_paths)) return false;
    d.xg_rank = rank; d.xg_world = world; d.xg_slots = xg.d_slots; d.xg_flags = xg.d_flags; d.xg_epoch = xg.d_epoch;
    d.xg_paths = 1; d.xg_off_z = xg.off_z; d.xg_off_prz = xg.off_prz;
    d.z = (double*)(xg.local + XG_HDR) + xg.off_z;
    d.part_rz = (double*)(xg.local + XG_HDR) + xg.off_prz;
    return true;
  }
  void drop_graphs() {
    for (auto& kv : graphs) cudaGraphExecDestroy(kv.second);
    graphs.clear(); per_batch.clear();
  }
  void release(BaDev& d) override {
    for (auto it = graphs.begin(); it != graphs.end();) {
      if (it->first.first == (const void*)d.scal) { cudaGraphExecDestroy(it->second); per_batch.erase(it->first); it = graphs.erase(it); } else ++it;
    }
    set_cache.erase(d.scal);
  }
  int dense_capacity() const override { return DENSE_MAX; }
  void dense_solve(BaDev& d, double lambda) override { dense_solve_(one(d, lambda)); }
  void apply_update(BaDev& d, double lambda, bool reortho) override { run(k_apply_update<One>, one(d, lambda, reortho ? 1 : 0), BT_UPDATE, st); }

  BatchDev bdev{};
  std::vector<int> tab;
  std::vector<int> tflags;
  std::vector<int> wflags, wrt; std::vector<double> wlam, wtol2;
  std::vector<int> bfirst;
  size_t bsmem[BT_N] = {};
  void* bbuf = nullptr;
  static size_t align16(size_t b) { return (b + 15) & ~(size_t)15; }
  cudaGraphExec_t bpcg = nullptr; int bpcg_n = 0, bpcg_launches = 0;
  void batch_begin(BaDev* const* all, int n_all) override {
    BaBackend::batch_begin(all, n_all);
    tab.clear();
    for (int pass = 0; pass < 2; ++pass) {
      std::vector<int> ks;
      for (int k = 0; k < n_all; ++k) {
        const BaDev& d = *all[k];
        if (pass == 0 ? d.Sdense != nullptr : (!d.Sdense && d.tiled && !d.xg_paths && world == 1)) ks.push_back(k);
      }
      if (ks.size() >= 2) tab.insert(tab.end(), ks.begin(), ks.end());
    }
    const int n = (int)tab.size();
    tflags.assign(n, 0); wflags.assign(n, 0); wrt.assign(n, 0); wlam.assign(n, 0.0); wtol2.assign(n, 0.0);
    if (!n) return;
    bfirst.assign((size_t)BT_N * (n + 1), 0);
    std::vector<int> per(n, 1);
    for (int t = 0; t < BT_N; ++t) bsmem[t] = 0;
    for (int k = 0; k < n; ++k) {
      const BaDev& d = *all[tab[k]];
      const bool dn = d.Sdense != nullptr;
      per[k] = band_per(d);
      for (int t = 0; t < BT_N; ++t) {
        const int g = (t >= BT_PRE_BEGIN ? dn : (t >= BT_DINIT && !dn)) ? 0 : grid(d, t);
        bfirst[(size_t)t * (n + 1) + k + 1] = bfirst[(size_t)t * (n + 1) + k] + g;
        if (g > 0) bsmem[t] = std::max(bsmem[t], smem(d, t));
      }
    }
    const size_t o_first = align16(sizeof(BaDev) * (size_t)n), o_per = o_first + align16(sizeof(int) * bfirst.size()), o_flags = o_per + align16(sizeof(int) * n),
                 o_rt = o_flags + align16(sizeof(int) * n), o_lam = o_rt + align16(sizeof(int) * n), o_tol = o_lam + align16(sizeof(double) * (size_t)n),
                 total = o_tol + sizeof(double) * (size_t)n;
    std::vector<char> h(o_flags, 0);
    for (int k = 0; k < n; ++k) std::memcpy(h.data() + sizeof(BaDev) * (size_t)k, all[tab[k]], sizeof(BaDev));
    std::memcpy(h.data() + o_first, bfirst.data(), sizeof(int) * bfirst.size());
    std::memcpy(h.data() + o_per, per.data(), sizeof(int) * n);
    bbuf = alloc(total);
    h2d(bbuf, h.data(), h.size());
    char* b = (char*)bbuf;
    bdev = BatchDev{(const BaDev*)b, (const int*)(b + o_first), (const int*)(b + o_per), (int*)(b + o_flags), (double*)(b + o_lam), (int*)(b + o_rt), (double*)(b + o_tol), n};
  }
  void batch_end() override {
    if (bpcg) { CK(cudaGraphExecDestroy(bpcg)); bpcg = nullptr; }
    if (bbuf) free_(bbuf);
    bbuf = nullptr; bdev = BatchDev{}; tab.clear(); tflags.clear();
    BaBackend::batch_end();
  }
  void batch_set(const int* flags, const double* lambda, const int* reortho, const double* tol2) override {
    BaBackend::batch_set(flags, lambda, reortho, tol2);
    const int n = (int)tab.size();
    bool on = false, pcg = false;
    for (int i = 0; i < n; ++i) { tflags[i] = bflags_[tab[i]]; bflags_[tab[i]] = 0; on |= tflags[i] != 0; pcg |= (tflags[i] & BATCH_PCG) != 0; }
    const int mask = pcg ? ~0 : ~BATCH_PCG;
    bool stale = false;
    for (int i = 0; i < n; ++i) {
      const int k = tab[i];
      stale |= ((tflags[i] ^ wflags[i]) & mask) != 0 || lambda[k] != wlam[i] || reortho[k] != wrt[i] || tol2[k] != wtol2[i];
    }
    if (!on || !stale) return;
    for (int k0 = 0; k0 < n; k0 += BATCH_PARAMS_MAX) {
      BatchParams p;
      p.n0 = k0; p.n = std::min(BATCH_PARAMS_MAX, n - k0);
      for (int i = 0; i < p.n; ++i) {
        const int j = k0 + i, k = tab[j];
        p.flags[i] = wflags[j] = tflags[j]; p.lambda[i] = wlam[j] = lambda[k]; p.reortho[i] = wrt[j] = reortho[k]; p.tol2[i] = wtol2[j] = tol2[k];
      }
      k_batch_params<<<1, BATCH_PARAMS_MAX, 0, st>>>(bdev, p); ++n_launch;
    }
  }
  void lin_tracklets_batch(int bit, bool write) override { lin_tiles(many(bit), write, -1); BaBackend::lin_tracklets_batch(bit, write); }
  void lin_vertex_batch(int bit) override { run(k_tile_finalize_lin<Many>, many(bit), BT_FIN_LIN, st); BaBackend::lin_vertex_batch(bit); }
  void lin_se3_edges_batch(int bit, bool write) override {
    run(write ? k_lin_se3_edges<Many, true> : k_lin_se3_edges<Many, false>, many(bit), BT_SE3, st);
    BaBackend::lin_se3_edges_batch(bit, write);
  }
  void max_diagonal_batch(int bit) override { max_diag(many(bit)); BaBackend::max_diagonal_batch(bit); }
  void factor_landmarks_batch(int bit) override { run(k_factor_landmarks<Many>, many(bit), BT_FACTOR, st); BaBackend::factor_landmarks_batch(bit); }
  void dense_solve_batch(int bit) override { dense_solve_(many(bit)); BaBackend::dense_solve_batch(bit); }
  void back_substitute_batch(int bit) override {
    run(k_vertex_transform<Many>, many(bit), BT_VTRANS, st, (const double*)nullptr);
    backsub_tiles(many(bit));
    BaBackend::back_substitute_batch(bit);
  }
  void apply_update_batch(int bit) override { run(k_apply_update<Many>, many(bit), BT_UPDATE, st); BaBackend::apply_update_batch(bit); }
  void precondition_batch(int bit) override {
    const Many s = many(bit);
    each(s, [&](const BaDev& d) { zero(d.scal + SC_BAD, sizeof(double)); });
    run(k_precond_begin<Many>, s, BT_PRE_BEGIN, st);
    precond_tiles(s);
    pcr_factor(s);
    band_form_(s);
    BaBackend::precondition_batch(bit);
  }
  void schur_rhs_batch(int bit) override {
    const Many s = many(bit);
    rhs_tiles(s);
    each(s, [&](const BaDev& d) { d2d(d.rhs, d.bp, 48 * (size_t)d.C); });
    run(k_tile_finalize_schur2<Many, FIN_RHS>, s, BT_VERT, st);
    BaBackend::schur_rhs_batch(bit);
  }
  void pcg_init_batch(int bit) override { pcg_init_(many(bit)); BaBackend::pcg_init_batch(bit); }
  void pcg_iterate_batch(int bit, int n) override {
    if (many(bit).B.n) {
      if (bpcg && bpcg_n != n) { CK(cudaGraphExecDestroy(bpcg)); bpcg = nullptr; }
      if (!bpcg) {
        bpcg = capture([&] { for (int b = 0; b < n; ++b) pcg_fused(many(bit), b, false); }, &bpcg_launches);
        bpcg_n = n;
      }
      CK(cudaGraphLaunch(bpcg, st));
      n_launch += bpcg_launches;
    }
    BaBackend::pcg_iterate_batch(bit, n);
  }
};

BaBackend* make_backend(int device, char* err, size_t errlen) {
  int n = 0;
  cudaError_t e = cudaGetDeviceCount(&n);
  if (e != cudaSuccess || n <= 0) { std::snprintf(err, errlen, "no CUDA device (%s); libvdo_b200 has no CPU path", cudaGetErrorString(e)); return nullptr; }
  if (device < 0 || device >= n) { std::snprintf(err, errlen, "device %d out of range (%d visible)", device, n); return nullptr; }
  cudaDeviceProp prop;
  if ((e = cudaGetDeviceProperties(&prop, device)) != cudaSuccess) { std::snprintf(err, errlen, "cudaGetDeviceProperties: %s", cudaGetErrorString(e)); return nullptr; }
  if (prop.major != 9 || prop.minor != 0) { std::snprintf(err, errlen, "device %d is sm_%d%d; this build carries sm_90a code only", device, prop.major, prop.minor); return nullptr; }
  if ((e = cudaSetDevice(device)) != cudaSuccess) { std::snprintf(err, errlen, "cudaSetDevice: %s", cudaGetErrorString(e)); return nullptr; }
  CudaBackend::optin<One>();
  CudaBackend::optin<Many>();
  CudaBackend* b = new CudaBackend;
  b->dev = device;
  b->n_sm = prop.multiProcessorCount;
  if ((e = cudaStreamCreateWithFlags(&b->st, cudaStreamNonBlocking)) != cudaSuccess) { std::snprintf(err, errlen, "cudaStreamCreate: %s", cudaGetErrorString(e)); delete b; return nullptr; }
  for (int i = 0; i < 4; ++i) { cudaEventCreate(&b->ev0[i]); cudaEventCreate(&b->ev1[i]); }
  cudaStreamCreateWithFlags(&b->st2, cudaStreamNonBlocking);
  cudaEventCreateWithFlags(&b->ev_fork, cudaEventDisableTiming);
  cudaEventCreateWithFlags(&b->ev_join, cudaEventDisableTiming);
  return b;
}

}

struct vdo_ctx;
namespace vdo {
BaBackend* ctx_backend(vdo_ctx* c);
void ctx_device(vdo_ctx* c, int* dev, int* n_sm) {
  const CudaBackend* be = static_cast<const CudaBackend*>(ctx_backend(c));
  *dev = be->dev; *n_sm = be->n_sm;
}
}
extern "C" int vdo_nccl_unique_id(char* out128) {
  if (!out128) return -2;
  if (!vdo::g_nccl.load()) return -5;
  ncclUniqueId id;
  if (vdo::g_nccl.GetUniqueId(&id) != ncclSuccess) return -5;
  std::memcpy(out128, &id, sizeof id);
  return 0;
}
extern "C" int vdo_ctx_init_comm(vdo_ctx* ctx, int rank, int world, const char* id128) {
  vdo::CudaBackend* be = static_cast<vdo::CudaBackend*>(vdo::ctx_backend(ctx));
  if (!be || !id128 || world < 1 || rank < 0 || rank >= world) return -2;
  if (world == 1) { be->rank = 0; be->world = 1; return 0; }
  if (!vdo::g_nccl.load()) return -5;
  ncclUniqueId id;
  std::memcpy(&id, id128, sizeof id);
  cudaSetDevice(be->dev);
  ncclResult_t r = vdo::g_nccl.CommInitRank(&be->comm, world, id, rank);
  if (r != ncclSuccess) { std::fprintf(stderr, "[vdo_b200] ncclCommInitRank failed: %s\n", vdo::g_nccl.GetErrorString ? vdo::g_nccl.GetErrorString(r) : "?"); return -5; }
  be->rank = rank; be->world = world;
  return 0;
}
```

### vdo_slam_b200/csrc/ba_types.h

```cpp
#pragma once
#include <stdint.h>
#include <stddef.h>
#include <cstdio>
#include <cstdlib>
#include <vector>

#define VDO_CHUNK 512
#define VDO_TILE_L 256
#define VDO_TILE_E 768
#define VDO_PCR_SHORT 32
#define VDO_SEG 64
#define VDO_SEG2 15

namespace vdo {

struct Chunk { int v, begin, end, pad; };
struct Tile { int k0, k1, e0, e1, t0, t1, os0, os1, ts0, ts1, qo0, qo1, qt0, qt1, vs0, nv; };
struct Seg { int v, begin, n, pad; };

struct BaDev {
  int own = 1;
  int Tstat = 0;
  int C = 0, P = 0, T = 0, Eobs = 0, Eter = 0, Ese = 0, n_obs_chunks = 0, n_ter_chunks = 0, n_nbr = 0;
  double *se3 = 0, *pt = 0, *se3_bk = 0, *pt_bk = 0, *se3_init = 0, *pt_init = 0;
  int* tk_begin = 0;
  int* lm_obs_begin = 0; int* lm_cam = 0; double* lm_z = 0; uint8_t* lm_cls = 0; double* lm_omega = 0;
  int* tk_h = 0; uint8_t* tk_cls = 0; double* tk_omega = 0;
  int* vm_pt = 0; double* vm_z = 0; uint8_t* vm_cls = 0; double* vm_omega = 0; Chunk* obs_chunks = 0;
  int* hm_p1 = 0; uint8_t* hm_cls = 0; double* hm_omega = 0; Chunk* ter_chunks = 0;
  int *se_i = 0, *se_j = 0; double *se_Z = 0, *se_w = 0, *se_delta = 0, *se_Hoff = 0;
  int *nbr_begin = 0, *nbr_edge = 0, *nbr_other = 0; uint8_t* nbr_tr = 0;
  double *Hpp = 0, *bp = 0, *hll = 0, *bl = 0, *pt_s = 0, *Minv = 0;
  double *pt_g = 0, *tk_gamma = 0;
  int n_paths = 0, pcr_levels = 0;
  int* path_begin = 0;
  int* path_of = 0;
  int* pcr_edge = 0; uint8_t* pcr_tr = 0;
  double *pcr_D = 0, *pcr_L = 0, *pcr_Dinv = 0;
  double *pcr_A = 0, *pcr_G = 0;
  double *pcr_b = 0;
  double *xp = 0, *r = 0, *z = 0, *p = 0, *Ap = 0, *rhs = 0;
  double* band = 0; int band_W = 0, band_v0 = 0, band_n = 0;
  double* Sdense = 0;
  double* p2 = 0;
  unsigned int* ticket = 0;
  int xg_rank = 0, xg_world = 1;
  double** xg_slots = 0;
  unsigned long long** xg_flags = 0;
  unsigned long long* xg_epoch = 0;
  int xg_paths = 0;
  size_t xg_off_z = 0, xg_off_prz = 0;
  int* own_paths = 0; int n_own_paths = 0;
  int n_own_long = 0;
  double *zl = 0, *xl = 0;
  double *vw = 0;
  double *obs_cls_w = 0, *obs_cls_d = 0, *ter_cls_w = 0, *ter_cls_d = 0;
  int tiled = 0, n_tiles_stat = 0, n_tiles = 0, n_osegs = 0, n_tsegs = 0;
  int capE_st = 16, capE_ch = 16;
  Tile* tiles = 0; Seg* osegs = 0; Seg* tsegs = 0; Seg* osegs2 = 0; Seg* tsegs2 = 0;
  uint32_t* ob_ps = 0;
  int* tile_verts = 0;
  uint8_t* lm_cslot = 0;
  uint8_t* tk_hslot = 0;
  int capV_st = 1, capV_ch = 1, capH_ch = 1;
  uint16_t* ob_perm = 0;
  uint16_t* tr_perm = 0;
  uint8_t* lm_lml = 0;
  double* pt_Q = 0;
  double *accO = 0, *accT = 0;
  double* acc6 = 0;
  double* vh = 0;
  double* scal = 0;
  double *part_pap = 0, *part_rz = 0;
  int n_part_pap = 0, n_part_rz = 0;
};

enum { SC_CHI2 = 0, SC_SCALE = 1, SC_MAXDIAG = 2, SC_PAP = 3, SC_RZ = 4, SC_RZ_NEW = 5, SC_RZ0 = 6, SC_DONE = 7, SC_ITERS = 8, SC_BAD = 9,
       SC_LAMBDA = 10, SC_TOL2 = 11, SC_BETA = 12, SC_DENSE = 13, SC_N = 16 };

struct HostArena {
  struct Block { char* p; size_t cap, used; };
  std::vector<Block> blocks;
  int users = 0;
  virtual ~HostArena() {}
  virtual char* raw_alloc(size_t bytes) = 0;
  virtual void raw_free(char* p) = 0;
  void* take(size_t bytes) {
    bytes = (bytes + 255) & ~(size_t)255;
    for (Block& b : blocks) if (b.cap - b.used >= bytes) { void* r = b.p + b.used; b.used += bytes; return r; }
    const size_t cap = bytes > ((size_t)64 << 20) ? bytes : ((size_t)64 << 20);
    if (std::getenv("VDO_ARENA_TRACE")) std::fprintf(stderr, "[vdo_b200] staging arena: new block of %zu MB for a request of %zu bytes (%zu blocks, users %d)\n", cap >> 20, bytes, blocks.size(), users);
    Block nb{raw_alloc(cap), cap, bytes};
    blocks.push_back(nb);
    return nb.p;
  }
  void acquire() { ++users; }
  void release() {
    if (--users > 0) return;
    users = 0;
    if (blocks.size() > 1) {
      size_t total = 0;
      for (Block& b : blocks) { total += b.cap; raw_free(b.p); }
      blocks.clear();
      blocks.push_back(Block{raw_alloc(total), total, 0});
    }
    for (Block& b : blocks) b.used = 0;
  }
  void destroy() { for (Block& b : blocks) raw_free(b.p); blocks.clear(); }
};

struct BaBackend {
  virtual ~BaBackend() {}
  int rank = 0, world = 1;
  virtual void allreduce_sum(double* buf, size_t n) { (void)buf; (void)n; }
  virtual void allreduce_max(double* buf, size_t n) { (void)buf; (void)n; }
  virtual void* alloc(size_t bytes) = 0;
  virtual void free_(void* p) = 0;
  virtual void h2d(void* dst, const void* src, size_t bytes) = 0;
  virtual void h2d_async(void* dst, const void* src, size_t bytes) { h2d(dst, src, bytes); }
  virtual HostArena& staging() = 0;
  virtual void d2h(void* dst, const void* src, size_t bytes) = 0;
  virtual void read_scalars(const double* const* src, int n, int len, double* out) {
    for (int k = 0; k < n; ++k) d2h(out + (size_t)k * len, src[k], sizeof(double) * (size_t)len);
  }
  virtual void d2d(void* dst, const void* src, size_t bytes) = 0;
  virtual void zero(void* dst, size_t bytes) = 0;
  virtual void sync() = 0;
  virtual int launches() const = 0;
  virtual void* stream() const = 0;
  virtual void timer_start(int slot) = 0;
  virtual float timer_stop_ms(int slot) = 0;

  virtual void lin_tracklets(BaDev& d, bool write) = 0;
  virtual void lin_vertex_obs(BaDev& d) = 0;
  virtual void lin_vertex_ter(BaDev& d) = 0;
  virtual void lin_se3_edges(BaDev& d, bool write) = 0;
  virtual void max_diagonal(BaDev& d) = 0;
  virtual void factor_landmarks(BaDev& d, double lambda) = 0;
  virtual void precond_begin(BaDev& d, double lambda) = 0;
  virtual void precond_vertex_obs(BaDev& d) = 0;
  virtual void precond_vertex_ter(BaDev& d) = 0;
  virtual void precond_factor(BaDev& d, double lambda) = 0;
  virtual void schur_landmarks(BaDev& d, int mode, const double* v) = 0;
  virtual void schur_landmarks_part(BaDev& d, int mode, const double* v, int part) { (void)part; schur_landmarks(d, mode, v); }
  virtual void lin_tracklets_part(BaDev& d, bool write, int part) { (void)part; lin_tracklets(d, write); }
  virtual void schur_vertex_obs(BaDev& d, double sign, double* out) = 0;
  virtual void schur_vertex_ter(BaDev& d, double sign, double* out) = 0;
  virtual void vertex_transform(BaDev& d, const double* v) = 0;
  virtual void hpp_mul(BaDev& d, double lambda, const double* v, double* out) = 0;
  virtual void pcg_init(BaDev& d) = 0;
  virtual void pcg_dot_pAp(BaDev& d) = 0;
  virtual void pcg_step(BaDev& d, double tol2) = 0;
  virtual void pcg_iterate(BaDev& d, double lambda, double tol2, int n) {
    for (int b = 0; b < n; ++b) {
      hpp_mul(d, lambda, d.p, d.Ap);
      schur_landmarks(d, 1, d.p);
      schur_vertex_obs(d, -1.0, d.Ap);
      schur_vertex_ter(d, -1.0, d.Ap);
      allreduce_sum(d.Ap, 6 * (size_t)d.C);
      pcg_dot_pAp(d);
      pcg_step(d, tol2);
    }
  }
  virtual void release(BaDev& d) { (void)d; }
  virtual int dense_capacity() const { return 0; }
  virtual int band_max_width() const { return 0; }
  virtual void band_form(BaDev& d) { (void)d; }
  virtual void dense_solve(BaDev& d, double lambda) { (void)d; (void)lambda; }
  virtual bool shard_paths(BaDev& d) { (void)d; return false; }
  virtual void apply_update(BaDev& d, double lambda, bool reorthogonalize) = 0;

  enum { BATCH_LIN = 1, BATCH_MAXDIAG = 2, BATCH_TRIAL = 4, BATCH_DENSE = 8, BATCH_PCG = 16 };
  virtual void batch_begin(BaDev* const* ds, int n) {
    bds_.assign(ds, ds + n); bflags_.assign(n, 0); blam_.assign(n, 0.0); brt_.assign(n, 0); btol2_.assign(n, 0.0);
  }
  virtual void batch_end() { bds_.clear(); }
  virtual void batch_set(const int* flags, const double* lambda, const int* reortho, const double* tol2) {
    for (size_t k = 0; k < bds_.size(); ++k) { bflags_[k] = flags[k]; blam_[k] = lambda[k]; brt_[k] = reortho[k]; btol2_[k] = tol2[k]; }
  }
  virtual void lin_tracklets_batch(int bit, bool write) { for (size_t k = 0; k < bds_.size(); ++k) if (bflags_[k] & bit) lin_tracklets(*bds_[k], write); }
  virtual void lin_vertex_batch(int bit) { for (size_t k = 0; k < bds_.size(); ++k) if (bflags_[k] & bit) { lin_vertex_obs(*bds_[k]); lin_vertex_ter(*bds_[k]); } }
  virtual void lin_se3_edges_batch(int bit, bool write) { for (size_t k = 0; k < bds_.size(); ++k) if (bflags_[k] & bit) lin_se3_edges(*bds_[k], write); }
  virtual void max_diagonal_batch(int bit) { for (size_t k = 0; k < bds_.size(); ++k) if (bflags_[k] & bit) max_diagonal(*bds_[k]); }
  virtual void factor_landmarks_batch(int bit) { for (size_t k = 0; k < bds_.size(); ++k) if (bflags_[k] & bit) factor_landmarks(*bds_[k], blam_[k]); }
  virtual void dense_solve_batch(int bit) { for (size_t k = 0; k < bds_.size(); ++k) if (bflags_[k] & bit) dense_solve(*bds_[k], blam_[k]); }
  virtual void back_substitute_batch(int bit) {
    for (size_t k = 0; k < bds_.size(); ++k) if (bflags_[k] & bit) { vertex_transform(*bds_[k], bds_[k]->xp); schur_landmarks(*bds_[k], 2, bds_[k]->xp); }
  }
  virtual void apply_update_batch(int bit) { for (size_t k = 0; k < bds_.size(); ++k) if (bflags_[k] & bit) apply_update(*bds_[k], blam_[k], brt_[k] != 0); }
  virtual void precondition_batch(int bit) {
    for (size_t k = 0; k < bds_.size(); ++k) {
      if (!(bflags_[k] & bit)) continue;
      BaDev& d = *bds_[k];
      zero(d.scal + SC_BAD, sizeof(double));
      precond_begin(d, blam_[k]); precond_vertex_obs(d); precond_vertex_ter(d);
      allreduce_sum(d.Minv, 36 * (size_t)d.C);
      precond_factor(d, blam_[k]);
      if (d.band) band_form(d);
    }
  }
  virtual void schur_rhs_batch(int bit) {
    for (size_t k = 0; k < bds_.size(); ++k) {
      if (!(bflags_[k] & bit)) continue;
      BaDev& d = *bds_[k];
      schur_landmarks(d, 0, nullptr);
      if (d.own) d2d(d.rhs, d.bp, 48 * (size_t)d.C); else zero(d.rhs, 48 * (size_t)d.C);
      schur_vertex_obs(d, -1.0, d.rhs); schur_vertex_ter(d, -1.0, d.rhs);
    }
  }
  virtual void pcg_init_batch(int bit) { for (size_t k = 0; k < bds_.size(); ++k) if (bflags_[k] & bit) pcg_init(*bds_[k]); }
  virtual void pcg_iterate_batch(int bit, int n) {
    for (size_t k = 0; k < bds_.size(); ++k) if (bflags_[k] & bit) pcg_iterate(*bds_[k], blam_[k], btol2_[k], n);
  }
 protected:
  std::vector<BaDev*> bds_;
  std::vector<int> bflags_, brt_;
  std::vector<double> blam_, btol2_;
};

BaBackend* make_backend(int device, char* err, size_t errlen);

}
```

Before: 186.6.

## Replace parallel cyclic reduction preconditioner with block cyclic reduction

Result: faster. 204.4 (median of 6 runs) (+9.6%).

```diff
diff --git a/vdo_slam_b200/csrc/ba_bodies.cuh b/vdo_slam_b200/csrc/ba_bodies.cuh
--- a/vdo_slam_b200/csrc/ba_bodies.cuh
+++ b/vdo_slam_b200/csrc/ba_bodies.cuh
@@ -459,18 +459,6 @@
   }
   for (int i = 0; i < 6; ++i) bn[6 * (size_t)v + i] = o[i];
 }
-VDO_HD double pcr_apply_row(int v, int row, int pb, int pe, int s, const double* A, const double* G, const double* b) {
-  double o = b[6 * (size_t)v + row];
-  if (v - s >= pb) {
-    const double* a = A + 36 * (size_t)v + 6 * row; const double* x = b + 6 * (size_t)(v - s);
-    o += a[0] * x[0] + a[1] * x[1] + a[2] * x[2] + a[3] * x[3] + a[4] * x[4] + a[5] * x[5];
-  }
-  if (v + s < pe) {
-    const double* g = G + 36 * (size_t)v + 6 * row; const double* x = b + 6 * (size_t)(v + s);
-    o += g[0] * x[0] + g[1] * x[1] + g[2] * x[2] + g[3] * x[3] + g[4] * x[4] + g[5] * x[5];
-  }
-  return o;
-}
 VDO_HD int pcr_num_levels(int m) { int l = 0; while ((1 << l) < m) ++l; return l; }
 VDO_HD void mul6(const double* M, const double* x, double* o) {
 #pragma unroll
diff --git a/vdo_slam_b200/csrc/ba_driver.cpp b/vdo_slam_b200/csrc/ba_driver.cpp
--- a/vdo_slam_b200/csrc/ba_driver.cpp
+++ b/vdo_slam_b200/csrc/ba_driver.cpp
@@ -308,7 +308,7 @@
 struct BaGraph::Chunked { std::vector<int> vm_pt; std::vector<double> vm_z; std::vector<uint8_t> vm_cls; std::vector<Chunk> obs_chunks;
                           std::vector<int> hm_p1; std::vector<uint8_t> hm_cls; std::vector<Chunk> ter_chunks; };
 struct BaGraph::Se3Edges { std::vector<int> i, j; std::vector<double> Z, w, d; std::vector<int> nbr_begin, nbr_edge, nbr_other;
-                           std::vector<uint8_t> nbr_tr; std::vector<int> path_of, pcr_edge; std::vector<uint8_t> pcr_tr; int pcr_levels = 0; };
+                           std::vector<uint8_t> nbr_tr; std::vector<int> path_of, pcr_edge; std::vector<uint8_t> pcr_tr; int max_len = 1; };
 struct BaGraph::Solvers { bool dense = false; int band_W = 0, band_v0 = 0, band_n = 0; };
 int BaGraph::order_tracklets(int NT, const Lap& lap, Tracklets& tk) {
   const int C = n_se3_, P = n_pt_, Eo = (int)ob_w_.size(), Et = (int)te_w_.size(), rank = be_->rank, world = be_->world;
@@ -580,10 +580,9 @@
   }
   const int n_paths = (int)path_begin.size() - 1;
   se.path_of.resize(C); se.pcr_edge.assign(C, -1); se.pcr_tr.assign(C, 0);
-  int max_len = 1;
   for (int pth = 0; pth < n_paths; ++pth) {
     for (int v = path_begin[pth]; v < path_begin[pth + 1]; ++v) se.path_of[v] = pth;
-    max_len = std::max(max_len, path_begin[pth + 1] - path_begin[pth]);
+    se.max_len = std::max(se.max_len, path_begin[pth + 1] - path_begin[pth]);
   }
   for (int e = Ep; e < Ese; ++e) {
     int a = se.i[e], b = se.j[e];
@@ -591,7 +590,6 @@
     if (b == a + 1) { se.pcr_edge[b] = e; se.pcr_tr[b] = 1; }
     else if (a == b + 1) { se.pcr_edge[a] = e; se.pcr_tr[a] = 0; }
   }
-  while ((1 << se.pcr_levels) < max_len) ++se.pcr_levels;
   return se;
 }
 void BaGraph::states(const Tracklets& tk, int NT, HostBuf<double>& se3, HostBuf<double>& pt) {
@@ -671,11 +669,13 @@
   d.Hpp = dalloc<double>(42 * (size_t)C); d.bp = d.Hpp + 36 * (size_t)C; d.hll = dalloc<double>(P); d.bl = dalloc<double>(3 * (size_t)P);
   d.pt_s = dalloc<double>(P); d.Minv = dalloc<double>(36 * (size_t)C);
   d.pt_g = dalloc<double>(P); d.tk_gamma = dalloc<double>(P);
-  d.n_paths = n_paths; d.pcr_levels = se.pcr_levels;
+  d.n_paths = n_paths;
   d.path_begin = upload(path_begin); d.path_of = upload(se.path_of); d.pcr_edge = upload(se.pcr_edge); d.pcr_tr = upload(se.pcr_tr);
-  d.pcr_D = dalloc<double>(72 * (size_t)C); d.pcr_L = dalloc<double>(72 * (size_t)C); d.pcr_Dinv = dalloc<double>(36 * (size_t)C);
-  d.pcr_A = dalloc<double>(36 * (size_t)C * std::max(se.pcr_levels, 1)); d.pcr_G = dalloc<double>(36 * (size_t)C * std::max(se.pcr_levels, 1));
-  d.pcr_b = dalloc<double>(12 * (size_t)C);
+  size_t nDL = 0, nAG = 0, nb = 0;
+  be_->precond_blocks(C, se.max_len, nDL, nAG, nb);
+  d.pcr_D = dalloc<double>(36 * nDL); d.pcr_L = dalloc<double>(36 * nDL); d.pcr_Dinv = dalloc<double>(36 * (size_t)C);
+  d.pcr_A = dalloc<double>(36 * nAG); d.pcr_G = dalloc<double>(36 * nAG);
+  d.pcr_b = dalloc<double>(6 * nb);
   d.xp = dalloc<double>(6 * (size_t)C); d.r = dalloc<double>(6 * (size_t)C); d.z = dalloc<double>(6 * (size_t)C);
   d.p = dalloc<double>(6 * (size_t)C); d.Ap = dalloc<double>(6 * (size_t)C); d.rhs = dalloc<double>(6 * (size_t)C);
   d.p2 = dalloc<double>(6 * (size_t)C); d.ticket = dalloc<unsigned int>(4);
diff --git a/vdo_slam_b200/csrc/ba_kernels.cu b/vdo_slam_b200/csrc/ba_kernels.cu
--- a/vdo_slam_b200/csrc/ba_kernels.cu
+++ b/vdo_slam_b200/csrc/ba_kernels.cu
@@ -355,199 +355,271 @@
   if (v < d.C) body_hpp_mul(d, v, lambda, x, out);
 }
 
+template <class S> constexpr int bcr_ctas_per_sm() { return std::is_same<S, One>::value ? 4 : 2; }
+__device__ __forceinline__ int bcr_survivors(int n, int l) { return (n - 1 + (2 << l)) >> (l + 1); }
+__device__ __forceinline__ int bcr_eliminated(int n, int l) { return (n - 1 + (1 << l)) >> (l + 1); }
 
 __device__ __forceinline__ bool gj6_rows(double (&a)[6], int i) {
   bool ok = true;
 #pragma unroll
   for (int k = 0; k < 6; ++k) {
-    double rk[6];
-#pragma unroll
-    for (int c = 0; c < 6; ++c) rk[c] = __shfl_sync(0xffffffffu, a[c], k, 8);
-    const double piv = rk[k];
+    const double piv = __shfl_sync(0xffffffffu, a[k], k, 8);
     if (!(piv > 0.0) || !(piv < 1e300)) ok = false;
-    const double pinv = 1.0 / piv;
-    if (i == k) {
-#pragma unroll
-      for (int c = 0; c < 6; ++c) a[c] = (c == k) ? pinv : rk[c] * pinv;
-    } else {
-      const double f = a[k] * pinv;
-#pragma unroll
-      for (int c = 0; c < 6; ++c) a[c] = (c == k) ? -f : a[c] - f * rk[c];
+    const double pinv = 1.0 / piv, f = a[k] * pinv;
+#pragma unroll
+    for (int c = 0; c < 6; ++c) {
+      const double rk = __shfl_sync(0xffffffffu, a[c], k, 8);
+      if (i == k) a[c] = (c == k) ? pinv : rk * pinv;
+      else a[c] = (c == k) ? -f : a[c] - f * rk;
     }
   }
   return ok;
+}
+__device__ __forceinline__ bool inv6_rows(double (&a)[6], const double* src, bool act, int i, double lambda) {
+  double dii = 1.0;
+#pragma unroll
+  for (int c = 0; c < 6; ++c) {
+    a[c] = act ? src[c] : (c == (i % 6) ? 1.0 : 0.0);
+    if (c == i) dii = a[c];
+  }
+  const bool ok = gj6_rows(a, i);
+  if (!ok) {
+#pragma unroll
+    for (int c = 0; c < 6; ++c) a[c] = (c == i) ? 1.0 / (fabs(dii) + lambda) : 0.0;
+  }
+  return ok || !act;
 }
 template <int CL>
 __device__ __forceinline__ void k_pcr_factor_body(const BaDev& d, double lambda, int path0, int bx) {
   cg::cluster_group cl = cg::this_cluster();
   const int path = d.own_paths[path0 + bx / CL];
-  const int pb = d.path_begin[path], pe = d.path_begin[path + 1];
-  const int nl = pcr_num_levels(pe - pb);
-  const int tid = cl.block_rank() * blockDim.x + threadIdx.x, nth = CL * blockDim.x;
-  const int grp = tid >> 3, i = tid & 7, ngrp = nth >> 3;
-  const size_t N36 = 36 * (size_t)d.C;
+  const int pb = d.path_begin[path], n = d.path_begin[path + 1] - pb;
+  const int nl = pcr_num_levels(n), rank = (int)cl.block_rank(), i = threadIdx.x & 7;
   __shared__ double sblk[32 * 180];
-  double* const Dm = d.pcr_D;
-  double* const DI[2] = {d.pcr_Dinv, d.pcr_D + N36};
+  double* const blk = sblk + 180 * (threadIdx.x >> 3);
   int bad = 0;
-  const int n_round = (pe - pb + ngrp - 1) / ngrp;
-  auto idle_row = [&](double (&a)[6]) {
-#pragma unroll
-    for (int c = 0; c < 6; ++c) a[c] = (c == (i % 6)) ? 1.0 : 0.0;
-  };
-  auto finish = [&](double (&a)[6], bool act, int v, double* out) {
-    double dii = 1.0;
-#pragma unroll
-    for (int c = 0; c < 6; ++c) if (act && c == i) dii = a[c];
-    const bool ok = gj6_rows(a, i);
-    if (!act) return;
-    if (!ok) {
-#pragma unroll
-      for (int c = 0; c < 6; ++c) a[c] = (c == i) ? 1.0 / (fabs(dii) + lambda) : 0.0;
-      if (i == 0) bad = 1;
-    }
-    double* o = out + 36 * (size_t)v + 6 * i;
-#pragma unroll
-    for (int c = 0; c < 6; ++c) o[c] = a[c];
-  };
-  for (int r = 0; r < n_round; ++r) {
-    const int v = pb + r * ngrp + grp;
-    const bool act = v < pe && i < 6;
-    double a[6];
-    idle_row(a);
-    if (act) {
-      const double* S = d.Minv + 36 * (size_t)v + 6 * i;
-      double* Dv = Dm + 36 * (size_t)v + 6 * i;
-#pragma unroll
-      for (int c = 0; c < 6; ++c) { a[c] = S[c]; Dv[c] = a[c]; }
-      const int e = d.pcr_edge[v];
-      double* Lv = d.pcr_L + 36 * (size_t)v + 6 * i;
-      if (e < 0) {
-#pragma unroll
-        for (int c = 0; c < 6; ++c) Lv[c] = 0.0;
-      } else {
-        const double* B = d.se_Hoff + 36 * (size_t)e;
-        const bool tr = d.pcr_tr[v] != 0;
-#pragma unroll
-        for (int c = 0; c < 6; ++c) Lv[c] = tr ? B[6 * c + i] : B[6 * i + c];
-      }
-    }
-    finish(a, act, v, nl > 0 ? DI[0] : d.Minv);
-  }
-  if (nl > 0) cl.sync();
-  int cur = 0;
+  size_t off = 2 * (size_t)pb;
+#pragma unroll 1
   for (int l = 0; l < nl; ++l) {
-    const double* L = d.pcr_L + cur * N36; double* Ln = d.pcr_L + (1 - cur) * N36;
-    const double* Di = DI[cur]; double* Dout = (l + 1 < nl) ? DI[1 - cur] : d.Minv;
-    double *A = d.pcr_A + l * N36, *G = d.pcr_G + l * N36;
-    const int s = 1 << l;
-    for (int r = 0; r < n_round; ++r) {
-      const int v = pb + r * ngrp + grp;
-      const bool has_v = v < pe, act = has_v && i < 6;
-      double* blk = sblk + 180 * (threadIdx.x >> 3);
+    const int s = 1 << l, cnt = bcr_survivors(n, l);
+    const bool wide = cnt > 32;
+    if (!wide && rank != 0) break;
+    const int g0 = (wide ? rank * (int)blockDim.x + (int)threadIdx.x : (int)threadIdx.x) >> 3, ng = wide ? CL * 32 : 32;
+    const double* const Ds = l ? d.pcr_D : d.Minv;
+#pragma unroll 1
+    for (int k0 = 0; k0 < cnt; k0 += ng) {
+      const int k = k0 + g0, j = 2 * s * k, v = pb + j;
+      const bool has = k < cnt, hm = has && k > 0, hp = has && j + s < n, act = has && i < 6;
       __syncwarp();
-      if (has_v) {
-        const bool hm = v - s >= pb, hp = v + s < pe, hmm = v - 2 * s >= pb;
-        const double *s0 = L + 36 * (size_t)v, *s1 = Di + 36 * (size_t)(hm ? v - s : v), *s2 = L + 36 * (size_t)(hm ? v - s : v), *s3 = L + 36 * (size_t)(hp ? v + s : v),
-                     *s4 = Di + 36 * (size_t)(hp ? v + s : v);
-        double tmp[23];
-#pragma unroll
-        for (int u = 0; u < 23; ++u) {
-          const int e = (threadIdx.x & 7) + 8 * u, bq = e / 36, o = e - 36 * bq;
-          const double* sp = bq == 0 ? s0 : bq == 1 ? s1 : bq == 2 ? s2 : bq == 3 ? s3 : s4;
-          const bool on = bq == 0 ? true : bq == 1 ? hm : bq == 2 ? hmm : hp;
-          tmp[u] = (e < 180 && on) ? sp[o] : 0.0;
+      if (has) {
+#pragma unroll 1
+        for (int q = 0; q < 5; ++q) {
+          const int w = q == 0 ? v : q <= 2 ? v - s : v + s;
+          const double* src = nullptr;
+          bool tr = false;
+          if (q <= 2 ? hm : hp) {
+            if (q == 1 || q == 4) src = Ds + 36 * (size_t)w;
+            else if (l) src = d.pcr_L + 36 * (size_t)w;
+            else if (const int ed = d.pcr_edge[w]; ed >= 0) { src = d.se_Hoff + 36 * (size_t)ed; tr = d.pcr_tr[w] != 0; }
+          }
+#pragma unroll
+          for (int t = 0; t < 5; ++t) {
+            const int o = i + 8 * t;
+            if (o < 36) blk[36 * q + o] = src ? src[tr ? 6 * (o % 6) + o / 6 : o] : 0.0;
+          }
         }
-#pragma unroll
-        for (int u = 0; u < 23; ++u) { const int e = (threadIdx.x & 7) + 8 * u; if (e < 180) blk[e] = tmp[u]; }
       }
       __syncwarp();
-      double dn[6];
-      idle_row(dn);
+      double a[6];
+      inv6_rows(a, blk + 36 + 6 * i, act && hm, i, lambda);
+      if (act) {
+#pragma unroll
+        for (int c = 0; c < 6; ++c) blk[36 + 6 * i + c] = a[c];
+      }
+      __syncwarp();
+      const bool ok = inv6_rows(a, blk + 144 + 6 * i, act && hp, i, lambda);
+      if (act && hp) {
+        double* o = d.pcr_Dinv + 36 * (size_t)(v + s) + 6 * i;
+#pragma unroll
+        for (int c = 0; c < 6; ++c) { blk[144 + 6 * i + c] = a[c]; o[c] = a[c]; }
+        if (!ok && i == 0) bad = 1;
+      }
+      __syncwarp();
       if (act) {
         const double *Lv = blk, *Dim = blk + 36, *Lm = blk + 72, *Lp = blk + 108, *Dip = blk + 144;
-        double av[6] = {0, 0, 0, 0, 0, 0}, gv[6] = {0, 0, 0, 0, 0, 0}, ln[6] = {0, 0, 0, 0, 0, 0};
-        double* Dv = Dm + 36 * (size_t)v + 6 * i;
-#pragma unroll
-        for (int c = 0; c < 6; ++c) dn[c] = Dv[c];
-#pragma unroll
-        for (int k = 0; k < 6; ++k) {
-          const double lk = Lv[6 * i + k], lp = Lp[6 * k + i];
-#pragma unroll
-          for (int c = 0; c < 6; ++c) { av[c] -= lk * Dim[6 * k + c]; gv[c] -= lp * Dip[6 * k + c]; }
+        double av[6] = {0, 0, 0, 0, 0, 0}, t[6] = {0, 0, 0, 0, 0, 0};
+#pragma unroll
+        for (int kk = 0; kk < 6; ++kk) {
+          const double lk = Lv[6 * i + kk];
+#pragma unroll
+          for (int c = 0; c < 6; ++c) av[c] -= lk * Dim[6 * kk + c];
         }
 #pragma unroll
-        for (int k = 0; k < 6; ++k) {
-#pragma unroll
-          for (int c = 0; c < 6; ++c) { dn[c] += av[k] * Lv[6 * c + k] + gv[k] * Lp[6 * k + c]; ln[c] += av[k] * Lm[6 * k + c]; }
+        for (int kk = 0; kk < 6; ++kk) {
+#pragma unroll
+          for (int c = 0; c < 6; ++c) t[c] += av[kk] * Lm[6 * kk + c];
         }
-        double* Ao = A + 36 * (size_t)v + 6 * i; double* Go = G + 36 * (size_t)v + 6 * i; double* Lo = Ln + 36 * (size_t)v + 6 * i;
-#pragma unroll
-        for (int c = 0; c < 6; ++c) { Ao[c] = av[c]; Go[c] = gv[c]; Lo[c] = ln[c]; Dv[c] = dn[c]; }
-      }
-      finish(dn, act, v, Dout);
-    }
-    if (l + 1 < nl) cl.sync();
-    cur = 1 - cur;
+        double* Ao = d.pcr_A + 36 * (off + k) + 6 * i; double* Lo = d.pcr_L + 36 * (size_t)v + 6 * i;
+#pragma unroll
+        for (int c = 0; c < 6; ++c) { Ao[c] = av[c]; Lo[c] = t[c]; t[c] = Ds[36 * (size_t)v + 6 * i + c]; }
+#pragma unroll
+        for (int kk = 0; kk < 6; ++kk) {
+#pragma unroll
+          for (int c = 0; c < 6; ++c) t[c] += av[kk] * Lv[6 * c + kk];
+        }
+#pragma unroll
+        for (int c = 0; c < 6; ++c) av[c] = 0.0;
+#pragma unroll
+        for (int kk = 0; kk < 6; ++kk) {
+          const double lp = Lp[6 * kk + i];
+#pragma unroll
+          for (int c = 0; c < 6; ++c) av[c] -= lp * Dip[6 * kk + c];
+        }
+#pragma unroll
+        for (int kk = 0; kk < 6; ++kk) {
+#pragma unroll
+          for (int c = 0; c < 6; ++c) t[c] += av[kk] * Lp[6 * kk + c];
+        }
+        double* Go = d.pcr_G + 36 * (off + k) + 6 * i; double* Do = d.pcr_D + 36 * (size_t)v + 6 * i;
+#pragma unroll
+        for (int c = 0; c < 6; ++c) { Go[c] = av[c]; Do[c] = t[c]; }
+      }
+    }
+    if (wide) cl.sync(); else __syncthreads();
+    off += cnt;
+  }
+  if (rank == 0 && threadIdx.x < 32) {
+    double a[6];
+    const bool act = threadIdx.x < 6;
+    const bool ok = inv6_rows(a, (nl ? d.pcr_D : d.Minv) + 36 * (size_t)pb + 6 * i, act, i, lambda);
+    if (act) {
+#pragma unroll
+      for (int c = 0; c < 6; ++c) d.pcr_Dinv[36 * (size_t)pb + 6 * i + c] = a[c];
+      if (!ok && i == 0) bad = 1;
+    }
   }
   if (bad) atomicAdd(d.scal + SC_BAD, 1.0);
 }
 template <class S, int CL>
-__global__ void __cluster_dims__(CL, 1, 1) __launch_bounds__(256, 2) k_pcr_factor(S s) { VDO_PICK k_pcr_factor_body<CL>(d, s.lambda(g_), CL > 1 ? 0 : d.n_own_long, blk_); }
-
+__global__ void __cluster_dims__(CL, 1, 1) __launch_bounds__(256, bcr_ctas_per_sm<S>()) k_pcr_factor(S s) { VDO_PICK k_pcr_factor_body<CL>(d, s.lambda(g_), CL > 1 ? 0 : d.n_own_long, blk_); }
+
+__device__ __forceinline__ double dot6(const double* a, const double* x) { return a[0] * x[0] + a[1] * x[1] + a[2] * x[2] + a[3] * x[3] + a[4] * x[4] + a[5] * x[5]; }
+constexpr int BCR_TOP = 84;
 template <int CL>
-__device__ __forceinline__ double pcr_solve_path(const BaDev& d, cg::cluster_group& cl, int pb, int pe, const double* __restrict__ r, double* __restrict__ z) {
-  const int nl = pcr_num_levels(pe - pb);
-  const int tid = cl.block_rank() * blockDim.x + threadIdx.x, nth = CL * blockDim.x;
-  const int n_items = 6 * (pe - pb);
-  const size_t N6 = 6 * (size_t)d.C, N36 = 36 * (size_t)d.C;
-  const double* src = r;
-  int cur = 0;
-  constexpr int KP = 3;
-  double pa[KP][6], pg[KP][6];
-  auto fetch = [&](int l) {
-    const int s = 1 << l;
-    const double* A = d.pcr_A + l * N36; const double* G = d.pcr_G + l * N36;
-#pragma unroll
-    for (int k = 0; k < KP; ++k) {
-      const int w = tid + k * nth;
-      const int v = pb + w / 6, row = w % 6;
-      const bool ia = w < n_items && v - s >= pb, ig = w < n_items && v + s < pe;
-      const double* a = A + 36 * (size_t)v + 6 * row; const double* g = G + 36 * (size_t)v + 6 * row;
-#pragma unroll
-      for (int i = 0; i < 6; ++i) { pa[k][i] = ia ? a[i] : 0.0; pg[k][i] = ig ? g[i] : 0.0; }
-    }
+__device__ __forceinline__ double pcr_solve_path(const BaDev& d, cg::cluster_group& cl, int pb, int pe, const double* r, double* z) {
+  __shared__ double sb[12 * BCR_TOP], sx[12 * BCR_TOP];
+  const int n = pe - pb, nl = pcr_num_levels(n), rank = (int)cl.block_rank();
+  const int tid = rank * blockDim.x + threadIdx.x, nth = CL * blockDim.x;
+  double* const b = d.pcr_b;
+  int l0 = 0, slots = 0;
+  #pragma unroll 1
+  for (int l = 0; l < nl; ++l) { const int c = bcr_survivors(n, l); if (c > BCR_TOP) l0 = l + 1; slots += c; }
+  {
+    const double *A = d.pcr_A + 72 * (size_t)pb, *G = d.pcr_G + 72 * (size_t)pb, *Di = d.pcr_Dinv + 36 * (size_t)pb;
+    for (int o = 16 * tid; o < 36 * slots; o += 16 * nth) {
+      asm volatile("prefetch.global.L2 [%0];" ::"l"(A + o));
+      asm volatile("prefetch.global.L2 [%0];" ::"l"(G + o));
+    }
+    for (int o = 16 * tid; o < 36 * n; o += 16 * nth) asm volatile("prefetch.global.L2 [%0];" ::"l"(Di + o));
+  }
+  double p0[6], p1[6], x0 = 0.0, rz = 0.0;
+  size_t off = 2 * (size_t)pb;
+  auto fetch_fwd = [&](int w, int end, int s) {
+    const int k = w / 6, i = w - 6 * k;
+    const bool on = w < end, ia = on && k > 0, ig = on && 2 * s * k + s < n;
+    const double* a = d.pcr_A + 36 * (off + k) + 6 * i; const double* g = d.pcr_G + 36 * (off + k) + 6 * i;
+#pragma unroll
+    for (int c = 0; c < 6; ++c) { p0[c] = ia ? a[c] : 0.0; p1[c] = ig ? g[c] : 0.0; }
   };
-  if (nl > 0) fetch(0);
-  for (int l = 0; l < nl; ++l) {
-    double* dst = d.pcr_b + cur * N6;
-    const int s = 1 << l;
-#pragma unroll
-    for (int k = 0; k < KP; ++k) {
-      const int w = tid + k * nth;
-      if (w < n_items) {
-        const int v = pb + w / 6, row = w % 6;
-        double o = src[6 * (size_t)v + row];
-        if (v - s >= pb) { const double* x = src + 6 * (size_t)(v - s); o += pa[k][0] * x[0] + pa[k][1] * x[1] + pa[k][2] * x[2] + pa[k][3] * x[3] + pa[k][4] * x[4] + pa[k][5] * x[5]; }
-        if (v + s < pe) { const double* x = src + 6 * (size_t)(v + s); o += pg[k][0] * x[0] + pg[k][1] * x[1] + pg[k][2] * x[2] + pg[k][3] * x[3] + pg[k][4] * x[4] + pg[k][5] * x[5]; }
-        dst[6 * (size_t)v + row] = o;
-      }
-    }
-    for (int w = tid + KP * nth; w < n_items; w += nth) {
-      const int v = pb + w / 6, row = w % 6;
-      dst[6 * (size_t)v + row] = pcr_apply_row(v, row, pb, pe, s, d.pcr_A + l * N36, d.pcr_G + l * N36, src);
-    }
-    if (l + 1 < nl) fetch(l + 1);
+  auto fetch_back = [&](int w, int end, int s, auto bu) {
+    const int m = w / 6, i = w - 6 * m, j = s + 2 * s * m;
+    const bool on = w < end, ia = on && j + s < n;
+    const double* g = d.pcr_G + 36 * (off + m) + i; const double* a = d.pcr_A + 36 * (off + m + 1) + i;
+#pragma unroll
+    for (int c = 0; c < 6; ++c) { p0[c] = on ? g[6 * c] : 0.0; p1[c] = ia ? a[6 * c] : 0.0; }
+    x0 = on ? dot6(d.pcr_Dinv + 36 * ((size_t)pb + j) + 6 * i, bu(j)) : 0.0;
+  };
+  auto row6 = [](const double* p, const double* x) { return p[0] * x[0] + p[1] * x[1] + p[2] * x[2] + p[3] * x[3] + p[4] * x[4] + p[5] * x[5]; };
+  #pragma unroll 1
+  for (int l = 0; l < l0; ++l) {
+    const int s = 1 << l, end = 6 * bcr_survivors(n, l);
+    const double* src = l ? b : r;
+    int w = tid;
+    fetch_fwd(w, end, s);
+    if (l) cl.sync();
+    for (; w < end; w += nth) {
+      const int k = w / 6, i = w - 6 * k, j = 2 * s * k;
+      const size_t v = pb + j;
+      double o = src[6 * v + i];
+      if (k > 0) o += row6(p0, src + 6 * (v - s));
+      if (j + s < n) o += row6(p1, src + 6 * (v + s));
+      b[6 * v + i] = o;
+      fetch_fwd(w + nth, end, s);
+    }
+    off += end / 6;
+  }
+  if (l0) cl.sync();
+  const int S0 = 1 << l0, nq = (n - 1 + S0) >> l0;
+  if (rank == 0) {
+    const int bd = (int)blockDim.x;
+    const double* src = l0 ? b : r;
+    for (int w = threadIdx.x; w < 6 * nq; w += bd) { const int q = w / 6; sb[w] = src[6 * ((size_t)pb + (size_t)q * S0) + w - 6 * q]; }
+    #pragma unroll 1
+    for (int l = l0; l < nl; ++l) {
+      const int s = 1 << l, h = s >> l0, end = 6 * bcr_survivors(n, l);
+      int w = threadIdx.x;
+      fetch_fwd(w, end, s);
+      __syncthreads();
+      for (; w < end; w += bd) {
+        const int k = w / 6, i = w - 6 * k, q = 2 * h * k;
+        double o = sb[6 * q + i];
+        if (k > 0) o += row6(p0, sb + 6 * (q - h));
+        if (2 * s * k + s < n) o += row6(p1, sb + 6 * (q + h));
+        sb[6 * q + i] = o;
+        fetch_fwd(w + bd, end, s);
+      }
+      off += end / 6;
+    }
+    __syncthreads();
+    if (threadIdx.x < 6) sx[threadIdx.x] = dot6(d.pcr_Dinv + 36 * (size_t)pb + 6 * threadIdx.x, sb);
+    auto sbu = [&](int j) { return sb + 6 * (j >> l0); };
+    #pragma unroll 1
+    for (int l = nl - 1; l >= l0; --l) {
+      const int s = 1 << l, h = s >> l0, end = 6 * bcr_eliminated(n, l);
+      off -= bcr_survivors(n, l);
+      int w = threadIdx.x;
+      fetch_back(w, end, s, sbu);
+      __syncthreads();
+      for (; w < end; w += bd) {
+        const int m = w / 6, i = w - 6 * m, q = h + 2 * h * m;
+        double x = x0 + row6(p0, sx + 6 * (q - h));
+        if (s + 2 * s * m + s < n) x += row6(p1, sx + 6 * (q + h));
+        sx[6 * q + i] = x;
+        fetch_back(w + bd, end, s, sbu);
+      }
+    }
+    __syncthreads();
+    for (int w = threadIdx.x; w < 6 * nq; w += bd) {
+      const int q = w / 6; const size_t e = 6 * ((size_t)pb + (size_t)q * S0) + w - 6 * q;
+      z[e] = sx[w]; rz += sx[w] * r[e];
+    }
+  }
+  #pragma unroll 1
+  for (int l = l0 - 1; l >= 0; --l) {
+    const int s = 1 << l, end = 6 * bcr_eliminated(n, l);
+    const double* src = l ? b : r;
+    off -= bcr_survivors(n, l);
+    int w = tid;
+    fetch_back(w, end, s, [&](int j) { return src + 6 * ((size_t)pb + j); });
     cl.sync();
-    src = dst; cur = 1 - cur;
-  }
-  double rz = 0.0;
-  for (int w = tid; w < n_items; w += nth) {
-    const int v = pb + w / 6, row = w % 6;
-    const double* m = d.Minv + 36 * (size_t)v + 6 * row; const double* x = src + 6 * (size_t)v;
-    const double zz = m[0] * x[0] + m[1] * x[1] + m[2] * x[2] + m[3] * x[3] + m[4] * x[4] + m[5] * x[5];
-    z[6 * (size_t)v + row] = zz;
-    rz += zz * r[6 * (size_t)v + row];
+    for (; w < end; w += nth) {
+      const int m = w / 6, i = w - 6 * m, j = s + 2 * s * m;
+      const size_t u = pb + j;
+      double x = x0 + row6(p0, z + 6 * (u - s));
+      if (j + s < n) x += row6(p1, z + 6 * (u + s));
+      z[6 * u + i] = x; rz += x * r[6 * u + i];
+      fetch_back(w + nth, end, s, [&](int jj) { return src + 6 * ((size_t)pb + jj); });
+    }
   }
   return rz;
 }
@@ -600,6 +672,7 @@
   for (int w = tid; w < 6 * (pe - pb); w += nth) { const size_t q = 6 * (size_t)pb + w; d.r[q] = d.rhs[q]; d.xp[q] = 0.0; }
   if (pe - pb > 1) cl.sync();
   double rz = pcr_solve_path<CL>(d, cl, pb, pe, d.r, d.z);
+  cl.sync();
   for (int w = tid; w < 6 * (pe - pb); w += nth) { const size_t q = 6 * (size_t)pb + w; d.p[q] = d.z[q]; }
   rz = block_sum(rz, red);
   if (threadIdx.x == 0) red[0] = rz;
@@ -607,7 +680,7 @@
   xchg_publish_z<CL>(d, cl, path, pb, pe, red[0], &is_last, total_ctas);
 }
 template <class S, int CL>
-__global__ void __cluster_dims__(CL, 1, 1) __launch_bounds__(256) k_pcg_init(S s) { VDO_PICK k_pcg_init_body<CL>(d, CL > 1 ? 0 : d.n_own_long, pcg_total_ctas(d), blk_); }
+__global__ void __cluster_dims__(CL, 1, 1) __launch_bounds__(256, bcr_ctas_per_sm<S>()) k_pcg_init(S s) { VDO_PICK k_pcg_init_body<CL>(d, CL > 1 ? 0 : d.n_own_long, pcg_total_ctas(d), blk_); }
 __device__ __forceinline__ void k_pcg_init_fin_body(const BaDev& d) {
   __shared__ double red[33];
   __shared__ int okw;
@@ -667,7 +740,7 @@
   if (rz_new <= d.scal[SC_TOL2] * d.scal[SC_RZ0]) d.scal[SC_DONE] = 1.0;
 }
 template <class S, bool FUSED, int CL>
-__global__ void __cluster_dims__(CL, 1, 1) __launch_bounds__(256) k_pcg_step_a(S s) {
+__global__ void __cluster_dims__(CL, 1, 1) __launch_bounds__(256, bcr_ctas_per_sm<S>()) k_pcg_step_a(S s) {
   VDO_PICK k_pcg_step_a_body<FUSED, CL>(d, s.parity() ? d.p : d.p2, CL > 1 ? 0 : d.n_own_long, pcg_total_ctas(d), blk_);
 }
 __device__ __forceinline__ void k_pcg_p_hpp_body(const BaDev& d, const double* __restrict__ p_in, double* __restrict__ p_out, double* __restrict__ out, int bx) {
@@ -1470,6 +1543,7 @@
   }
   void precond_vertex_ter(BaDev& d) override { if (d.tiled) return; auto k = k_vertex_sym<1, false>; LAUNCH(k, d.n_ter_chunks, 128, d); }
   void precond_factor(BaDev& d, double lambda) override { pcr_factor(one(d, lambda)); }
+  void precond_blocks(int C, int, size_t& nDL, size_t& nAG, size_t& nb) const override { nDL = (size_t)C; nAG = 2 * (size_t)C; nb = (size_t)C; }
   void schur_landmarks(BaDev& d, int mode, const double* v) override {
     if (d.tiled) {
       if (mode == 0) rhs_tiles(one(d)); else if (mode == 1) schur_product(one(d), -1, st); else backsub_tiles(one(d));
diff --git a/vdo_slam_b200/csrc/ba_types.h b/vdo_slam_b200/csrc/ba_types.h
--- a/vdo_slam_b200/csrc/ba_types.h
+++ b/vdo_slam_b200/csrc/ba_types.h
@@ -32,7 +32,7 @@
   int *nbr_begin = 0, *nbr_edge = 0, *nbr_other = 0; uint8_t* nbr_tr = 0;
   double *Hpp = 0, *bp = 0, *hll = 0, *bl = 0, *pt_s = 0, *Minv = 0;
   double *pt_g = 0, *tk_gamma = 0;
-  int n_paths = 0, pcr_levels = 0;
+  int n_paths = 0;
   int* path_begin = 0;
   int* path_of = 0;
   int* pcr_edge = 0; uint8_t* pcr_tr = 0;
@@ -137,6 +137,11 @@
   virtual void lin_se3_edges(BaDev& d, bool write) = 0;
   virtual void max_diagonal(BaDev& d) = 0;
   virtual void factor_landmarks(BaDev& d, double lambda) = 0;
+  virtual void precond_blocks(int C, int max_len, size_t& nDL, size_t& nAG, size_t& nb) const {
+    int nl = 1;
+    while ((1 << nl) < max_len) ++nl;
+    nDL = 2 * (size_t)C; nAG = (size_t)C * nl; nb = 2 * (size_t)C;
+  }
   virtual void precond_begin(BaDev& d, double lambda) = 0;
   virtual void precond_vertex_obs(BaDev& d) = 0;
   virtual void precond_vertex_ter(BaDev& d) = 0;
```
